# VachaLab/gorder

Hardware: AMD Instinct MI355X
Metric: trajectory frames/sec (higher is better)
Workload: dtype f32

## Files before the change

### gorder_amd/csrc/gorder_hip.hip

```cpp
#include <hip/hip_runtime.h>

#include <dlfcn.h>

#include <cmath>
#include <cstdio>
#include <cstdlib>
#include <cstring>
#include <mutex>
#include <new>
#include <string>
#include <deque>
#include <type_traits>
#include <vector>

#include "../../include/gorder_hip.h"
#include "gm_math.h"
#include "plan.h"
#include "collect_store.h"
#include "device_mem.h"
#include "replay_rows.h"
#include "leaflet_rows.h"
#include "timewise_blocks.h"
#include "ordermap_final.h"
#include "order_route.h"
#include "molecule_rows.h"
#include "ua_molecule_rows.h"
#include "order_hist.h"
#include "bond_corr.h"
#include "neighbour_classes.h"

#pragma clang fp contract(off)

using gorder::DirectItem;
using gorder::Item;
using gorder::kBlock;
using gorder::Plan;
using gorder::Tile;

#include "kernels_common.h"
#include "kernels_tile.h"
#include "kernels_bonds.h"
#include "kernels_extras.h"
#include "kernels_ua.h"
#include "kernels_molrows.h"
#include "kernels_radial.h"
#include "kernels_neighbours.h"
#include "kernels_hist.h"
#include "kernels_ua_samples.h"
#include "kernels_corr.h"
#include "kernels_leaflets.h"
#include "kernels_cluster.h"
#include "kernels_cluster_cutoff.h"
#include "kernels_normals.h"
#include "kernels_xtc.h"
#include "kernels_trr.h"
#include "kernels_collect.h"
#include "kernels_replay.h"
#include "kernels_timewise.h"
#include "kernels_ordermap.h"


struct DeviceMem {
    static void *alloc(size_t bytes) { void *p = nullptr; return hipMalloc(&p, bytes) == hipSuccess ? p : nullptr; }
    static void release(void *p) { (void)hipFree(p); }
};
struct PinnedMem {
    static void *alloc(size_t bytes) { void *p = nullptr; return hipHostMalloc(&p, bytes) == hipSuccess ? p : nullptr; }
    static void release(void *p) { (void)hipHostFree(p); }
};
template <typename T> using DBuf = gorder::Buf<T, DeviceMem>;
template <typename T> using HBuf = gorder::Buf<T, PinnedMem>;
using u64 = unsigned long long;

struct Event {
    hipEvent_t ev = nullptr;
    Event() = default;
    Event(const Event &) = delete;
    Event &operator=(const Event &) = delete;
    ~Event() { if (ev) (void)hipEventDestroy(ev); }
    hipError_t create(unsigned flags = hipEventDisableTiming) { return ev ? hipSuccess : hipEventCreateWithFlags(&ev, flags); }
    operator hipEvent_t() const { return ev; }
};
struct Stream {
    hipStream_t s = nullptr;
    Stream() = default;
    Stream(const Stream &) = delete;
    Stream &operator=(const Stream &) = delete;
    ~Stream() { if (s) (void)hipStreamDestroy(s); }
    hipError_t create() { return s ? hipSuccess : hipStreamCreateWithFlags(&s, hipStreamNonBlocking); }
    operator hipStream_t() const { return s; }
};

struct RepAcc {
    DBuf<u64> acc, rep;
    uint32_t n_rep = 1;
    size_t words = 0;
    bool alloc(size_t n_words, uint32_t n_rep_wanted) {
        words = n_words;
        n_rep = gorder::replica_count(n_rep_wanted, n_words);
        return acc.alloc(words) && rep.alloc((size_t)n_rep * words);
    }
    void reset() { acc.reset(); rep.reset(); words = 0; }
    hipError_t zero_async(hipStream_t stream) {
        const hipError_t e = hipMemsetAsync(acc, 0, words * sizeof(u64), stream);
        return e != hipSuccess ? e : hipMemsetAsync(rep, 0, (size_t)n_rep * words * sizeof(u64), stream);
    }
    hipError_t fold(hipStream_t stream) {
        hipLaunchKernelGGL(k_fold_replicas, dim3((uint32_t)((words + 255) / 256)), dim3(256), 0, stream, acc.get(), rep.get(), n_rep, (uint32_t)words);
        return hipGetLastError();
    }
};

struct BondCorr {
    std::vector<uint32_t> lags;
    DBuf<uint32_t> d_lags;
    DBuf<float4> ring;
    uint32_t ring_planes = 0, subrange = 0;
    uint32_t plane_items = 0;
    uint64_t seen = 0;
    RepAcc acc;
    uint32_t forced_subrange = 0;
    bool chunk_major = false;
    bool on() const { return !lags.empty(); }
};

struct NeighbourClasses {
    uint32_t n_classes = 0;
    float radius = 0.0f, thr = 0.0f;
    std::vector<uint32_t> centres, neighbours;
    DBuf<uint32_t> d_centres, d_neighbours;
    DBuf<uint8_t> rows;
    uint32_t rows_frames = 0;
    RepAcc acc;
    size_t lds_bytes = 0;
    bool direct = false;
    bool force_direct = false;
    uint32_t forced_subrange = 0;
    uint64_t row_bytes = gorder::kClassRowBytes;
    bool on() const { return n_classes != 0; }
};

struct gorder_hip_handle {
    void *traj_cache = nullptr;
    void (*traj_cache_free)(gorder_hip_handle *) = nullptr;
    Plan plan;
    gorder_tables_t tables{};
    int device = 0;
    Stream own_stream;
    hipStream_t stream = nullptr;
    DBuf<Tile> d_tiles;
    DBuf<Item> d_items;
    DBuf<uint32_t> d_tile_slots;
    DBuf<DirectItem> d_direct;
    DBuf<Tile> d_ua_tiles;
    DBuf<gorder::UaItem> d_ua_items;
    DBuf<uint32_t> d_ua_tile_slots;
    uint32_t map_nx = 0, map_ny = 0;
    DBuf<u64> d_map_sums, d_map_cnts;
    DBuf<u64> d_map_packed;
    DBuf<u64> d_map_rec;
    DBuf<gorder::MapRun> d_ua_runs, d_runs;
    DBuf<uint32_t> d_ua_run_begin, d_run_begin;
    DBuf<Item> d_items_by_slot;
    DBuf<uint32_t> d_ua_item_run, d_item_run;
    DBuf<uint4> d_lgrid;
    DBuf<LocalRowPre> d_lrowpre;
    DBuf<LocalEdge> d_ledge;
    DBuf<float4> d_lfinfo;
    static constexpr uint32_t kDecidePause = 16;
    DBuf<uint32_t> d_lsummary;
    HBuf<uint32_t> h_lsummary;
    Event lsummary_written;
    bool lsummary_pending = false;
    uint32_t decide_pause = 0;
    uint64_t decide_submits = 0, decide_paused_submits = 0;
    DBuf<uint32_t> d_lneed;
    DBuf<uint2> d_ltodo;
    size_t map_lds_bytes = 0;
    bool map_staged = false;
    uint64_t map_pending = 0;
    uint64_t map_fold_limit = kMapFoldLimit;
    uint32_t map_max_mol = 1;
    DBuf<u64> d_tw_sums, d_tw_cnts;
    uint64_t tw_cap = 0;
    DBuf<u64> d_twx_blocks, d_twx_rows, d_twx_totals, d_twx_edge;
    DBuf<uint32_t> d_twx_groups;
    DBuf<float> d_twx_out;
    DBuf<uint32_t> d_omx_groups;
    DBuf<float> d_omx_out;
    ExtraArgs extra{};
    DBuf<uint32_t> d_geom_group;
    DBuf<float> d_shapes;
    DBuf<float> d_inv_box;
    uint32_t dyn_slab = 4, local_slab = 4;
    bool local_halo = false;
    size_t local_rec_stride = 0;
    DBuf<XtcCheckpoint> d_xtc_cp;
    bool dyn = false;
    DBuf<uint32_t> d_dyn_cloud, d_dyn_heads;
    DBuf<uint32_t> d_dyn_cell_of, d_dyn_count;
    DBuf<float> d_dyn_rec;
    DBuf<float4> d_dyn_normals;
    DBuf<DynCov> d_dyn_cov;
    std::vector<float> last_normals;
    std::vector<float> manual_normals;
    uint32_t manual_frames = 0;
    bool manual_active = false;
    DBuf<uint32_t> d_err;
    u64 *d_acc = nullptr;
    DBuf<u64> own_acc;
    DBuf<u64> d_rep;
    uint32_t n_rep = 32;
    bool rep_dirty = false;
    size_t acc_words = 0;
    DBuf<uint32_t> d_heads, d_membrane, d_methyl_begin, d_methyl_atoms;
    DBuf<uint8_t> d_aflags;
    size_t aflags_rows = 0;
    DBuf<float> d_adist;
    DBuf<float> d_sph_spill, d_sph_stats;
    uint32_t sph_spill = 0, sph_slab = 1u << 20, sph_threads = 1024;
    DBuf<char> d_cl_scratch;
    DBuf<uint32_t> d_cl_head_slot;
    DBuf<uint8_t> d_cl_carry, d_cl_is0;
    DBuf<float> d_cl_stats;
    uint32_t cl_slab = 1, cl_m_max = 0;
    bool cl_stored_w = false;
    bool cl_have_carry = false;
    bool cl_cut = false;
    uint32_t cl_tiles = 0, cl_sort = 0;
    std::vector<uint8_t> cl_is0;
    DBuf<uint32_t> d_lcell_of, d_lcell_count, d_lcell_fill;
    DBuf<float> d_ltrig;
    DBuf<uint32_t> d_arow, d_aframes;
    std::vector<uint32_t> up_arow, up_aframes;
    bool up_arow_valid = false, up_aframes_valid = false;
    bool have_assignment = false;
    uint64_t assignment_frame = 0;
    bool spec_enabled = false;
    DBuf<uint2> d_own;
    DBuf<float4> d_mom;
    DBuf<float> d_head_z;
    DBuf<uint32_t> d_own_head_begin;
    DBuf<uint2> d_own_heads;
    DBuf<float> d_spec_center;
    DBuf<uint8_t> d_spec_ok;
    DBuf<uint32_t> d_spec_counters;
    static constexpr uint32_t kSpecRing = 8;
    HBuf<uint32_t> h_spec_counters;
    Event spec_counters_copied[kSpecRing];
    uint64_t spec_ring_frames[kSpecRing] = {};
    DBuf<uint32_t> d_spec_mol_begin;
    DBuf<SpecSample> d_spec_samples;
    uint64_t spec_batches = 0, spec_fixed = 0, spec_exact_frames = 0;
    DBuf<float> d_stage_xyz[2], d_stage_box[2];
    Event stage_copied[2], stage_computed[2];
    bool stage_used[2] = {false, false};
    int stage_next = 0;
    Stream copy_stream;
    float n2 = 1.0f, n2sq = 1.0f;
    int axis = -1;
    int frames_per_stage = kFramesPerStage;
    bool membrane_is_frame = false;
    bool use_gather = false;
    uint32_t wg_capacity = 256u * 6u;
    uint32_t wg_target = 0;
    uint32_t lw = 0;
    size_t lds_bytes = 0;
    uint64_t n_frames = 0;
    uint64_t err_index = 0;
    std::string err_msg;
    static constexpr uint32_t kTimingEvents = 1024;
    struct TimingSeg { uint32_t label, ev_a, ev_b; };
    bool timing_on = false;
    Event timing_ev[kTimingEvents];
    uint32_t timing_next_ev = 0;
    int timing_open_label = -1;
    uint32_t timing_open_ev = 0;
    std::deque<TimingSeg> timing_pending;
    std::vector<std::string> timing_labels;
    std::vector<double> timing_label_ms;
    std::vector<uint64_t> timing_label_n;
    uint64_t timing_launches = 0;
    std::string timed_kernels;
    std::vector<uint32_t> host_heads, host_dyn_heads;
    DBuf<uint32_t> d_mol_slot0;
    uint64_t err_frame = 0;
    struct BatchLog { uint64_t ordinal, first, stride; std::vector<uint64_t> list; };
    static constexpr size_t kBatchLog = 4096;
    std::deque<BatchLog> batch_log;
    uint64_t n_submits = 0;
    const unsigned long long *decoder_key = nullptr;
    uint32_t collect = 0;
    bool collect_locked = false;
    gorder::CollectStore collect_flags;
    gorder::CollectStore collect_normals;
    DBuf<u64> d_collect_words;
    DBuf<CollectVec3> d_collect_vec;
    DBuf<uint8_t> d_touched;
    DBuf<u64> d_ltable;
    gorder::ReplayWindow ltable_win;
    bool replay_have_carry = false;
    uint64_t replay_carry_index = 0;
    DBuf<ReplayVec3> d_ntable;
    gorder::ReplayWindow ntable_win;
    uint32_t ntable_step = 1;
    DBuf<uint32_t> d_nrow;
    uint32_t n_shells = 0;
    float shell_thr[GORDER_RADIAL_MAX_SHELLS] = {};
    RepAcc shells;
    size_t shell_lds_bytes = 0;
    bool shell_direct = false;
    bool shell_force_direct = false;
    uint32_t hist_edges = 0;
    DBuf<int32_t> d_hist_edges;
    RepAcc hist;
    size_t hist_table_words = 0;
    bool hist_direct = false;
    bool hist_force_direct = false;
    uint32_t hist_samples_per_word = gorder::kDistSamplesPerWord;
    BondCorr corr;
    NeighbourClasses nb;
    gorder::MolRows mol;
    DBuf<Item> d_mol_items;
    DBuf<gorder::MolRun> d_mol_runs;
    DBuf<uint32_t> d_mol_run_begin;
    gorder::UaMolRows ua_mol;
    DBuf<gorder::UaLaneWords> d_ua_mol_lanes;
    DBuf<uint32_t> d_ua_mol_words, d_ua_mol_word_begin;
    DBuf<u64> d_mol_stage;
    size_t mol_stage_bytes = (size_t)1 << 30;
    gorder::CollectStore mol_store;
    const uint64_t *mol_frame_index = nullptr;
    bool mol_failed = false;
    std::deque<std::pair<uint64_t, uint64_t>> mol_batch_log;
};

namespace {

int fail(gorder_hip_handle *h, int status, const std::string &msg) {
    if (h) h->err_msg = msg;
    return status;
}

#define HIP_TRY(h, expr)                                                                    \
    do {                                                                                    \
        hipError_t e_ = (expr);                                                             \
        if (e_ != hipSuccess)                                                               \
            return fail(h, GORDER_ERR_DEVICE, std::string(#expr) + ": " + hipGetErrorString(e_)); \
    } while (0)

#define ST_TRY(expr)                                \
    do {                                            \
        const int st_ = (expr);                     \
        if (st_ != GORDER_OK) return st_;           \
    } while (0)

int alloc_failed(gorder_hip_handle *h, const char *call) {
    return fail(h, GORDER_ERR_DEVICE, std::string(call) + ": " + hipGetErrorString(hipGetLastError()));
}

template <typename T, typename Mem>
int allocate(gorder_hip_handle *h, gorder::Buf<T, Mem> &dst, size_t n, int fill = -1) {
    if (!dst.alloc(n)) return alloc_failed(h, std::is_same<Mem, DeviceMem>::value ? "hipMalloc" : "hipHostMalloc");
    if (fill >= 0 && n) HIP_TRY(h, hipMemset(dst, fill, n * sizeof(T)));
    return GORDER_OK;
}

template <typename T>
int upload(gorder_hip_handle *h, DBuf<T> &dst, const std::vector<T> &src) {
    ST_TRY(allocate(h, dst, src.size()));
    if (!src.empty()) HIP_TRY(h, hipMemcpy(dst, src.data(), src.size() * sizeof(T), hipMemcpyHostToDevice));
    return GORDER_OK;
}

template <typename T>
int ensure(gorder_hip_handle *h, DBuf<T> &buf, size_t need, bool *grew = nullptr) {
    const gorder::Reserve r = buf.reserve(need);
    if (grew) *grew = r == gorder::Reserve::Grew;
    return r == gorder::Reserve::Failed ? alloc_failed(h, "hipMalloc") : GORDER_OK;
}

int alloc_zeroed(gorder_hip_handle *h, RepAcc &r, size_t words) {
    if (!r.alloc(words, h->n_rep)) {
        r.reset();
        return alloc_failed(h, "hipMalloc");
    }
    HIP_TRY(h, r.zero_async(h->stream));
    return GORDER_OK;
}

uint32_t sample_atom(const Plan &p, uint32_t slot, uint32_t mol, uint32_t which) {
    for (const Tile &t : p.tiles)
        for (uint32_t q = 0; q < t.n_items; q++) {
            const Item &it = p.items[t.item0 + q];
            if (it.mol == mol && p.tile_slots[t.slot0 + it.lslot] == slot) return t.atom0 + (which ? it.lj : it.li);
        }
    for (const DirectItem &d : p.direct)
        if (d.mol == mol && d.slot == slot) return which ? d.j : d.i;
    for (const Tile &t : p.ua_tiles)
        for (uint32_t q = 0; q < t.n_items; q++) {
            const gorder::UaItem &it = p.ua_items[t.item0 + q];
            if (it.mol == mol && p.ua_tile_slots[t.slot0 + it.lslot0] == slot) return t.atom0 + it.l[which & 3u];
        }
    return 0;
}

// ... 217 lines not shown
                                       b.aflags, b.arow, h->d_tiles, h->d_mol_items, h->d_tile_slots, n_tiles, h->lw);
                });
            }); }); });
            HIP_TRY(h, hipGetLastError());
        }
        if (ua) {
            const gorder::FrameChunks c = gorder::extras_chunks(nf, n_ua, h->wg_target, h->wg_capacity, false, true);
            const uint64_t grid = ua_grid(n_ua, c.n_chunks);
            if (grid > 0x7fffffffull) return fail(h, GORDER_ERR_INVALID_ARGUMENT, "batch too large");
            b.frames_per_chunk = c.frames_per_chunk;
            if (bonds) TIMING_MARK(h, "k_ua_mol");
            with_bool(ac, [&](auto AC) {
                hipLaunchKernelGGL((k_ua_mol<AC()>), dim3((uint32_t)grid), dim3(kBlock), gorder::ua_mol_lds_bytes(h->ua_mol.max_local), h->stream, b, e,
                                   um, b.xyz, b.box9, b.aflags, b.arow, h->d_ua_tiles, h->d_ua_items, h->d_ua_tile_slots, n_ua);
            });
            HIP_TRY(h, hipGetLastError());
        }
        if ((st = collect_copy_out(h, h->mol_store, h->d_mol_stage, h->mol_frame_index + lo, nf)) != GORDER_OK) return st;
    }
    return GORDER_OK;
}

bool literal_cosine(const gorder_hip_handle *h) { return (h->tables.flags & GORDER_FLAG_TRIG_ACOS_COS) != 0; }

int launch_geometry_shapes(gorder_hip_handle *h, const FrameArgs &a) {
    ST_TRY(ensure(h, h->d_shapes, (size_t)a.n_frames * 8));
    const gorder_geometry_t &ge = h->tables.geometry;
    GeomArgs ga{};
    ga.xyz = a.xyz; ga.box9 = a.box9; ga.n_atoms = a.n_atoms; ga.pbc = a.pbc;
    ga.kind = ge.kind; ga.reference = ge.reference; ga.orientation = ge.orientation;
    for (int d = 0; d < 3; d++) { ga.point[d] = ge.point[d]; ga.structure_box[d] = ge.structure_box[d]; }
    for (int d = 0; d < 2; d++) { ga.xdim[d] = ge.xdim[d]; ga.ydim[d] = ge.ydim[d]; ga.zdim[d] = ge.zdim[d]; ga.span[d] = ge.span[d]; }
    ga.radius = ge.radius; ga.group = h->d_geom_group; ga.n_group = ge.n_group;
    ga.shapes = h->d_shapes; ga.err = h->d_err;
    TIMING_MARK(h, "k_geom_shapes");
    hipLaunchKernelGGL(k_geom_shapes, dim3(a.n_frames), dim3(256), 0, h->stream, ga);
    HIP_TRY(h, hipGetLastError());
    return GORDER_OK;
}

int launch_tiled(gorder_hip_handle *h, FrameArgs &a, const gorder::OrderRoute &route) {
    const uint32_t n_tiles = (uint32_t)h->plan.tiles.size();
    const gorder::FrameChunks c = gorder::tiled_chunks(a.n_frames, (uint32_t)h->frames_per_stage, n_tiles, h->wg_target, h->wg_capacity);
    a.frames_per_chunk = c.frames_per_chunk;
    const uint64_t grid = (uint64_t)n_tiles * c.n_chunks;
    if (grid > 0x7fffffffull) return fail(h, GORDER_ERR_INVALID_ARGUMENT, "batch too large");
    const dim3 g((uint32_t)grid), b(kBlock);
    TIMING_MARK(h, route.label);
    with_bool(literal_cosine(h), [&](auto AC) { with_bool(a.pbc, [&](auto PBC) { with_bool(a.leaflets, [&](auto LF) {
        if (route.family == gorder::BondFamily::Gather)
            hipLaunchKernelGGL((k_bonds_gather<4, AC(), PBC(), LF()>), g, b, 0, h->stream, a, a.xyz, a.box9, a.aflags, a.arow,
                               h->d_tiles, h->d_items, h->d_tile_slots, n_tiles);
        else with_npf(route.npf, [&](auto NPF) { with_axis(h->axis, [&](auto AX) { with_bool(route.mom, [&](auto MOM) {
            if constexpr (LF() || !MOM())
                hipLaunchKernelGGL((k_bonds_tiled<4, NPF(), AC(), PBC(), LF(), AX(), MOM()>), g, b, h->lds_bytes, h->stream, a,
                                   a.xyz, a.box9, a.aflags, a.arow, h->d_tiles, h->d_items, h->d_tile_slots, n_tiles, h->lw);
        }); }); });
    }); }); });
    HIP_TRY(h, hipGetLastError());
    return GORDER_OK;
}

struct SubRange {
    const FrameArgs &a;
    const gorder::OrderRoute &route;
    uint32_t lo, hi;
    bool class_rows_whole;
    uint32_t nf() const { return hi - lo; }
    FrameArgs frames(const gorder::FrameChunks &c) const {
        FrameArgs b = a;
        b.frame0 = lo; b.n_frames = hi; b.frames_per_chunk = c.frames_per_chunk;
        return b;
    }
};
const Item *bond_items(const gorder_hip_handle *h, const gorder::OrderRoute &route) { return route.items_by_slot ? h->d_items_by_slot : h->d_items; }

int launch_classes(gorder_hip_handle *h, const SubRange &s) {
    const Plan &p = h->plan;
    NeighbourClasses &nb = h->nb;
    const uint32_t nt = (uint32_t)p.tiles.size(), nf = s.nf();
    const gorder::FrameChunks c = gorder::shells_chunks(nf, nt, h->wg_target, h->wg_capacity, kShellChunkMax);
    FrameArgs b = s.frames(c);
    ClassArgs ca{};
    ca.centres = nb.d_centres; ca.neighbours = nb.d_neighbours; ca.n_neighbours = (uint32_t)nb.neighbours.size();
    ca.thr = nb.thr; ca.n = nb.n_classes; ca.rows = nb.rows; ca.row_base = s.class_rows_whole ? 0u : s.lo;
    ca.axis = h->axis; ca.rep = nb.acc.rep; ca.n_rep = nb.acc.n_rep;
    nb.rows_frames = s.class_rows_whole ? s.a.n_frames : nf;
    TIMING_MARK(h, "k_neighbour_counts");
    hipLaunchKernelGGL(k_neighbour_counts, dim3((p.n_mol_total + 255u) / 256u, nf), dim3(256), 0, h->stream, ca, b.xyz, b.box9,
                       b.n_atoms, p.n_mol_total, b.pbc, s.lo, h->d_err);
    TIMING_MARK(h, s.route.label);
    const size_t lds = nb.direct ? (size_t)kBlock * 24u : nb.lds_bytes;
    with_bool(literal_cosine(h), [&](auto AC) { with_bool(nb.direct, [&](auto DIRECT) {
        hipLaunchKernelGGL((k_bonds_classes<AC(), DIRECT()>), dim3(nt * c.n_chunks), dim3(kBlock), lds, h->stream, b, ca, b.xyz, b.box9,
                           b.aflags, b.arow, h->d_tiles, bond_items(h, s.route), h->d_tile_slots, nt);
    }); });
    return GORDER_OK;
}

int launch_shells(gorder_hip_handle *h, const SubRange &s, const ExtraArgs &e) {
    const uint32_t nt = (uint32_t)h->plan.tiles.size();
    const gorder::FrameChunks c = gorder::shells_chunks(s.nf(), nt, h->wg_target, h->wg_capacity, kShellChunkMax);
    FrameArgs b = s.frames(c);
    ShellArgs sa{};
    sa.n = h->n_shells; sa.rep = h->shells.rep; sa.n_rep = h->shells.n_rep;
    for (uint32_t k = 0; k < GORDER_RADIAL_MAX_SHELLS; k++) sa.thr[k] = k < h->n_shells ? h->shell_thr[k] : INFINITY;
    const size_t lds = h->shell_direct ? (size_t)kBlock * 24u : h->shell_lds_bytes;
    TIMING_MARK(h, s.route.label);
    with_bool(literal_cosine(h), [&](auto AC) { with_bool(h->shell_direct, [&](auto DIRECT) {
        hipLaunchKernelGGL((k_bonds_shells<AC(), DIRECT()>), dim3(nt * c.n_chunks), dim3(kBlock), lds, h->stream, b, e, sa, b.xyz, b.box9,
                           b.aflags, b.arow, h->d_tiles, bond_items(h, s.route), h->d_tile_slots, nt);
    }); });
    return GORDER_OK;
}

int launch_dist(gorder_hip_handle *h, const SubRange &s, const ExtraArgs &e) {
    const uint32_t nt = (uint32_t)h->plan.tiles.size();
    const gorder::FrameChunks c = gorder::dist_chunks(s.nf(), nt, h->wg_target, h->wg_capacity, h->hist_direct ? 0u : (uint32_t)h->hist_table_words,
                                                      h->hist_samples_per_word, kDistChunkMax);
    FrameArgs b = s.frames(c);
    DistArgs da{};
    da.n_edges = h->hist_edges; da.edges = h->d_hist_edges; da.rep = h->hist.rep; da.n_rep = h->hist.n_rep;
    const size_t lds = kDistEdgeBytes + std::max<size_t>(kDistReduceBytes, h->hist_direct ? 0u : h->hist_table_words * sizeof(uint32_t));
    TIMING_MARK(h, s.route.label);
    with_bool(literal_cosine(h), [&](auto AC) { with_bool(h->hist_direct, [&](auto DIRECT) {
        hipLaunchKernelGGL((k_bonds_dist<AC(), DIRECT()>), dim3(nt * c.n_chunks), dim3(kBlock), lds, h->stream, b, e, da, b.xyz, b.box9,
                           b.aflags, b.arow, h->d_tiles, bond_items(h, s.route), h->d_tile_slots, nt);
    }); });
    return GORDER_OK;
}

int launch_extras(gorder_hip_handle *h, const SubRange &s, const ExtraArgs &e) {
    const uint32_t nt = (uint32_t)h->plan.tiles.size();
    const gorder::FrameChunks c = gorder::extras_chunks(s.nf(), nt, h->wg_target, h->wg_capacity, s.route.map_accumulate, false);
    FrameArgs b = s.frames(c);
    TIMING_MARK(h, s.route.label);
    with_bool(literal_cosine(h), [&](auto AC) { with_bool(s.route.maps_only, [&](auto MO) {
        hipLaunchKernelGGL((k_bonds_extras<AC(), MO()>), dim3(nt * c.n_chunks), dim3(kBlock), 0, h->stream, b, e, b.xyz, b.box9, b.aflags,
                           b.arow, h->d_tiles, bond_items(h, s.route), h->d_tile_slots, nt);
    }); });
    return GORDER_OK;
}

int launch_tiled_out(gorder_hip_handle *h, const SubRange &s, const ExtraArgs &e) {
    const gorder::OrderRoute &route = s.route;
    const uint32_t nt = (uint32_t)h->plan.tiles.size();
    const gorder::FrameChunks c = gorder::extras_chunks(s.nf(), nt, h->wg_target, h->wg_capacity, route.map_accumulate,
                                                        route.family == gorder::BondFamily::TiledTw);
    FrameArgs b = s.frames(c);
    const dim3 g(nt * c.n_chunks), blk(kBlock);
    const Item *items = bond_items(h, route);
    TIMING_MARK(h, route.label);
    with_npf(route.npf, [&](auto NPF) { with_bool(b.pbc, [&](auto PBC) { with_bool(b.leaflets, [&](auto LF) { with_axis(h->axis, [&](auto AX) {
        if (route.family == gorder::BondFamily::TiledMaps)
            hipLaunchKernelGGL((k_bonds_tiled_maps<NPF(), PBC(), LF(), AX()>), g, blk, h->lds_bytes, h->stream, b, e, b.xyz,
                               b.box9, b.aflags, b.arow, h->d_tiles, items, h->d_tile_slots, nt, h->lw);
        else with_bool(route.tw_maps, [&](auto MAPS) { with_bool(route.mom, [&](auto MOM) {
            if constexpr (!MOM() || (LF() && !MAPS()))
                hipLaunchKernelGGL((k_bonds_tiled_tw<NPF(), PBC(), LF(), AX(), MAPS(), MOM()>), g, blk, h->lds_bytes, h->stream, b, e,
                                   b.xyz, b.box9, b.aflags, b.arow, h->d_tiles, items, h->d_tile_slots, nt, h->lw);
        }); });
    }); }); }); });
    return GORDER_OK;
}

int launch_map_accumulate(gorder_hip_handle *h, const SubRange &s, uint32_t rec_stride, const gorder::MapRun *runs,
                          const uint32_t *run_begin, uint32_t per_item) {
    const uint32_t n_acc = h->plan.n_acc;
    const uint32_t planes = h->tables.leaflets.method != GORDER_LEAFLETS_NONE ? 2u : 1u;
    const uint32_t ntm = h->map_nx * h->map_ny, n_words = planes * ntm;
    const char *ev = getenv("GORDER_HIP_MAP_CHUNKS");
    const gorder::FrameChunks m = gorder::map_chunks(s.nf(), n_acc, ev ? (uint32_t)std::max(1, atoi(ev)) : 0u);
    TIMING_MARK(h, "k_map_accumulate");
    hipLaunchKernelGGL(k_map_accumulate, dim3(n_acc * m.n_chunks), dim3(1024), n_words * sizeof(unsigned long long), h->stream,
                       h->d_map_rec, runs, run_begin, n_acc, s.nf(), rec_stride, m.frames_per_chunk, per_item, n_words, ntm,
                       h->d_map_packed, n_acc);
    return GORDER_OK;
}

int launch_bond_pass(gorder_hip_handle *h, const SubRange &s, ExtraArgs &e) {
    using gorder::BondFamily;
    e.item_run = h->d_item_run;
    switch (s.route.family) {
    case BondFamily::Classes: ST_TRY(launch_classes(h, s)); break;
    case BondFamily::Shells: ST_TRY(launch_shells(h, s, e)); break;
    case BondFamily::Dist: ST_TRY(launch_dist(h, s, e)); break;
    case BondFamily::Extras: ST_TRY(launch_extras(h, s, e)); break;
    default: ST_TRY(launch_tiled_out(h, s, e)); break;
    }
    if (s.route.map_accumulate) ST_TRY(launch_map_accumulate(h, s, e.rec_stride, h->d_runs, h->d_run_begin, 1u));
    HIP_TRY(h, hipGetLastError());
    return GORDER_OK;
}

int launch_ua_dist(gorder_hip_handle *h, const SubRange &s, const ExtraArgs &e) {
    const uint32_t nt = (uint32_t)h->plan.ua_tiles.size();
    const gorder::FrameChunks c = gorder::dist_chunks(s.nf(), nt, h->wg_target, h->wg_capacity, h->hist_direct ? 0u : (uint32_t)h->hist_table_words,
                                                      h->hist_samples_per_word, kDistChunkMax);
    FrameArgs b = s.frames(c);
    DistArgs da{};
    da.n_edges = h->hist_edges; da.edges = h->d_hist_edges; da.rep = h->hist.rep; da.n_rep = h->hist.n_rep;
    const size_t lds = kDistEdgeBytes + std::max<size_t>(kUaSumBytes, h->hist_direct ? 0u : h->hist_table_words * sizeof(uint32_t));
    const dim3 g((uint32_t)ua_grid(nt, c.n_chunks)), blk(kBlock);
    TIMING_MARK(h, "k_ua_dist");
    with_bool(literal_cosine(h), [&](auto AC) { with_bool(h->hist_direct, [&](auto DIRECT) {
        hipLaunchKernelGGL((k_ua_dist<AC(), DIRECT()>), g, blk, lds, h->stream, b, e, da, b.xyz, b.box9, b.aflags, b.arow, h->d_ua_tiles,
                           h->d_ua_items, h->d_ua_tile_slots, nt);
    }); });
    HIP_TRY(h, hipGetLastError());
    return GORDER_OK;
}

int launch_ua_pass(gorder_hip_handle *h, const SubRange &s, ExtraArgs &e) {
    const gorder::OrderRoute &route = s.route;
    if (route.ua_kernel == gorder::UaKernel::Dist) return launch_ua_dist(h, s, e);
    const uint32_t nt = (uint32_t)h->plan.ua_tiles.size();
    const gorder::FrameChunks c = gorder::extras_chunks(s.nf(), nt, h->wg_target, h->wg_capacity, route.map_accumulate, false);
    FrameArgs b = s.frames(c);
    e.item_run = h->d_ua_item_run;
    const dim3 g((uint32_t)ua_grid(nt, c.n_chunks)), blk(kBlock);
    TIMING_MARK(h, "k_ua_extras");
    with_bool(literal_cosine(h), [&](auto AC) { with_bool(route.ua_fast, [&](auto FAST) { with_int<0, 1, 2, 3>(route.ua_mode, [&](auto MODE) {
        if constexpr (FAST() && !AC())
            hipLaunchKernelGGL((k_ua_extras_fast<MODE()>), g, blk, 0, h->stream, b, e, b.xyz, b.box9, b.aflags, b.arow,
                               h->d_ua_tiles, h->d_ua_items, h->d_ua_tile_slots, nt, (const float *)e.inv_box);
        else if constexpr (!FAST())
            hipLaunchKernelGGL((k_ua_extras<AC(), MODE()>), g, blk, 0, h->stream, b, e, b.xyz, b.box9, b.aflags, b.arow,
                               h->d_ua_tiles, h->d_ua_items, h->d_ua_tile_slots, nt, (const float *)nullptr);
    }); }); });
    if (route.map_accumulate) ST_TRY(launch_map_accumulate(h, s, e.rec_stride, h->d_ua_runs, h->d_ua_run_begin, 3u));
    HIP_TRY(h, hipGetLastError());
    return GORDER_OK;
}

int launch_scatter_passes(gorder_hip_handle *h, const FrameArgs &a, const gorder::OrderRoute &route) {
    const Plan &p = h->plan;
    ExtraArgs e = h->extra;
    e.tw_sums = h->d_tw_sums; e.tw_cnts = h->d_tw_cnts; e.tw_row0 = h->n_frames;
    e.shapes = h->d_shapes; e.inv_box = nullptr;
    if (route.ua_fast && a.pbc) {
        ST_TRY(ensure(h, h->d_inv_box, (size_t)a.n_frames * 8));
        hipLaunchKernelGGL(k_inv_box, dim3((4u * a.n_frames + 255u) / 256u), dim3(256), 0, h->stream, a.box9, a.n_frames, h->d_inv_box);
        e.inv_box = h->d_inv_box;
    }
    e.dyn = (h->dyn || h->manual_active) ? h->d_dyn_normals : nullptr;
    const bool staged = route.map_accumulate;
    const size_t rec_per_frame = std::max(p.ua_tiles.size() * 3u, route.extras ? p.tiles.size() : (size_t)0) * kBlock;
    uint32_t sub = gorder::map_subrange(a.n_frames, e.maps != 0, staged, h->map_fold_limit, h->map_max_mol, rec_per_frame);
    bool class_rows_whole = false;
    if (route.family == gorder::BondFamily::Classes) {
        class_rows_whole = gorder::class_rows_whole(a.n_frames, p.n_mol_total, h->nb.row_bytes);
        sub = gorder::class_subrange(a.n_frames, p.n_mol_total, h->nb.forced_subrange, h->nb.row_bytes);
        ST_TRY(ensure(h, h->nb.rows, (size_t)(class_rows_whole ? a.n_frames : sub) * p.n_mol_total));
    }
    if (staged) ST_TRY(ensure(h, h->d_map_rec, rec_per_frame * (((size_t)sub + 15) / 16 * 16)));
    e.map_rec = staged ? h->d_map_rec : nullptr;
    for (uint32_t lo = 0; lo < a.n_frames; lo += sub) {
        const SubRange s{a, route, lo, std::min(a.n_frames, lo + sub), class_rows_whole};
        if (e.maps) {
            const uint64_t cost = (uint64_t)s.nf() * h->map_max_mol;
            if (h->map_pending + cost >= h->map_fold_limit) ST_TRY(fold_maps(h));
            h->map_pending += cost;
        }
        e.rec_frame0 = lo; e.rec_stride = (s.nf() + 15u) / 16u * 16u;
        if (route.extras && !p.tiles.empty()) ST_TRY(launch_bond_pass(h, s, e));
        if (!p.ua_tiles.empty() && route.ua_kernel != gorder::UaKernel::Mol) ST_TRY(launch_ua_pass(h, s, e));
    }
    return GORDER_OK;
}

int launch_bonds_direct(gorder_hip_handle *h, const FrameArgs &a) {
    const uint32_t n_items = (uint32_t)h->plan.direct.size(), bpc = (n_items + kBlock - 1) / kBlock;
    const gorder::FrameChunks c = gorder::direct_chunks(a.n_frames, bpc, h->wg_target);
    FrameArgs b = a;
    b.frames_per_chunk = c.frames_per_chunk;
    TIMING_MARK(h, "k_bonds_direct");
    with_bool(literal_cosine(h), [&](auto AC) { hipLaunchKernelGGL(k_bonds_direct<AC()>, dim3(bpc * c.n_chunks), dim3(kBlock), 0, h->stream, b, h->d_direct, n_items, bpc); });
    HIP_TRY(h, hipGetLastError());
    return GORDER_OK;
}

int launch_orders(gorder_hip_handle *h, FrameArgs &a, const gorder::OrderRoute &route) {
    using gorder::BondFamily;
    if (h->dyn && !h->manual_active) ST_TRY(run_dynamic_normals(h, a));
    if (h->extra.geom_kind) ST_TRY(launch_geometry_shapes(h, a));
    if (route.family == BondFamily::Tiled || route.family == BondFamily::Gather) ST_TRY(launch_tiled(h, a, route));
    const bool ua_mol = route.ua_kernel == gorder::UaKernel::Mol;
    if (route.family == BondFamily::TiledMol || ua_mol) ST_TRY(launch_molecule_rows(h, a, route));
    if (route.extras || (route.ua_mode >= 0 && !ua_mol)) ST_TRY(launch_scatter_passes(h, a, route));
    if (route.direct) ST_TRY(launch_bonds_direct(h, a));
    return GORDER_OK;
}

int collect_copy_out(gorder_hip_handle *h, gorder::CollectStore &store, const void *d_block, const uint64_t *frames, size_t n_rows) {
    std::vector<gorder::CollectPiece> pieces;
    if (!store.reserve(frames, n_rows, pieces)) return fail(h, GORDER_ERR_DEVICE, "collect: no pinned host memory for the history");
    const char *src = static_cast<const char *>(d_block);
    for (const gorder::CollectPiece &pc : pieces) {
        const size_t bytes = pc.rows * store.row_bytes();
        HIP_TRY(h, hipMemcpyAsync(pc.host, src, bytes, hipMemcpyDeviceToHost, h->stream));
        src += bytes;
    }
    return GORDER_OK;
}

int collect_flag_rows(gorder_hip_handle *h, size_t first_row, const std::vector<uint64_t> &frames) {
    if (frames.empty()) return GORDER_OK;
    const uint32_t n_mol = h->plan.n_mol_total, wpr = (uint32_t)gorder::collect_flag_words(n_mol);
    const unsigned long long total = (unsigned long long)frames.size() * wpr;
    if ((total + 3u) / 4u > 0x7fffffffull || frames.size() > 0xffffffffull) return fail(h, GORDER_ERR_INVALID_ARGUMENT, "collect: batch too large");
    int st;
    if ((st = ensure(h, h->d_collect_words, (size_t)total)) != GORDER_OK) return st;
    TIMING_MARK(h, "k_collect_flags");
    hipLaunchKernelGGL(k_collect_flags, dim3((uint32_t)((total + 3u) / 4u)), dim3(256), 0, h->stream,
                       h->d_aflags + first_row * (size_t)n_mol, n_mol, (uint32_t)frames.size(), wpr, h->d_collect_words);
    HIP_TRY(h, hipGetLastError());
    return collect_copy_out(h, h->collect_flags, h->d_collect_words, frames.data(), frames.size());
}

int collect_normal_rows(gorder_hip_handle *h, const uint64_t *frame_index, uint32_t n_frames, const uint8_t *touched) {
    const unsigned long long n = (unsigned long long)n_frames * h->plan.n_mol_total;
    if ((n + 255u) / 256u > 0x7fffffffull) return fail(h, GORDER_ERR_INVALID_ARGUMENT, "collect: batch too large");
    int st;
    if ((st = ensure(h, h->d_collect_vec, (size_t)n)) != GORDER_OK) return st;
    TIMING_MARK(h, "k_collect_normals");
    hipLaunchKernelGGL(k_collect_normals, dim3((uint32_t)((n + 255u) / 256u)), dim3(256), 0, h->stream,
                       (const float4 *)h->d_dyn_normals, touched, n, h->d_collect_vec);
    HIP_TRY(h, hipGetLastError());
    return collect_copy_out(h, h->collect_normals, h->d_collect_vec, frame_index, n_frames);
}

int upload_rows(gorder_hip_handle *h, DBuf<uint32_t> &buf, const std::vector<uint32_t> &rows) {
    ST_TRY(ensure(h, buf, rows.size()));
    HIP_TRY(h, hipMemcpyAsync(buf, rows.data(), rows.size() * sizeof(uint32_t), hipMemcpyHostToDevice, h->stream));
    return GORDER_OK;
}
int upload_if_changed(gorder_hip_handle *h, DBuf<uint32_t> &buf, std::vector<uint32_t> &held, bool &valid, const std::vector<uint32_t> &rows) {
    bool grew = false;
    const int st = ensure(h, buf, rows.size(), &grew);
    if (grew || st != GORDER_OK) valid = false;
    if (st != GORDER_OK || (valid && held == rows)) return st;
    ST_TRY(upload_rows(h, buf, rows));
// ... 168 lines not shown
    }
    return st;
}

namespace {
__global__ void k_selftest_trig(int fn, uint32_t first_bits, uint32_t stride, uint32_t n, float *out) {
    const uint32_t i = blockIdx.x * blockDim.x + threadIdx.x;
    if (i >= n) return;
    const float x = __uint_as_float(first_bits + i * stride);
    float s, c;
    gm_sincosf_0pi(x, s, c);
    out[i] = fn == 0 ? gm_acosf_t<false>(x) : fn == 1 ? gm_acosf_t<true>(x) : fn == 2 ? c : s;
}
}

int gorder_hip_selftest_trig(int device, int fn, uint32_t first_bits, uint32_t stride, uint32_t n, float *out) {
    if (!out || fn < 0 || fn > 3) return GORDER_ERR_INVALID_ARGUMENT;
    int count = 0;
    if (hipGetDeviceCount(&count) != hipSuccess || count <= 0) return GORDER_ERR_NO_DEVICE;
    if (device < 0 || device >= count || hipSetDevice(device) != hipSuccess) return GORDER_ERR_INVALID_ARGUMENT;
    if (n == 0) return GORDER_OK;
    DBuf<float> d;
    if (!d.alloc(n)) return GORDER_ERR_DEVICE;
    hipLaunchKernelGGL(k_selftest_trig, dim3((n + 255u) / 256u), dim3(256), 0, 0, fn, first_bits, stride, n, d.get());
    if (hipDeviceSynchronize() != hipSuccess || hipMemcpy(out, d, (size_t)n * sizeof(float), hipMemcpyDeviceToHost) != hipSuccess)
        return GORDER_ERR_DEVICE;
    return GORDER_OK;
}

namespace {
__global__ __launch_bounds__(1024) void k_selftest_wave_ops(const double *in_f64, const float *in_f32, const uint32_t *in_u32,
                                                            int finfo_empty, double *out_f64, float *out_f32, uint32_t *out_u32,
                                                            uint4 *out_finfo) {
    __shared__ double scratch[32];
    __shared__ float fscratch[32], l_lo[16], l_hi[16];
    __shared__ uint32_t l_flags[16];
    const uint32_t tid = threadIdx.x, lane = tid & 63u, n = blockDim.x;
    const double d = in_f64[tid];
    const float x = in_f32[tid];
    const uint32_t u = in_u32[tid];
    if (tid < 16u) { l_lo[tid] = 3.0e38f; l_hi[tid] = -3.0e38f; l_flags[tid] = 0u; }
    __syncthreads();
    double s = d, q = 3.0 * d, bs[2] = {d, 3.0 * d};
    float lo4 = x, hi4 = x, lo2 = x, hi2 = x, lo3 = x, hi3 = x, blo = x, bhi = x;
    uint32_t or3 = u;
    wave_sum2_minmax_bfly(s, q, lo4, hi4);
    wave_minmax_bfly(lo2, hi2);
    wave_minmax_or_bfly(lo3, hi3, or3);
    block_sum_n<2>(bs, scratch);
    block_minmax(blo, bhi, fscratch);
    const double o64[GORDER_WAVE_OPS_F64_ROWS] = {row_sum(d), rows_to_wave(row_sum(d)), wave_sum_rows(d), wave_scan_rows(d, lane),
                                                  wave_sum_bfly(d), bs[0], bs[1], lane_value(d, 47), s, q};
    const float o32[GORDER_WAVE_OPS_F32_ROWS] = {row_sum(x), rows_to_wave(row_sum(x)), wave_sum_rows(x), wave_min_rows(x),
                                                 wave_max_rows(x), lo2, hi2, blo, bhi, dpp_or_self<0x111>(x),
                                                 dpp_or_zero<0x143, 0xc>(x), lane_value(x, 47), lo4, hi4, lo3, hi3};
    const uint32_t ou[GORDER_WAVE_OPS_U32_ROWS] = {row_sum(u), rows_to_wave(row_sum(u)), wave_sum_rows(u), wave_scan_rows(u, lane),
                                                   wave_scan_shfl(u, lane), or3, wave_max_bfly(u),
                                                   (uint32_t)wave_sum_rows((int)u), lane_value(u, 47)};
    for (int r = 0; r < GORDER_WAVE_OPS_F64_ROWS; r++) out_f64[r * n + tid] = o64[r];
    for (int r = 0; r < GORDER_WAVE_OPS_F32_ROWS; r++) out_f32[r * n + tid] = o32[r];
    for (int r = 0; r < GORDER_WAVE_OPS_U32_ROWS; r++) out_u32[r * n + tid] = ou[r];
    const float zlo = finfo_empty ? 3.0e38f : x, zhi = finfo_empty ? -3.0e38f : x;
    uint32_t fl = u;
    block_finfo_record(zlo, zhi, fl, ~0u, l_lo, l_hi, l_flags, out_finfo);
    if (tid == 0u) out_finfo[2].x = fl;
    __syncthreads();
    fl = u;
    block_finfo_record(zlo, zhi, fl, 1u, l_lo, l_hi, l_flags, out_finfo + 1);
}
}

int gorder_hip_selftest_wave_ops(int device, uint32_t block, const double *f64, const float *f32, const uint32_t *u32,
                                 int finfo_empty, double *out_f64, float *out_f32, uint32_t *out_u32, uint32_t *out_finfo) {
    if (!f64 || !f32 || !u32 || !out_f64 || !out_f32 || !out_u32 || !out_finfo || block < 64u || block > 1024u || (block & 63u))
        return GORDER_ERR_INVALID_ARGUMENT;
    int count = 0;
    if (hipGetDeviceCount(&count) != hipSuccess || count <= 0) return GORDER_ERR_NO_DEVICE;
    if (device < 0 || device >= count || hipSetDevice(device) != hipSuccess) return GORDER_ERR_INVALID_ARGUMENT;
    const size_t n = block, b_fi = 0, b_i64 = 48, b_o64 = b_i64 + 8 * n, b_i32 = b_o64 + 8 * n * GORDER_WAVE_OPS_F64_ROWS,
                 b_iu = b_i32 + 4 * n, b_o32 = b_iu + 4 * n, b_ou = b_o32 + 4 * n * GORDER_WAVE_OPS_F32_ROWS,
                 bytes = b_ou + 4 * n * GORDER_WAVE_OPS_U32_ROWS;
    DBuf<char> owned;
    if (!owned.alloc(bytes)) return GORDER_ERR_DEVICE;
    char *d = owned;
    int st = GORDER_OK;
    if (hipMemset(d, 0, bytes) != hipSuccess || hipMemcpy(d + b_i64, f64, 8 * n, hipMemcpyHostToDevice) != hipSuccess ||
        hipMemcpy(d + b_i32, f32, 4 * n, hipMemcpyHostToDevice) != hipSuccess ||
        hipMemcpy(d + b_iu, u32, 4 * n, hipMemcpyHostToDevice) != hipSuccess)
        st = GORDER_ERR_DEVICE;
    if (st == GORDER_OK) {
        hipLaunchKernelGGL(k_selftest_wave_ops, dim3(1), dim3(block), 0, 0, (const double *)(d + b_i64), (const float *)(d + b_i32),
                           (const uint32_t *)(d + b_iu), finfo_empty, (double *)(d + b_o64), (float *)(d + b_o32),
                           (uint32_t *)(d + b_ou), (uint4 *)(d + b_fi));
        if (hipDeviceSynchronize() != hipSuccess ||
            hipMemcpy(out_f64, d + b_o64, 8 * n * GORDER_WAVE_OPS_F64_ROWS, hipMemcpyDeviceToHost) != hipSuccess ||
            hipMemcpy(out_f32, d + b_o32, 4 * n * GORDER_WAVE_OPS_F32_ROWS, hipMemcpyDeviceToHost) != hipSuccess ||
            hipMemcpy(out_u32, d + b_ou, 4 * n * GORDER_WAVE_OPS_U32_ROWS, hipMemcpyDeviceToHost) != hipSuccess ||
            hipMemcpy(out_finfo, d + b_fi, 4 * GORDER_WAVE_OPS_FINFO_WORDS, hipMemcpyDeviceToHost) != hipSuccess)
            st = GORDER_ERR_DEVICE;
    }
    return st;
}

int gorder_hip_plan_tables(const gorder_tables_t *tables, gorder_hip_plan_t *out, int *selfcheck) {
    if (!tables || !out) return GORDER_ERR_INVALID_ARGUMENT;
    Plan p;
    ST_TRY(gorder::build_plan(*tables, env_flag("GORDER_HIP_FORCE_DIRECT"), p));
    out->n_tiles = (uint32_t)p.tiles.size();
    out->block_threads = kBlock;
    out->max_window_atoms = p.max_window;
    out->n_direct_items = (uint32_t)p.direct.size();
    out->frames_per_stage = kFramesPerStage;
    const uint32_t lw = ((3u * p.max_window + 3u + 3u) / 4u) * 4u;
    size_t lds = (size_t)kFramesPerStage * lw * sizeof(float);
    if (lds < (size_t)kBlock * 24) lds = (size_t)kBlock * 24;
    out->lds_bytes = (uint32_t)lds;
    out->map_staged = 0;
    out->map_lds_bytes = 0;
    out->leaflets_one_read = p.spec_ok ? 1u : 0u;
    if (selfcheck) *selfcheck = gorder::selfcheck_plan(*tables, p);
    return GORDER_OK;
}

static size_t cl_frame_bytes(uint32_t n, uint32_t m_max);
static size_t clcut_frame_bytes(uint32_t n, uint32_t m_max);

static int create_ordermaps(gorder_hip_handle *h, const gorder_tables_t *t) {
    const gorder_ordermap_t &om = t->ordermap;
    if (!om.enabled) return GORDER_OK;
    const Plan &p = h->plan;
    ExtraArgs &e = h->extra;
    if (!(om.bin[0] > 0.0f) || !(om.bin[1] > 0.0f) || om.plane > 2)
        return fail(h, GORDER_ERR_INVALID_ARGUMENT, "ordermap bin/plane");
    const float fx = roundf((om.span_x[1] - om.span_x[0]) / om.bin[0]);
    const float fy = roundf((om.span_y[1] - om.span_y[0]) / om.bin[1]);
    if (!(fx >= 0.0f) || !(fy >= 0.0f) || fx > 65535.0f || fy > 65535.0f)
        return fail(h, GORDER_ERR_INVALID_ARGUMENT, "ordermap span");
    h->map_nx = (uint32_t)fx + 1u;
    h->map_ny = (uint32_t)fy + 1u;
    const size_t nmap = 3 * (size_t)p.n_acc * h->map_nx * h->map_ny;
    const size_t npk = (t->leaflets.method != GORDER_LEAFLETS_NONE ? 2 : 1) * (nmap / 3);
    ST_TRY(allocate(h, h->d_map_sums, nmap, 0));
    ST_TRY(allocate(h, h->d_map_cnts, nmap, 0));
    ST_TRY(allocate(h, h->d_map_packed, npk, 0));
    const size_t lds_bytes = npk / p.n_acc * sizeof(u64);
    h->map_lds_bytes = lds_bytes;
    if (lds_bytes <= 150u * 1024u && !env_flag("GORDER_HIP_MAP_DIRECT")) {
        ST_TRY(upload(h, h->d_ua_runs, p.ua_runs));
        ST_TRY(upload(h, h->d_ua_run_begin, p.ua_run_begin));
        ST_TRY(upload(h, h->d_runs, p.runs));
        ST_TRY(upload(h, h->d_run_begin, p.run_begin));
        ST_TRY(upload(h, h->d_items_by_slot, p.items_by_slot));
        ST_TRY(upload(h, h->d_ua_item_run, p.ua_item_run));
        HIP_TRY(h, hipFuncSetAttribute(reinterpret_cast<const void *>(k_map_accumulate),
                                       hipFuncAttributeMaxDynamicSharedMemorySize, (int)lds_bytes));
        h->map_staged = true;
    }
    e.maps = 1; e.plane = om.plane; e.x0 = om.span_x[0]; e.y0 = om.span_y[0];
    e.binx = om.bin[0]; e.biny = om.bin[1]; e.nx = h->map_nx; e.ny = h->map_ny;
    e.inv_binx = 1.0f / om.bin[0]; e.inv_biny = 1.0f / om.bin[1];
    e.bin_core = (om.bin[0] >= 0x1p-40f && om.bin[0] <= 0x1p+40f && om.bin[1] >= 0x1p-40f && om.bin[1] <= 0x1p+40f) ? 1 : 0;
    e.map_packed = h->d_map_packed;
    return GORDER_OK;
}

static int create_geometry(gorder_hip_handle *h, const gorder_tables_t *t) {
    const gorder_geometry_t &ge = t->geometry;
    if (ge.kind == GORDER_GEOM_NONE) return GORDER_OK;
    ExtraArgs &e = h->extra;
    if (ge.kind > GORDER_GEOM_SPHERE || ge.reference > GORDER_GEOMREF_GROUP || ge.orientation > 2)
        return fail(h, GORDER_ERR_INVALID_ARGUMENT, "geometry kind/reference/orientation");
    if (ge.reference == GORDER_GEOMREF_BOX_CENTER && !t->handle_pbc)
        return fail(h, GORDER_ERR_INVALID_ARGUMENT, "box-centre reference needs handle_pbc (pbc.rs:243-245)");
    if (ge.reference == GORDER_GEOMREF_POINT && t->handle_pbc &&
        !(ge.structure_box[0] > 0.0f && ge.structure_box[1] > 0.0f && ge.structure_box[2] > 0.0f))
        return fail(h, GORDER_ERR_INVALID_ARGUMENT, "geometry.structure_box");
    if (ge.reference == GORDER_GEOMREF_GROUP) {
        if (!ge.group || ge.n_group == 0) return fail(h, GORDER_ERR_INVALID_ARGUMENT, "geometry.group");
        std::vector<uint32_t> grp(ge.group, ge.group + ge.n_group);
        for (uint32_t a : grp)
            if (a >= t->n_atoms) return fail(h, GORDER_ERR_INVALID_ARGUMENT, "geometry group index out of range");
        ST_TRY(upload(h, h->d_geom_group, grp));
    }
    e.geom_kind = (int)ge.kind; e.geom_invert = ge.invert ? 1 : 0; e.geom_orient = (int)ge.orientation;
    e.geom_thr = local_radius_threshold(ge.radius);
    h->tables.geometry.group = nullptr;
    return GORDER_OK;
}

static int create_accumulators(gorder_hip_handle *h) {
    const Plan &p = h->plan;
    ST_TRY(allocate(h, h->d_err, kErrWords + 2u));
    HIP_TRY(h, hipMemset(h->d_err, 0xff, kErrWords * sizeof(uint32_t)));
    HIP_TRY(h, hipMemset(h->d_err + kErrWords, 0, 2u * sizeof(uint32_t)));
    h->acc_words = 4 * (size_t)p.n_acc + 1;
    ST_TRY(allocate(h, h->own_acc, h->acc_words, 0));
    h->d_acc = h->own_acc;
    if (const char *e = getenv("GORDER_HIP_MAP_FOLD_LIMIT")) {
        const long v = atol(e);
        if (v >= 2 && (unsigned long long)v <= kMapFoldLimit) h->map_fold_limit = (uint64_t)v;
    }
    if (const char *e = getenv("GORDER_HIP_REPLICAS")) {
        const int r = atoi(e);
        if (r >= 1 && r <= 1024) h->n_rep = (uint32_t)r;
    }
    return p.n_acc ? allocate(h, h->d_rep, (size_t)h->n_rep * 4u * p.n_acc, 0) : GORDER_OK;
}

static int local_build_attributes(gorder_hip_handle *h) {
    for (const void *fn : {reinterpret_cast<const void *>(k_local_build<2>), reinterpret_cast<const void *>(k_local_build<5>),
                           reinterpret_cast<const void *>(k_local_build<kLocalBuildTrips>)})
        HIP_TRY(h, hipFuncSetAttribute(fn, hipFuncAttributeMaxDynamicSharedMemorySize, (int)kLocalBuildLds));
    return GORDER_OK;
}

static int create_dynamic_normals(gorder_hip_handle *h, const gorder_tables_t *t) {
    const gorder_dynamic_normal_t &dn = t->dynamic_normal;
    if (!dn.enabled) return GORDER_OK;
    const Plan &p = h->plan;
    if (!(dn.radius > 0.0f)) return fail(h, GORDER_ERR_INVALID_ARGUMENT, "dynamic normals need a positive radius");
    if (!dn.cloud || dn.n_cloud == 0) return fail(h, GORDER_ERR_INVALID_ARGUMENT, "dynamic normals need the NormalHeads group");
    if (!p.direct.empty()) return fail(h, GORDER_ERR_INVALID_ARGUMENT, "dynamic normals: a bond spans more than the LDS window");
    std::vector<uint32_t> cloud(dn.cloud, dn.cloud + dn.n_cloud), nheads;
    for (uint32_t a : cloud)
        if (a >= t->n_atoms) return fail(h, GORDER_ERR_INVALID_ARGUMENT, "NormalHeads index out of range");
    for (uint32_t m = 0; m < t->n_molecule_types; m++) {
        const gorder_moltype_t &mt = t->molecule_types[m];
        if (!mt.normal_heads) return fail(h, GORDER_ERR_INVALID_ARGUMENT, "dynamic normals need normal_heads[] per molecule type");
        for (uint32_t k = 0; k < mt.n_molecules; k++) {
            if (mt.normal_heads[k] >= t->n_atoms) return fail(h, GORDER_ERR_INVALID_ARGUMENT, "normal head index out of range");
            nheads.push_back(mt.normal_heads[k]);
        }
    }
    ST_TRY(upload(h, h->d_dyn_cloud, cloud));
    ST_TRY(upload(h, h->d_dyn_heads, nheads));
    h->host_dyn_heads = nheads;
    const size_t nm = dn.n_cloud, ncell = (size_t)kLocalMaxCells1D * kLocalMaxCells1D;
    const size_t sl = h->dyn_slab = local_slab_frames(nm);
    ST_TRY(local_build_attributes(h));
    ST_TRY(allocate(h, h->d_dyn_cell_of, sl * nm));
    ST_TRY(allocate(h, h->d_dyn_rec, sl * nm * 4));
    ST_TRY(allocate(h, h->d_dyn_count, sl * (2 * ncell + 1)));
    ST_TRY(allocate(h, h->d_dyn_cov, sl * (size_t)(p.n_mol_total ? p.n_mol_total : 1)));
    h->dyn = true;
    return GORDER_OK;
}

static int create_leaflet_tables(gorder_hip_handle *h, const gorder_tables_t *t, std::vector<uint32_t> &heads) {
    const gorder_leaflets_t &lf = t->leaflets;
    const Plan &p = h->plan;
    if (lf.method > GORDER_LEAFLETS_CLUSTERING) return fail(h, GORDER_ERR_INVALID_ARGUMENT, "leaflets.method");
    if (lf.method != GORDER_LEAFLETS_SPHERICAL && lf.method != GORDER_LEAFLETS_CLUSTERING && lf.normal_dim > 2) return fail(h, GORDER_ERR_INVALID_ARGUMENT, "leaflets.normal_dim");
    std::vector<uint32_t> mb(1, 0), ma;
    for (uint32_t m = 0; m < t->n_molecule_types; m++) {
        const gorder_moltype_t &mt = t->molecule_types[m];
        if (lf.method != GORDER_LEAFLETS_MANUAL && !mt.heads)
            return fail(h, GORDER_ERR_INVALID_ARGUMENT, "leaflets need heads[] per molecule type");
        if (lf.method == GORDER_LEAFLETS_INDIVIDUAL && (!mt.methyls || mt.n_methyls == 0))
            return fail(h, GORDER_ERR_INVALID_ARGUMENT, "individual leaflets need methyls[]");
        for (uint32_t k = 0; k < mt.n_molecules; k++) {
            const uint32_t hd = mt.heads ? mt.heads[k] : 0;
            if (hd >= t->n_atoms) return fail(h, GORDER_ERR_INVALID_ARGUMENT, "head index out of range");
            heads.push_back(hd);
            if (lf.method == GORDER_LEAFLETS_INDIVIDUAL)
                for (uint32_t q = 0; q < mt.n_methyls; q++) {
                    const uint32_t a = mt.methyls[(size_t)k * mt.n_methyls + q];
                    if (a >= t->n_atoms) return fail(h, GORDER_ERR_INVALID_ARGUMENT, "methyl index out of range");
                    ma.push_back(a);
                }
            mb.push_back((uint32_t)ma.size());
        }
    }
    ST_TRY(upload(h, h->d_heads, heads));
    h->host_heads = heads;
    if (lf.method == GORDER_LEAFLETS_LOCAL) {
        std::vector<uint32_t> ms;
        for (uint32_t m = 0; m < t->n_molecule_types; m++) ms.insert(ms.end(), t->molecule_types[m].n_molecules, p.slot0[m]);
        ST_TRY(upload(h, h->d_mol_slot0, ms));
    }
    ST_TRY(upload(h, h->d_methyl_begin, mb));
    ST_TRY(upload(h, h->d_methyl_atoms, ma));
    if (lf.method == GORDER_LEAFLETS_LOCAL && !(lf.radius > 0.0f))
        return fail(h, GORDER_ERR_INVALID_ARGUMENT, "local leaflets need a positive radius");
    if (lf.method == GORDER_LEAFLETS_GLOBAL || lf.method == GORDER_LEAFLETS_LOCAL) {
        if (!lf.membrane || lf.n_membrane == 0)
            return fail(h, GORDER_ERR_INVALID_ARGUMENT, "global/local leaflets need the membrane group");
        std::vector<uint32_t> mem(lf.membrane, lf.membrane + lf.n_membrane);
        for (uint32_t a : mem)
            if (a >= t->n_atoms) return fail(h, GORDER_ERR_INVALID_ARGUMENT, "membrane index out of range");
        ST_TRY(upload(h, h->d_membrane, mem));
        h->membrane_is_frame = lf.n_membrane == t->n_atoms && !env_flag("GORDER_HIP_LEAFLETS_GENERIC");
        for (uint32_t i = 0; i < lf.n_membrane && h->membrane_is_frame; i++) h->membrane_is_frame = mem[i] == i;
    }
    return GORDER_OK;
}

static int upload_cluster_group(gorder_hip_handle *h, const gorder_tables_t *t, const std::vector<uint32_t> &heads, bool ascending,
                                std::vector<uint32_t> &head_slot) {
    const gorder_leaflets_t &lf = t->leaflets;
    std::vector<uint32_t> grp(lf.membrane, lf.membrane + lf.n_membrane);
    std::vector<int32_t> slot_of(t->n_atoms, -1);
    for (uint32_t i = 0; i < lf.n_membrane; i++) {
        if (grp[i] >= t->n_atoms) return fail(h, GORDER_ERR_INVALID_ARGUMENT, "leaflets.membrane: index out of range");
        if (ascending && i && grp[i] <= grp[i - 1]) return fail(h, GORDER_ERR_INVALID_ARGUMENT, "leaflets.membrane: clustering needs ascending, distinct atoms");
        if (slot_of[grp[i]] < 0) slot_of[grp[i]] = (int32_t)i;
    }
    for (uint32_t hd : heads) {
// ... 398 lines not shown
        hipLaunchKernelGGL(k_cluster_embed, dim3(ns), dim3(1024), 0, h->stream, ca);
        TIMING_MARK(h, "k_cluster_orient");
        hipLaunchKernelGGL(k_cluster_orient, dim3(1), dim3(1024), 0, h->stream, oa);
    }
    h->cl_have_carry = true;
    return GORDER_OK;
}

static int launch_global_leaflets(gorder_hip_handle *h, const LeafletArgs &la) {
    const dim3 g(la.skip ? std::min<uint32_t>(la.n_assign, 512u) : la.n_assign), b(1024);
    TIMING_MARK(h, h->membrane_is_frame ? "k_leaflets_global_contig" : "k_leaflets_global");
    if (h->membrane_is_frame) {
        if (la.skip) hipLaunchKernelGGL(k_leaflets_global_contig<true>, g, dim3(256), 0, h->stream, la);
        else hipLaunchKernelGGL(k_leaflets_global_contig<false>, g, dim3(256), 0, h->stream, la);
    } else {
        if (la.skip) hipLaunchKernelGGL(k_leaflets_global<true>, g, b, 0, h->stream, la);
        else hipLaunchKernelGGL(k_leaflets_global<false>, g, b, 0, h->stream, la);
    }
    return GORDER_OK;
}

static int launch_individual_leaflets(gorder_hip_handle *h, const LeafletArgs &la) {
    TIMING_MARK(h, "k_leaflets_individual");
    for (uint32_t done = 0; done < la.n_assign;) {
        const uint32_t ny = std::min<uint32_t>(la.n_assign - done, 65535u);
        LeafletArgs lb = la;
        lb.aframes = la.aframes + done;
        lb.row0 = la.row0 + done;
        if (done + ny < la.n_assign) lb.adist = nullptr;
        hipLaunchKernelGGL(k_leaflets_individual, dim3((la.n_mol_total + 255) / 256, ny), dim3(256), 0,
                           h->stream, lb);
        done += ny;
    }
    return GORDER_OK;
}

static int launch_spherical_leaflets(gorder_hip_handle *h, const LeafletArgs &la) {
    TIMING_MARK(h, "k_leaflets_spherical");
    SphArgs sa{};
    sa.xyz = la.xyz; sa.box9 = la.box9; sa.n_atoms = la.n_atoms;
    sa.aflags = la.aflags; sa.n_mol_total = la.n_mol_total; sa.heads = la.heads;
    sa.group = la.membrane; sa.n_group = la.n_membrane;
    sa.flip = la.flip; sa.pbc = la.pbc;
    sa.spill = h->d_sph_spill; sa.n_spill = h->sph_spill; sa.err = la.err;
    for (size_t done = 0; done < la.n_assign; done += h->sph_slab) {
        const uint32_t ns = (uint32_t)std::min<size_t>(la.n_assign - done, h->sph_slab);
        const bool last = done + ns == la.n_assign;
        sa.aframes = la.aframes + done;
        sa.row0 = la.row0 + (uint32_t)done;
        sa.n_assign = ns;
        sa.adist = last ? h->d_adist : nullptr;
        sa.stats = last ? h->d_sph_stats : nullptr;
        if (h->sph_threads == 256u) hipLaunchKernelGGL(k_leaflets_spherical<256>, dim3(ns), dim3(256), 0, h->stream, sa);
        else hipLaunchKernelGGL(k_leaflets_spherical<1024>, dim3(ns), dim3(1024), 0, h->stream, sa);
    }
    return GORDER_OK;
}

struct LocalDecisions { bool decide, sums, report; };
static LocalDecisions local_decisions(gorder_hip_handle *h, const LocalArgs &lo) {
    LocalDecisions d{};
    d.decide = lo.halo && lo.prune && lo.n_mol_total && !env_flag("GORDER_HIP_LOCAL_NO_DECIDE");
    if (d.decide) {
        if (h->lsummary_pending) {
            if (hipEventQuery(h->lsummary_written) == hipSuccess) {
                h->lsummary_pending = false;
                if (2u * h->h_lsummary[0] > h->h_lsummary[1]) h->decide_pause = gorder_hip_handle::kDecidePause;
            } else {
                (void)hipGetLastError();
            }
        }
        if (h->decide_pause) { h->decide_pause--; h->decide_paused_submits++; d.decide = false; }
        else h->decide_submits++;
    }
    d.sums = d.decide && lo.n_membrane <= kLocalBuildMax && !env_flag("GORDER_HIP_LOCAL_THREE_KERNELS") &&
             !env_flag("GORDER_HIP_LOCAL_NO_SUMS");
    d.report = d.decide && !h->lsummary_pending;
    return d;
}

static int launch_local_slabs(gorder_hip_handle *h, LocalArgs lo, uint32_t n_assign, uint32_t row0, bool report) {
    const size_t ncell = (size_t)kLocalMaxCells1D * kLocalMaxCells1D;
    for (size_t done = 0; done < n_assign; done += h->local_slab) {
        const uint32_t ns = (uint32_t)std::min<size_t>(n_assign - done, h->local_slab);
        lo.aframes = h->d_aframes + done;
        lo.n_slab = ns;
        lo.row0 = row0 + (uint32_t)done;
        lo.write_dist_frame = (done + ns == n_assign) ? (int)ns - 1 : -1;
        lo.summary_host = report && done + ns == n_assign ? h->h_lsummary : nullptr;
        if (lo.n_membrane > kLocalBuildMax || env_flag("GORDER_HIP_LOCAL_THREE_KERNELS"))
            HIP_TRY(h, hipMemsetAsync(h->d_lcell_fill, 0, ns * ncell * sizeof(uint32_t), h->stream));
        if (lo.sums) {
            HIP_TRY(h, hipMemsetAsync(h->d_lneed, 0, (ns + 1) * sizeof(uint32_t), h->stream));
            TIMING_MARK(h, "k_local_sums");
            hipLaunchKernelGGL(k_local_sums, dim3(ns), dim3(1024), kSumsLds, h->stream, lo);
            TIMING_MARK(h, "k_local_decide");
            hipLaunchKernelGGL(k_local_decide, dim3(ns), dim3(1024), kDecideLds, h->stream, lo);
        }
        ST_TRY(launch_cell_list(h, lo, ns, lo.n_membrane, h->d_lcell_count, ns * (ncell + 1) * sizeof(uint32_t)));
        if (lo.halo) {
            TIMING_MARK(h, "k_local_rowprefix");
            hipLaunchKernelGGL(k_local_rowprefix, dim3(kLocalMaxCells1D / 4u, ns), dim3(256), 0, h->stream, lo);
            lo.rows_groups = (lo.n_mol_total + 15u) / 16u;
            if (lo.need && !lo.sums) {
                TIMING_MARK(h, "k_local_decide");
                hipLaunchKernelGGL(k_local_decide, dim3(ns), dim3(1024), kDecideLds, h->stream, lo);
            }
            TIMING_MARK(h, "k_local_flags_rows");
            if (lo.need) hipLaunchKernelGGL(k_local_flags_rows_open, dim3(lo.rows_groups * 8u * kRowsSlots), dim3(256), 0, h->stream, lo);
            else hipLaunchKernelGGL(k_local_flags_rows, dim3(lo.rows_groups * ((ns + 7u) / 8u * 8u)), dim3(256), 0, h->stream, lo);
            TIMING_MARK(h, "k_local_flags_todo");
            hipLaunchKernelGGL(k_local_flags_todo, dim3(512), dim3(256), 0, h->stream, lo);
        } else {
            TIMING_MARK(h, "k_local_flags");
            hipLaunchKernelGGL(k_local_flags, dim3((lo.n_mol_total + 3) / 4, ns), dim3(256), 0, h->stream, lo);
        }
    }
    return GORDER_OK;
}

static int launch_local_leaflets(gorder_hip_handle *h, const LeafletArgs &la) {
    const gorder_leaflets_t &lf = h->tables.leaflets;
    LocalArgs lo{};
    lo.xyz = la.xyz; lo.box9 = la.box9; lo.n_atoms = la.n_atoms;
    lo.aflags = la.aflags; lo.adist = la.adist; lo.n_mol_total = la.n_mol_total;
    lo.heads = la.heads; lo.mol_slot0 = h->d_mol_slot0; lo.n_membrane = la.n_membrane;
    lo.membrane = h->membrane_is_frame ? nullptr : h->d_membrane;
    lo.dim = la.dim; lo.flip = la.flip; lo.pbc = la.pbc;
    lo.radius = lf.radius;
    lo.radius_thr = local_radius_threshold(lf.radius);
    lo.cell_of = h->d_lcell_of; lo.trig = h->d_ltrig; lo.cell_count = h->d_lcell_count;
    lo.cell_fill = h->d_lcell_fill; lo.err = la.err;
    lo.grid = h->d_lgrid;
    lo.halo = h->local_halo ? 1 : 0;
    lo.prune = env_flag("GORDER_HIP_LOCAL_NO_PRUNE") ? 0 : (env_flag("GORDER_HIP_LOCAL_DECIDE_NOTHING") ? 2 : 1);
    lo.rec_stride = (uint32_t)h->local_rec_stride;
    lo.rowpre = h->d_lrowpre;
    lo.edge = h->d_ledge;
    lo.finfo = h->d_lfinfo;
    lo.todo = h->d_ltodo;
    const LocalDecisions d = local_decisions(h, lo);
    lo.need = d.decide ? h->d_lneed : nullptr;
    lo.sums = d.sums ? 1 : 0;
    lo.summary = d.report ? h->d_lsummary : nullptr;
    ST_TRY(launch_local_slabs(h, lo, la.n_assign, la.row0, d.report));
    if (d.report) {
        HIP_TRY(h, hipEventRecord(h->lsummary_written, h->stream));
        h->lsummary_pending = true;
    }
    return GORDER_OK;
}

static int run_leaflets(gorder_hip_handle *h, const float *d_xyz, const float *d_box,
                        const std::vector<uint32_t> &aframes, uint32_t row0, const uint8_t *skip = nullptr) {
    if (aframes.empty()) return GORDER_OK;
    ST_TRY(upload_if_changed(h, h->d_aframes, h->up_aframes, h->up_aframes_valid, aframes));
    const gorder_leaflets_t &lf = h->tables.leaflets;
    LeafletArgs la{};
    la.xyz = d_xyz; la.box9 = d_box; la.n_atoms = h->plan.n_atoms;
    la.aframes = h->d_aframes; la.row0 = row0; la.aflags = h->d_aflags; la.adist = h->d_adist;
    la.n_mol_total = h->plan.n_mol_total; la.heads = h->d_heads;
    la.membrane = h->d_membrane; la.n_membrane = lf.n_membrane;
    la.methyl_begin = h->d_methyl_begin; la.methyl_atoms = h->d_methyl_atoms;
    la.dim = lf.normal_dim; la.flip = lf.flip ? 1 : 0; la.pbc = h->tables.handle_pbc ? 1 : 0;
    la.err = h->d_err;
    la.skip = skip;
    la.n_assign = (uint32_t)aframes.size();
    switch (lf.method) {
    case GORDER_LEAFLETS_GLOBAL: ST_TRY(launch_global_leaflets(h, la)); break;
    case GORDER_LEAFLETS_INDIVIDUAL: ST_TRY(launch_individual_leaflets(h, la)); break;
    case GORDER_LEAFLETS_SPHERICAL: ST_TRY(launch_spherical_leaflets(h, la)); break;
    case GORDER_LEAFLETS_CLUSTERING: ST_TRY(run_clustering(h, d_xyz, d_box, aframes.size(), row0)); break;
    case GORDER_LEAFLETS_LOCAL: ST_TRY(launch_local_leaflets(h, la)); break;
    default: break;
    }
    HIP_TRY(h, hipGetLastError());
    return GORDER_OK;
}

static int launch_bond_corr(gorder_hip_handle *h, const FrameArgs &a) {
    BondCorr &bc = h->corr;
    const Plan &p = h->plan;
    const uint32_t n_tiles = (uint32_t)p.tiles.size(), n_lags = (uint32_t)bc.lags.size(), max_lag = bc.lags.back();
    if (!bc.ring) {
        const uint64_t fit = gorder::corr_subrange_fit(gorder::corr_plane_bytes(n_tiles, kBlock), max_lag, gorder::kCorrRingBudget);
        bc.subrange = gorder::corr_subrange(fit, a.n_frames, bc.forced_subrange);
        bc.ring_planes = gorder::corr_ring_planes(max_lag, bc.subrange);
        bc.plane_items = n_tiles * kBlock;
        ST_TRY(allocate(h, bc.ring, (size_t)bc.ring_planes * bc.plane_items));
    }
    CorrArgs c{};
    c.ring = bc.ring; c.ring_planes = bc.ring_planes; c.plane_items = bc.plane_items;
    c.base = gorder::corr_plane_of(bc.seen, bc.ring_planes);
    c.history = (uint32_t)std::min<uint64_t>(bc.seen, GORDER_CORR_MAX_LAG);
    c.n_lags = n_lags; c.lags = bc.d_lags; c.rep = bc.acc.rep; c.n_rep = bc.acc.n_rep; c.n_acc = p.n_acc;
    c.leaflets = a.leaflets; c.aflags = a.aflags; c.arow = a.arow; c.n_mol_total = a.n_mol_total;
    c.xyz = a.xyz; c.box9 = a.box9; c.n_atoms = a.n_atoms; c.pbc = a.pbc;
    for (uint32_t lo = 0; lo < a.n_frames; lo += bc.subrange) {
        const uint32_t hi = (uint32_t)std::min<uint64_t>(a.n_frames, (uint64_t)lo + bc.subrange), nf = hi - lo;
        const gorder::CorrChunks ch = gorder::corr_chunks(nf, n_tiles, h->wg_target, h->wg_capacity);
        const uint32_t n_groups = (n_lags + gorder::kCorrLagBlock - 1u) / gorder::kCorrLagBlock;
        const uint64_t grid = (uint64_t)n_tiles * ch.n_chunks * (bc.chunk_major ? 1u : n_groups);
        if ((uint64_t)n_tiles * nf > 0x7fffffffull || grid > 0x7fffffffull) return fail(h, GORDER_ERR_INVALID_ARGUMENT, "batch too large");
        c.frame0 = lo; c.n_frames = hi; c.frames_per_chunk = ch.frames_per_chunk; c.n_chunks = bc.chunk_major ? 0u : ch.n_chunks;
        TIMING_MARK(h, "k_bond_units");
        hipLaunchKernelGGL(k_bond_units, dim3(n_tiles * nf), dim3(kBlock), 0, h->stream, c, h->d_tiles, h->d_items, n_tiles);
        TIMING_MARK(h, "k_bond_corr");
        hipLaunchKernelGGL((k_bond_corr<gorder::kCorrLagBlock>), dim3((uint32_t)grid), dim3(kBlock), 0, h->stream, c, h->d_tiles,
                           h->d_items, h->d_tile_slots, n_tiles);
        HIP_TRY(h, hipGetLastError());
    }
    return GORDER_OK;
}

static int ensure_flag_rows(gorder_hip_handle *h, size_t need, size_t alloc_rows, bool keep_row0) {
    if (need <= h->aflags_rows) return GORDER_OK;
    const size_t n_mol = h->plan.n_mol_total;
    DBuf<uint8_t> nb;
    ST_TRY(allocate(h, nb, alloc_rows * n_mol));
    if (keep_row0 && h->d_aflags) {
        HIP_TRY(h, hipMemcpyAsync(nb, h->d_aflags, n_mol, hipMemcpyDeviceToDevice, h->stream));
        HIP_TRY(h, hipStreamSynchronize(h->stream));
    }
    h->d_aflags.swap(nb);
    h->aflags_rows = alloc_rows;
    return GORDER_OK;
}

namespace {
struct Batch {
    const float *d_xyz, *d_box;
    const uint64_t *frame_index;
    uint32_t n_frames;
    bool pbc = false, leaflets = false;
    bool ltable = false;
    gorder::ReplayLeafletBatch replay;
    std::vector<uint32_t> normal_rows;
    std::vector<uint32_t> arow, aframes;
    std::vector<uint32_t> spec_aframes;
    std::vector<uint64_t> collect_frames;
    uint64_t last_assign_frame = 0;
    size_t n_new_rows = 0;
    uint64_t mol_rows_before = 0;
    gorder::OrderRouteIn ri;
    gorder::OrderRoute route;
    FrameArgs a{};

    int abort_batch(gorder_hip_handle *h, int status) const {
        h->mol_store.truncate(mol_rows_before);
        hipLaunchKernelGGL(k_batch_abort, dim3(1), dim3(1), 0, h->stream, h->d_err);
        (void)hipGetLastError();
        (void)timing_mark(h, nullptr);
        return status;
    }
};
#define BATCH_TRY(expr)                                                 \
    do {                                                                \
        const int bst_ = (expr);                                        \
        if (bst_ != GORDER_OK) return b.abort_batch(h, bst_);           \
    } while (0)
}

static int check_batch(gorder_hip_handle *h, Batch &b) {
    const gorder_leaflets_t &lf = h->tables.leaflets;
    if ((h->n_frames + b.n_frames) > (uint64_t)(9223372036854775807ll / 1000000ll) / h->map_max_mol)
        return fail(h, GORDER_ERR_OVERFLOW, "order accumulators could overflow i64 (frames x molecules >= 2^63 / 1e6)");
    if (h->manual_frames) {
        if (h->manual_frames != b.n_frames) return fail(h, GORDER_ERR_INVALID_ARGUMENT, "gorder_hip_set_normals: frame count differs from the batch");
        if (!h->plan.direct.empty()) return fail(h, GORDER_ERR_INVALID_ARGUMENT, "manual normals: a bond spans more than the LDS window");
    }
    b.ltable = lf.method == GORDER_LEAFLETS_MANUAL && h->d_ltable;
    uint64_t bad = 0;
    if (b.ltable && gorder::replay_plan_leaflets(lf.frequency, h->ltable_win, h->replay_have_carry, h->replay_carry_index, b.frame_index,
                                                 b.n_frames, b.replay, &bad) != gorder::kReplayOk) {
        h->err_frame = bad;
        return fail(h, GORDER_ERR_MANUAL_LEAFLET_FRAME, "manual leaflet table: no row for frame " + std::to_string(bad));
    }
    if (h->d_ntable) {
        const gorder::ReplayStatus rs = gorder::replay_plan_normals(h->ntable_step, h->ntable_win, b.frame_index, b.n_frames, b.normal_rows, &bad);
        if (rs != gorder::kReplayOk) {
            h->err_frame = bad;
            if (rs == gorder::kReplayBadStep)
                return fail(h, GORDER_ERR_INVALID_ARGUMENT, "manual normal table: frame " + std::to_string(bad) + " is no multiple of the step");
            return fail(h, GORDER_ERR_MANUAL_NORMAL_FRAME, "manual normal table: no row for frame " + std::to_string(bad));
        }
    }
    return GORDER_OK;
}

static int plan_batch_rows(gorder_hip_handle *h, Batch &b) {
    const gorder_leaflets_t &lf = h->tables.leaflets;
    b.last_assign_frame = h->assignment_frame;
    if (!b.leaflets) return GORDER_OK;
    if (b.ltable) {
        b.arow = b.replay.arow;
        b.last_assign_frame = b.replay.carry_index * lf.frequency;
        return GORDER_OK;
    }
    switch (gorder::plan_assignment_rows(lf.method, lf.frequency, h->have_assignment, h->cl_have_carry, b.frame_index, b.n_frames,
                                         b.arow, b.aframes, h->cl_is0, b.last_assign_frame)) {
    case gorder::kLeafletRowsNoClusters:
        return fail(h, GORDER_ERR_LEAFLETS_NOT_PRIMED, "clustering: no clusters of an earlier assignment frame to match against");
    case gorder::kLeafletRowsNotPrimed:
        return fail(h, GORDER_ERR_LEAFLETS_NOT_PRIMED, "no leaflet assignment for the first frame");
    default: return GORDER_OK;
    }
}

static void choose_batch_route(gorder_hip_handle *h, Batch &b) {
    const Plan &p = h->plan;
    gorder::OrderRouteIn &ri = b.ri;
    ri.acos = (h->tables.flags & GORDER_FLAG_TRIG_ACOS_COS) != 0; ri.pbc = b.pbc; ri.leaflets = b.leaflets; ri.axis = h->axis;
    ri.maps = h->extra.maps != 0; ri.map_staged = h->map_staged; ri.tw = h->extra.tw != 0; ri.geom = h->extra.geom_kind != 0;
    ri.manual_frames = h->manual_frames != 0; ri.normal_table = h->d_ntable != nullptr;
    ri.dyn_or_manual = h->dyn || ri.manual_frames || ri.normal_table;
    ri.use_gather = h->use_gather; ri.item_run = h->d_item_run != nullptr; ri.frames_per_stage = h->frames_per_stage; ri.max_window = p.max_window;
    ri.bond_tiles = !p.tiles.empty(); ri.ua_tiles = !p.ua_tiles.empty(); ri.direct_items = !p.direct.empty(); ri.ua_fast_flag = (h->tables.flags & GORDER_FLAG_UA_FAST_NORMALISE) != 0;
    ri.global_leaflets = h->tables.leaflets.method == GORDER_LEAFLETS_GLOBAL; ri.spec_enabled = h->spec_enabled && !h->corr.on(); ri.have_assignment = h->have_assignment;
    ri.shells = h->n_shells != 0;
    ri.dist = h->hist_edges != 0;
    ri.classes = h->nb.on();
    ri.mol_rows = h->mol.n_groups != 0 && !h->mol_failed;
    ri.ua_samples_flag = (h->tables.flags & GORDER_FLAG_UA_SAMPLES) != 0;
    ri.npf5 = env_flag("GORDER_HIP_NPF5"); ri.tw_gather = env_flag("GORDER_HIP_TW_GATHER"); ri.maps_gather = env_flag("GORDER_HIP_MAPS_GATHER");
    ri.every_frame_assigns = b.aframes.size() == b.n_frames;
    b.route = gorder::choose_order_route(ri);
    if (!b.route.speculative) return;
    spec_poll(h, false);
    const uint32_t slot = (uint32_t)(h->spec_batches % gorder_hip_handle::kSpecRing);
    if (h->spec_ring_frames[slot]) (void)hipEventSynchronize(h->spec_counters_copied[slot]), spec_poll(h, false);
    ri.spec_enabled = h->spec_enabled && !h->corr.on();
    if (!ri.spec_enabled) b.route = gorder::choose_order_route(ri);
}

static int fill_flag_rows(gorder_hip_handle *h, Batch &b) {
    if (!b.leaflets) return GORDER_OK;
    const bool spec = b.route.speculative;
    if (spec) std::fill(b.arow.begin(), b.arow.end(), 0u);
    const size_t rows = (b.ltable ? b.replay.expand.size() : b.aframes.size()) + 1;
    ST_TRY(ensure_flag_rows(h, rows, rows + rows / 4, true));
    ST_TRY(upload_if_changed(h, h->d_arow, h->up_arow, h->up_arow_valid, b.arow));
    if (h->collect & GORDER_COLLECT_LEAFLETS)
        for (uint32_t f : b.aframes) b.collect_frames.push_back(b.frame_index[f]);
    if (spec) b.spec_aframes = b.aframes;
    else if (b.ltable) BATCH_TRY(replay_flag_rows(h, b.replay));
    else BATCH_TRY(run_leaflets(h, b.d_xyz, b.d_box, b.aframes, 1));
    h->have_assignment = true;
    h->assignment_frame = b.last_assign_frame;
    b.n_new_rows = spec ? 0 : (b.ltable ? b.replay.expand.size() : b.aframes.size());
    return GORDER_OK;
}

static int grow_frame_rows(gorder_hip_handle *h, const Batch &b) {
    if (!h->extra.tw || h->n_frames + b.n_frames <= h->tw_cap) return GORDER_OK;
    const size_t row = 3 * (size_t)h->plan.n_acc;
    const uint64_t ncap = (h->n_frames + b.n_frames) * 2;
    DBuf<u64> ns, nc;
    ST_TRY(allocate(h, ns, ncap * row));
    ST_TRY(allocate(h, nc, ncap * row));
    HIP_TRY(h, hipMemsetAsync(ns, 0, ncap * row * sizeof(u64), h->stream));
    HIP_TRY(h, hipMemsetAsync(nc, 0, ncap * row * sizeof(u64), h->stream));
    if (h->d_tw_sums) {
        HIP_TRY(h, hipMemcpyAsync(ns, h->d_tw_sums, h->n_frames * row * sizeof(u64), hipMemcpyDeviceToDevice, h->stream));
        HIP_TRY(h, hipMemcpyAsync(nc, h->d_tw_cnts, h->n_frames * row * sizeof(u64), hipMemcpyDeviceToDevice, h->stream));
        HIP_TRY(h, hipStreamSynchronize(h->stream));
    }
    h->d_tw_sums.swap(ns); h->d_tw_cnts.swap(nc); h->tw_cap = ncap;
    return GORDER_OK;
}

static int set_batch_normals(gorder_hip_handle *h, Batch &b) {
    const Plan &p = h->plan;
    FrameArgs &a = b.a;
    a.xyz = b.d_xyz; a.box9 = b.d_box; a.n_atoms = p.n_atoms; a.n_frames = b.n_frames;
    a.pbc = b.pbc ? 1 : 0;
    a.nx = h->tables.normal[0]; a.ny = h->tables.normal[1]; a.nz = h->tables.normal[2]; a.n2 = h->n2; a.n2sq = h->n2sq;
    a.leaflets = b.leaflets ? 1 : 0; a.aflags = h->d_aflags; a.arow = h->d_arow; a.n_mol_total = p.n_mol_total;
    a.acc = h->d_acc; a.rep = h->d_rep; a.n_rep = h->n_rep; a.n_acc = p.n_acc; a.err = h->d_err;
    h->manual_active = false;
    if (h->manual_frames) {
        const size_t n4 = (size_t)b.n_frames * p.n_mol_total;
        BATCH_TRY(ensure(h, h->d_dyn_normals, n4));
        if (hipStreamSynchronize(h->stream) != hipSuccess ||
            hipMemcpy(h->d_dyn_normals, h->manual_normals.data(), n4 * 4 * sizeof(float), hipMemcpyHostToDevice) != hipSuccess)
            return b.abort_batch(h, fail(h, GORDER_ERR_DEVICE, "manual normals: copy to the device failed"));
        h->manual_active = true;
        h->manual_frames = 0;
    } else if (h->d_ntable) {
        BATCH_TRY(replay_normal_rows(h, b.normal_rows));
        h->manual_active = true;
    }
    return GORDER_OK;
}

static int run_batch_orders(gorder_hip_handle *h, Batch &b) {
    const Plan &p = h->plan;
    FrameArgs &a = b.a;
    if (b.route.speculative) {
        BATCH_TRY(ensure(h, h->d_mom, (size_t)b.n_frames * p.tiles.size()));
        BATCH_TRY(ensure(h, h->d_head_z, (size_t)b.n_frames * p.n_mol_total));
        a.own = h->d_own; a.mom = h->d_mom; a.mom_dim = (int)h->tables.leaflets.normal_dim;
        a.own_head_begin = h->d_own_head_begin; a.own_heads = h->d_own_heads; a.head_z = h->d_head_z;
    }
    h->extra.touched = nullptr;
    if ((h->collect & GORDER_COLLECT_NORMALS) && h->extra.geom_kind && !p.tiles.empty() && p.ua_tiles.empty()) {
        const size_t nt = (size_t)b.n_frames * p.n_mol_total;
        BATCH_TRY(ensure(h, h->d_touched, nt));
        if (hipMemsetAsync(h->d_touched, 0, nt, h->stream) != hipSuccess) return b.abort_batch(h, fail(h, GORDER_ERR_DEVICE, "collect: hipMemsetAsync"));
        h->extra.touched = h->d_touched;
    }
    h->mol_frame_index = b.frame_index;
    const int st = launch_orders(h, a, b.route);
    h->mol_frame_index = nullptr;
    h->manual_active = false;
    BATCH_TRY(st);
    h->rep_dirty = true;
    return GORDER_OK;
}

static int resolve_speculation(gorder_hip_handle *h, Batch &b) {
    if (!b.route.speculative) return GORDER_OK;
    const Plan &p = h->plan;
    const gorder_leaflets_t &lf = h->tables.leaflets;
    const uint32_t n_frames = b.n_frames;
    BATCH_TRY(ensure(h, h->d_spec_center, n_frames));
    BATCH_TRY(ensure(h, h->d_spec_ok, n_frames));
    uint32_t *cnt = h->d_spec_counters + 2u * (uint32_t)(h->spec_batches & 1u);
    uint32_t *cnt_next = h->d_spec_counters + 2u * (uint32_t)((h->spec_batches + 1u) & 1u);
    SpecArgs sa{};
    sa.xyz = b.d_xyz; sa.box9 = b.d_box; sa.n_atoms = p.n_atoms; sa.n_frames = n_frames; sa.n_tiles = (uint32_t)p.tiles.size();
    sa.n_mol_total = p.n_mol_total; sa.n_membrane = lf.n_membrane; sa.dim = lf.normal_dim; sa.flip = lf.flip ? 1 : 0;
    sa.pbc = b.pbc ? 1 : 0; sa.mom = h->d_mom; sa.head_z = h->d_head_z; sa.center = h->d_spec_center; sa.ok = h->d_spec_ok;
    sa.aflags = h->d_aflags; sa.adist = h->d_adist; sa.counters = cnt; sa.counters_next = cnt_next;
    const uint32_t ring_slot = (uint32_t)(h->spec_batches % gorder_hip_handle::kSpecRing);
    sa.host_counters = h->h_spec_counters + 2u * ring_slot; sa.err = h->d_err;
    (void)timing_mark(h, "k_spec_check + k_spec_fixup");
    hipLaunchKernelGGL(k_spec_check, dim3(std::min<uint32_t>(n_frames, 2048u)), dim3(256), 0, h->stream, sa);
    BATCH_TRY(run_leaflets(h, b.d_xyz, b.d_box, b.spec_aframes, 1, h->d_spec_ok));
    (void)timing_mark(h, "k_spec_check + k_spec_fixup");
    const uint32_t fix_grid = (uint32_t)std::min<uint64_t>(((uint64_t)n_frames * p.n_mol_total + 63u) / 64u, 4096u);
    with_bool(b.route.fixup_ac, [&](auto AC) { with_bool(b.route.fixup_tw, [&](auto TW) {
        if constexpr (!AC() || !TW())
            hipLaunchKernelGGL((k_spec_fixup<AC(), TW()>), dim3(fix_grid), dim3(64), 0, h->stream, b.a, sa, h->d_spec_mol_begin,
                               h->d_spec_samples, TW() ? h->d_tw_sums : nullptr, TW() ? h->d_tw_cnts : nullptr,
                               TW() ? (uint64_t)h->n_frames : (uint64_t)0);
    }); });
    hipLaunchKernelGGL(k_spec_finish, dim3(1), dim3(256), 0, h->stream, sa);
    HIP_TRY(h, hipGetLastError());
    HIP_TRY(h, hipEventRecord(h->spec_counters_copied[ring_slot], h->stream));
    h->spec_ring_frames[ring_slot] = n_frames;
    h->spec_batches++;
    return GORDER_OK;
}

static int collect_batch(gorder_hip_handle *h, const Batch &b) {
    BATCH_TRY(collect_flag_rows(h, 1, b.collect_frames));
    if (b.ltable && (h->collect & GORDER_COLLECT_LEAFLETS)) {
        const gorder::ReplayLeafletBatch &replay = b.replay;
        for (size_t k = 0; k < replay.collect_rows.size();) {
            size_t e = k + 1;
            while (e < replay.collect_rows.size() && replay.collect_rows[e] == replay.collect_rows[e - 1] + 1u) e++;
            const std::vector<uint64_t> run(replay.collect_frames.begin() + k, replay.collect_frames.begin() + e);
            BATCH_TRY(collect_flag_rows(h, replay.collect_rows[k], run));
            k = e;
        }
    }
    if ((h->collect & GORDER_COLLECT_NORMALS) && h->plan.n_mol_total && !h->d_ntable)
        BATCH_TRY(collect_normal_rows(h, b.frame_index, b.n_frames, h->extra.touched));
    return GORDER_OK;
}

static int close_batch(gorder_hip_handle *h, const Batch &b) {
    const Plan &p = h->plan;
    const uint64_t *frame_index = b.frame_index;
    const uint32_t n_frames = b.n_frames;
    if (b.n_new_rows) {
        HIP_TRY(h, hipMemcpyAsync(h->d_aflags, h->d_aflags + b.n_new_rows * (size_t)p.n_mol_total, p.n_mol_total,
                                  hipMemcpyDeviceToDevice, h->stream));
    }
    if (b.ltable) { h->replay_have_carry = b.replay.have_carry; h->replay_carry_index = b.replay.carry_index; }
    gorder_hip_handle::BatchLog rec{h->n_submits, frame_index[0], n_frames > 1 ? frame_index[1] - frame_index[0] : 0, {}};
    for (uint32_t f = 1; f < n_frames; f++)
        if (frame_index[f] != rec.first + (uint64_t)f * rec.stride) { rec.list.assign(frame_index, frame_index + n_frames); break; }
    if (h->batch_log.size() >= gorder_hip_handle::kBatchLog) h->batch_log.pop_front();
    h->batch_log.push_back(std::move(rec));
    if (b.ri.mol_rows) {
        if (h->mol_batch_log.size() >= gorder_hip_handle::kBatchLog) h->mol_batch_log.pop_front();
        h->mol_batch_log.push_back({h->n_submits, b.mol_rows_before});
    }
    TIMING_MARK(h, "k_batch_end");
    hipLaunchKernelGGL(k_batch_end, dim3(b.pbc ? std::min<uint32_t>((n_frames + 255u) / 256u, 256u) : 1u), dim3(256), 0, h->stream,
                       b.pbc ? b.d_box : nullptr, n_frames, h->d_err,
                       h->d_acc + 4 * (size_t)p.n_acc, (unsigned long long)h->n_submits, h->decoder_key);
    HIP_TRY(h, hipGetLastError());
    TIMING_MARK(h, nullptr);
    if (h->timing_on) h->timing_launches++;
    h->n_submits++;
    h->n_frames += n_frames;
    if (h->corr.on()) h->corr.seen += n_frames;
    return GORDER_OK;
}

int gorder_hip_submit_device(gorder_hip_handle *h, const float *d_xyz, const float *d_box,
                             const uint64_t *frame_index, uint32_t n_frames) {
    if (!h || !d_xyz || !frame_index) return GORDER_ERR_INVALID_ARGUMENT;
    Batch b{d_xyz, d_box, frame_index, n_frames};
    b.pbc = h->tables.handle_pbc != 0;
    b.leaflets = h->tables.leaflets.method != GORDER_LEAFLETS_NONE;
    if (b.pbc && !d_box) return fail(h, GORDER_ERR_INVALID_ARGUMENT, "box required when handle_pbc = 1");
    if (((uintptr_t)d_xyz & 15u) != 0) return fail(h, GORDER_ERR_INVALID_ARGUMENT, "d_xyz must be 16-byte aligned");
    if (n_frames == 0) return GORDER_OK;
    HIP_TRY(h, hipSetDevice(h->device));
    h->collect_locked = true;
    b.mol_rows_before = h->mol_store.n_rows();
    ST_TRY(check_batch(h, b));
    ST_TRY(plan_batch_rows(h, b));
    choose_batch_route(h, b);
    ST_TRY(fill_flag_rows(h, b));
    ST_TRY(grow_frame_rows(h, b));
    ST_TRY(set_batch_normals(h, b));
    ST_TRY(run_batch_orders(h, b));
    ST_TRY(resolve_speculation(h, b));
    if (h->corr.on()) BATCH_TRY(launch_bond_corr(h, b.a));
    ST_TRY(collect_batch(h, b));
    return close_batch(h, b);
}

int gorder_hip_submit_host(gorder_hip_handle *h, const float *xyz, const float *box, const uint64_t *frame_index,
                           uint32_t n_frames) {
    if (!h || !xyz || !frame_index) return GORDER_ERR_INVALID_ARGUMENT;
    if (n_frames == 0) return GORDER_OK;
    HIP_TRY(h, hipSetDevice(h->device));
    int st;
    const size_t nx = (size_t)n_frames * h->plan.n_atoms * 3u, nb = (size_t)n_frames * 9u;
    if (!h->copy_stream) {
        HIP_TRY(h, h->copy_stream.create());
        for (int k = 0; k < 2; k++) {
            HIP_TRY(h, h->stage_copied[k].create());
            HIP_TRY(h, h->stage_computed[k].create());
        }
    }
    const int b = h->stage_next;
    h->stage_next ^= 1;
    if (h->stage_used[b]) HIP_TRY(h, hipEventSynchronize(h->stage_computed[b]));
    if ((st = ensure(h, h->d_stage_xyz[b], nx)) != GORDER_OK) return st;
    HIP_TRY(h, hipMemcpyAsync(h->d_stage_xyz[b], xyz, nx * sizeof(float), hipMemcpyHostToDevice, h->copy_stream));
    if (box) {
        if ((st = ensure(h, h->d_stage_box[b], nb)) != GORDER_OK) return st;
        HIP_TRY(h, hipMemcpyAsync(h->d_stage_box[b], box, nb * sizeof(float), hipMemcpyHostToDevice, h->copy_stream));
    }
    HIP_TRY(h, hipEventRecord(h->stage_copied[b], h->copy_stream));
    HIP_TRY(h, hipStreamWaitEvent(h->stream, h->stage_copied[b], 0));
    st = gorder_hip_submit_device(h, h->d_stage_xyz[b], box ? h->d_stage_box[b] : nullptr, frame_index, n_frames);
    if (st != GORDER_OK) return st;
    HIP_TRY(h, hipEventRecord(h->stage_computed[b], h->stream));
    h->stage_used[b] = true;
    HIP_TRY(h, hipEventSynchronize(h->stage_copied[b]));
    return GORDER_OK;
}

int gorder_hip_prime_leaflets(gorder_hip_handle *h, const float *d_xyz, const float *d_box, uint64_t frame_index) {
    if (!h || !d_xyz) return GORDER_ERR_INVALID_ARGUMENT;
    const gorder_leaflets_t &lf = h->tables.leaflets;
    if (lf.method == GORDER_LEAFLETS_NONE || lf.method == GORDER_LEAFLETS_MANUAL) return GORDER_ERR_INVALID_ARGUMENT;
    if (h->tables.handle_pbc && !d_box) return fail(h, GORDER_ERR_INVALID_ARGUMENT, "box required when handle_pbc = 1");
    HIP_TRY(h, hipSetDevice(h->device));
    h->collect_locked = true;
    if (h->tables.handle_pbc) {
        hipLaunchKernelGGL(k_check_box, dim3(1), dim3(256), 0, h->stream, d_box, 1u, h->d_err);
        HIP_TRY(h, hipGetLastError());
    }
    ST_TRY(ensure_flag_rows(h, 2, 2, false));
    std::vector<uint32_t> aframes(1, 0);
    if (lf.method == GORDER_LEAFLETS_CLUSTERING) {
        if (frame_index != 0 && !h->cl_have_carry)
            return fail(h, GORDER_ERR_LEAFLETS_NOT_PRIMED, "clustering: prime frame 0 before a later assignment frame");
        h->cl_is0.assign(1, frame_index == 0 ? 1 : 0);
    }
    const int st = run_leaflets(h, d_xyz, d_box, aframes, 0);
    (void)timing_mark(h, nullptr);
    if (st != GORDER_OK) return st;
    h->have_assignment = true;
    h->assignment_frame = frame_index;
    return GORDER_OK;
}

int gorder_hip_set_manual_leaflets(gorder_hip_handle *h, const uint8_t *flags, uint64_t frame_index) {
    if (!h || !flags) return GORDER_ERR_INVALID_ARGUMENT;
    if (h->tables.leaflets.method != GORDER_LEAFLETS_MANUAL) return GORDER_ERR_INVALID_ARGUMENT;
    if (h->d_ltable) return fail(h, GORDER_ERR_INVALID_ARGUMENT, "gorder_hip_set_manual_leaflets: a manual leaflet table is set");
    HIP_TRY(h, hipSetDevice(h->device));
    const uint32_t n = h->plan.n_mol_total;
    std::vector<uint8_t> tmp(n);
    for (uint32_t i = 0; i < n; i++) tmp[i] = (uint8_t)((flags[i] & 1) ^ (h->tables.leaflets.flip ? 1 : 0));
    ST_TRY(ensure_flag_rows(h, 1, 2, false));
    HIP_TRY(h, hipStreamSynchronize(h->stream));
    HIP_TRY(h, hipMemcpy(h->d_aflags, tmp.data(), n, hipMemcpyHostToDevice));
    h->have_assignment = true;
    h->assignment_frame = frame_index;
    h->collect_locked = true;
    if (h->collect & GORDER_COLLECT_LEAFLETS) {
        const int st = collect_flag_rows(h, 0, std::vector<uint64_t>(1, frame_index));
        (void)timing_mark(h, nullptr);
// ... 1097 lines not shown
```

### gorder_amd/csrc/kernels_bonds.h

```cpp
#pragma once

namespace {

__device__ __forceinline__ int grid_index(float x, float lo, float bin, uint32_t n, bool core) {
    const float k = __builtin_roundf(core ? gm_div_core(x - lo, bin) : (x - lo) / bin);
    if (!(k >= 0.0f) || !(k < (float)n)) return -1;
    return (int)k;
}
__device__ __forceinline__ int grid_index_fast(float x, float lo, float inv_bin, uint32_t n) {
    const float k = __builtin_floorf(__builtin_fmaf(x - lo, inv_bin, 0.5f));
    if (!(k >= 0.0f) || !(k < (float)n)) return -1;
    return (int)k;
}
constexpr uint32_t kRecFrames = 4;
struct TiledMapOut {
    uint32_t plane;
    float x0, y0, binx, biny;
    uint32_t nx, ny;
    int bin_core;
    unsigned long long *words;
    unsigned long long *ticks;
};
__device__ __forceinline__ unsigned long long tick_sample_word(int tick, bool lower) {
    return ((unsigned long long)(lower ? 1u : 0u) << 32) | (unsigned long long)(uint32_t)tick;
}
__device__ __forceinline__ unsigned long long map_sample_word(const TiledMapOut &mo, float px, float py, float pz, int tick, bool lower) {
    float x, y;
    if (mo.plane == 0) { x = px; y = py; }
    else if (mo.plane == 1) { x = px; y = pz; }
    else { x = pz; y = py; }
    const int ix = grid_index(x, mo.x0, mo.binx, mo.nx, mo.bin_core != 0), iy = grid_index(y, mo.y0, mo.biny, mo.ny, mo.bin_core != 0);
    if (ix < 0 || iy < 0) return kMapNoSample;
    const uint32_t nt = mo.nx * mo.ny, t = (uint32_t)ix * mo.ny + (uint32_t)iy;
    return ((unsigned long long)((lower ? nt : 0u) + t) << 32) | (unsigned long long)(uint32_t)tick;
}

template <bool ACOS_COS>
__device__ __forceinline__ bool bond_sample(const FrameArgs &a, uint32_t f, float p1x, float p1y, float p1z,
                                            float p2x, float p2y, float p2z, uint32_t mol, SampleAcc &acc,
                                            int &bad, const TiledMapOut *mo = nullptr, unsigned long long *word = nullptr,
                                            unsigned long long *tick_word = nullptr) {
    float vx = p2x - p1x, vy = p2y - p1y, vz = p2z - p1z;
    if (a.pbc) {
        const float *b = a.box9 + 9 * (size_t)f;
        const float bx = b[0], by = b[4], bz = b[8];
        bool slow = false;
        const float rx = gm_min_image_step(vx, bx, slow);
        const float ry = gm_min_image_step(vy, by, slow);
        const float rz = gm_min_image_step(vz, bz, slow);
        if (__builtin_expect(slow, 0)) {
            vx = gm_min_image_loop(vx, bx, bad);
            vy = gm_min_image_loop(vy, by, bad);
            vz = gm_min_image_loop(vz, bz, bad);
        } else {
            vx = rx; vy = ry; vz = rz;
        }
    }
    const float sch = gm_calc_sch<ACOS_COS>(vx, vy, vz, a.nx, a.ny, a.nz, a.n2, a.n2sq);
    const long long tick = gm_tick(sch);
    acc.s_tot += tick;
    acc.n_tot += 1;
    bool lower = false;
    if (a.leaflets) {
        const uint8_t fl = a.aflags[(size_t)a.arow[f] * a.n_mol_total + mol];
        lower = fl != 0;
        if (fl == 0) {
            acc.s_up += tick;
            acc.n_up += 1;
        }
    }
    if (mo) {
        *word = mo->nx == 0u ? tick_sample_word((int)tick, lower)
                             : map_sample_word(*mo, p1x + vx / 2.0f, p1y + vy / 2.0f, p1z + vz / 2.0f, (int)tick, lower);
        if (tick_word) *tick_word = tick_sample_word((int)tick, lower);
    }
    return sch != sch;
}

#ifndef GORDER_COMPUTE_NF
#define GORDER_COMPUTE_NF 8
#endif
typedef float v4f __attribute__((ext_vector_type(4)));

template <int G, int NPF, bool ACOS_COS, bool PBC, bool LEAF, int AXIS = -1>
struct TiledStage {
    static constexpr uint32_t TPF = kBlock / G;

    template <bool TAIL>
    static __device__ __forceinline__ void load(const FrameArgs &a, const Tile &t, uint32_t f0, uint32_t f_end,
                                                uint32_t sk, uint32_t si, v4f (&pre)[NPF]) {
        const uint32_t f = f0 + sk;
        if (TAIL && f >= f_end) return;
        const size_t base = ((size_t)f * a.n_atoms + t.atom0) * 3u;
        const uint32_t n4 = ((uint32_t)(base & 3u) + 3u * t.n_window + 3u) >> 2;
        const v4f *src = reinterpret_cast<const v4f *>(a.xyz + (base & ~(size_t)3));
#pragma unroll
        for (int j = 0; j < NPF; j++) {
            const uint32_t i = si + (uint32_t)j * TPF;
            pre[j] = __builtin_nontemporal_load(src + (i < n4 ? i : n4 - 1u));
        }
    }
    template <bool TAIL, bool FINITE = false>
    static __device__ __forceinline__ bool store(const FrameArgs &a, const Tile &t, uint32_t f0, uint32_t f_end,
                                                 uint32_t sk, uint32_t si, const v4f (&pre)[NPF], float *lds,
                                                 uint32_t lw) {
        const uint32_t f = f0 + sk;
        if (TAIL && f >= f_end) return true;
        const size_t base = ((size_t)f * a.n_atoms + t.atom0) * 3u;
        const uint32_t n4 = ((uint32_t)(base & 3u) + 3u * t.n_window + 3u) >> 2;
        const v4f *src = reinterpret_cast<const v4f *>(a.xyz + (base & ~(size_t)3));
        v4f *dst = reinterpret_cast<v4f *>(lds + (size_t)sk * lw);
        typedef float v2f __attribute__((ext_vector_type(2)));
        v2f poison = {0.0f, 0.0f};
        const v2f zero2 = {0.0f, 0.0f};
#pragma unroll
        for (int j = 0; j < NPF; j++) {
            const uint32_t i = si + (uint32_t)j * TPF;
            if (i < n4) dst[i] = pre[j];
            if (FINITE) {
                poison = __builtin_elementwise_fma(pre[j].xy, zero2, poison);
                poison = __builtin_elementwise_fma(pre[j].zw, zero2, poison);
            }
        }
        for (uint32_t i = si + (uint32_t)NPF * TPF; i < n4; i += TPF) {
            const v4f v = __builtin_nontemporal_load(src + i);
            dst[i] = v;
            if (FINITE) {
                poison = __builtin_elementwise_fma(v.xy, zero2, poison);
                poison = __builtin_elementwise_fma(v.zw, zero2, poison);
            }
        }
        return poison.x + poison.y == 0.0f;
    }
    template <int NF, int OUT = 0>
    static __device__ __forceinline__ void compute_core(const FrameArgs &a, const Tile &t, const Item &it,
                                                        uint32_t f0, const float (&P)[NF][6], SampleAcc &acc,
                                                        int &bad, uint32_t &nan_which, uint32_t &nan_frame,
                                                        const TiledMapOut *mo = nullptr, uint32_t k0 = 0) {
        constexpr bool MAPS = OUT != 0;
        int tick[NF];
        uint8_t fl[NF];
        float bx[NF], by[NF], bz[NF];
        uint32_t rare = 0;
        auto stage_word = [&](int k, float vx, float vy, float vz) {
            mo->words[k0 + (uint32_t)k] = OUT == 2
                ? tick_sample_word(tick[k], LEAF && fl[k] != 0)
                : map_sample_word(*mo, P[k][0] + vx / 2.0f, P[k][1] + vy / 2.0f, P[k][2] + vz / 2.0f, tick[k], LEAF && fl[k] != 0);
            if (OUT == 3) mo->ticks[k0 + (uint32_t)k] = tick_sample_word(tick[k], LEAF && fl[k] != 0);
        };
#pragma unroll
        for (int k = 0; k < NF; k++) {
            if (PBC) {
                const float *b = a.box9 + 9 * (size_t)(f0 + k);
                bx[k] = b[0]; by[k] = b[4]; bz[k] = b[8];
            }
            if (LEAF) fl[k] = a.aflags[(size_t)a.arow[f0 + k] * a.n_mol_total + it.mol];
        }
#pragma unroll
        for (int k = 0; k < NF; k++) {
            float vx = P[k][3] - P[k][0], vy = P[k][4] - P[k][1], vz = P[k][5] - P[k][2];
            bool slow = false;
            if (PBC && AXIS >= 0 && !ACOS_COS && !MAPS) {
                const float ax = __builtin_fabsf(vx), ay = __builtin_fabsf(vy), az = __builtin_fabsf(vz);
                const float tx = bx[k] - ax, ty = by[k] - ay, tz = bz[k] - az;
                vx = ax > bx[k] / 2.0f ? tx : ax;
                vy = ay > by[k] / 2.0f ? ty : ay;
                vz = az > bz[k] / 2.0f ? tz : az;
                slow = __builtin_fminf(__builtin_fminf(tx, ty), tz) < 0.0f;
            } else if (PBC) {
                vx = gm_min_image_step(vx, bx[k], slow);
                vy = gm_min_image_step(vy, by[k], slow);
                vz = gm_min_image_step(vz, bz[k], slow);
            }
            if (AXIS >= 0 && !ACOS_COS) {
                const float sch = gm_sch_axis<AXIS>(vx, vy, vz, slow);
                rare |= (slow ? 1u : 0u) << k;
                tick[k] = gm_tick_finite(sch);
            } else if (AXIS >= 0) {
                const float sch = gm_sch_axis_acos<AXIS>(vx, vy, vz, slow);
                rare |= (slow ? 1u : 0u) << k;
                tick[k] = gm_tick_finite(sch);
            } else {
                bool nonfinite = false;
                const float sch = gm_calc_sch<ACOS_COS, AXIS>(vx, vy, vz, a.nx, a.ny, a.nz, a.n2, a.n2sq, &nonfinite);
                rare |= ((slow || nonfinite || sch != sch) ? 1u : 0u) << k;
                tick[k] = gm_tick(sch);
            }
            if (MAPS) stage_word(k, vx, vy, vz);
        }
        if (__builtin_expect(rare != 0, 0)) {
#pragma unroll
            for (int k = 0; k < NF; k++) {
                if (!((rare >> k) & 1u)) continue;
                float vx = P[k][3] - P[k][0], vy = P[k][4] - P[k][1], vz = P[k][5] - P[k][2];
                if (PBC) {
                    vx = gm_min_image_loop(vx, bx[k], bad);
                    vy = gm_min_image_loop(vy, by[k], bad);
                    vz = gm_min_image_loop(vz, bz[k], bad);
                }
                const float sch = gm_calc_sch<ACOS_COS>(vx, vy, vz, a.nx, a.ny, a.nz, a.n2, a.n2sq);
                tick[k] = gm_tick(sch);
                if (MAPS) stage_word(k, vx, vy, vz);
                if (sch != sch && nan_frame == kNoNan) note_undefined(P[k][0], P[k][3], f0 + k, nan_which, nan_frame);
            }
        }
        int st = 0, su = 0;
        uint32_t nu = 0;
#pragma unroll
        for (int k = 0; k < NF; k++) {
            st += tick[k];
            if (LEAF) {
                su += fl[k] == 0 ? tick[k] : 0;
                nu += fl[k] == 0 ? 1u : 0u;
            }
        }
        acc.s_tot += st;
        acc.n_tot += NF;
        acc.s_up += su;
        acc.n_up += nu;
    }
    template <int OUT = 0>
    static __device__ __forceinline__ void compute(const FrameArgs &a, const Tile &t, const Item &it, uint32_t f0,
                                                   const float *lds, uint32_t lw, SampleAcc &acc, int &bad,
                                                   uint32_t &nan_which, uint32_t &nan_frame, const TiledMapOut *mo = nullptr) {
        constexpr int NF = (OUT == 1 || OUT == 3 || (OUT == 2 && LEAF)) ? 2 : (GORDER_COMPUTE_NF < G ? GORDER_COMPUTE_NF : G);
#pragma unroll
        for (int h = 0; h < G; h += NF) {
            float P[NF][6];
#pragma unroll
            for (int k = 0; k < NF; k++) {
                const uint32_t sh = (uint32_t)((((size_t)(f0 + h + k) * a.n_atoms + t.atom0) * 3u) & 3u);
                const float *w = lds + (size_t)(h + k) * lw + sh;
                P[k][0] = w[3u * it.li]; P[k][1] = w[3u * it.li + 1]; P[k][2] = w[3u * it.li + 2];
                P[k][3] = w[3u * it.lj]; P[k][4] = w[3u * it.lj + 1]; P[k][5] = w[3u * it.lj + 2];
            }
            compute_core<NF, OUT>(a, t, it, f0 + h, P, acc, bad, nan_which, nan_frame, mo, (uint32_t)h);
        }
    }
    template <int OUT = 0>
    static __device__ __forceinline__ void compute_tail(const FrameArgs &a, const Tile &t, const Item &it,
                                                        uint32_t f0, uint32_t f_end, const float *lds, uint32_t lw,
                                                        SampleAcc &acc, int &bad, uint32_t &nan_which,
                                                        uint32_t &nan_frame, const TiledMapOut *mo = nullptr) {
        if (OUT != 0) {
#pragma unroll
            for (int k = 0; k < G; k++) {
                const uint32_t f = f0 + (uint32_t)k;
                if (f >= f_end) continue;
                const uint32_t sh = (uint32_t)((((size_t)f * a.n_atoms + t.atom0) * 3u) & 3u);
                const float *w = lds + (size_t)k * lw + sh;
                const float p1x = w[3u * it.li], p1y = w[3u * it.li + 1], p1z = w[3u * it.li + 2];
                const float p2x = w[3u * it.lj], p2y = w[3u * it.lj + 1], p2z = w[3u * it.lj + 2];
                if (bond_sample<ACOS_COS>(a, f, p1x, p1y, p1z, p2x, p2y, p2z, it.mol, acc, bad, mo, mo->words + k, OUT == 3 ? mo->ticks + k : nullptr) &&
                    nan_frame == kNoNan)
                    note_undefined(p1x, p2x, f, nan_which, nan_frame);
            }
            return;
        }
#pragma unroll 1
        for (uint32_t f = f0; f < f_end; f++) {
            const uint32_t sh = (uint32_t)((((size_t)f * a.n_atoms + t.atom0) * 3u) & 3u);
            const float *w = lds + (size_t)(f - f0) * lw + sh;
            const float p1x = w[3u * it.li], p1y = w[3u * it.li + 1], p1z = w[3u * it.li + 2];
            const float p2x = w[3u * it.lj], p2y = w[3u * it.lj + 1], p2z = w[3u * it.lj + 2];
            if (bond_sample<ACOS_COS>(a, f, p1x, p1y, p1z, p2x, p2y, p2z, it.mol, acc, bad) && nan_frame == kNoNan)
                note_undefined(p1x, p2x, f, nan_which, nan_frame);
        }
    }
};

#ifndef GORDER_TILED_MIN_WAVES
#define GORDER_TILED_MIN_WAVES 4
#endif
__device__ __forceinline__ float mom_min(float x, float y) { float r; __asm__("v_min_f32_e32 %0, %1, %2" : "=v"(r) : "v"(x), "v"(y)); return r; }
__device__ __forceinline__ float mom_max(float x, float y) { float r; __asm__("v_max_f32_e32 %0, %1, %2" : "=v"(r) : "v"(x), "v"(y)); return r; }
#define GORDER_MOM_MINMAX_DPP(CTRL_TEXT)                                                                    \
    __asm__("s_nop 1\n\tv_min_f32_dpp %0, %0, %0 " CTRL_TEXT "\n\tv_max_f32_dpp %1, %1, %1 " CTRL_TEXT : "+v"(mn), "+v"(mx))
__device__ __forceinline__ void tiled_moments(const FrameArgs &a, const Tile &t, uint2 own, uint32_t tile_id, uint32_t n_tiles,
                                              uint32_t f, const float *slot, bool finite, uint2 my_head) {
    const uint32_t lane = threadIdx.x & 63u;
    const uint32_t sh = (uint32_t)((((size_t)f * a.n_atoms + t.atom0) * 3u) & 3u);
    const float *w = slot + sh + a.mom_dim + 3u * (own.x - t.atom0);
    const uint32_t n_own = own.y - own.x;
    float s = 0.0f, q = 0.0f, mn = 3.0e38f, mx = -3.0e38f;
    for (uint32_t i0 = 0; i0 < n_own; i0 += 512u) {
        float z[8];
#pragma unroll
        for (uint32_t u = 0; u < 8u; u++) z[u] = w[3u * min(i0 + 64u * u + lane, n_own - 1u)];
#pragma unroll
        for (uint32_t u = 0; u < 8u; u++) {
            if (i0 + 64u * u >= n_own) break;
            float d = z[u];
            if (i0 + 64u * u + 64u > n_own) d = i0 + 64u * u + lane < n_own ? d : 0.0f;
            s += d;
            q = __builtin_fmaf(d, d, q);
            mn = mom_min(mn, z[u]);
            mx = mom_max(mx, z[u]);
        }
    }
#define GORDER_MOM_STEP(CTRL, MASK, CTRL_TEXT)                                                  \
    s += dpp_or_zero<CTRL, MASK>(s); q += dpp_or_zero<CTRL, MASK>(q);                               \
    GORDER_MOM_MINMAX_DPP(CTRL_TEXT);
    GORDER_MOM_STEP(0x111, 0xf, "row_shr:1 row_mask:0xf bank_mask:0xf")
    GORDER_MOM_STEP(0x112, 0xf, "row_shr:2 row_mask:0xf bank_mask:0xf")
    GORDER_MOM_STEP(0x114, 0xf, "row_shr:4 row_mask:0xf bank_mask:0xf")
    GORDER_MOM_STEP(0x118, 0xf, "row_shr:8 row_mask:0xf bank_mask:0xf")
    GORDER_MOM_STEP(0x142, 0xa, "row_bcast:15 row_mask:0xa bank_mask:0xf")
    GORDER_MOM_STEP(0x143, 0xc, "row_bcast:31 row_mask:0xc bank_mask:0xf")
#undef GORDER_MOM_STEP
    const bool all_finite = __all(finite);
    if (lane == 63u) a.mom[(size_t)f * n_tiles + tile_id] = make_float4(all_finite ? s : __builtin_nanf(""), q, mn, mx);
    if (my_head.y != 0xffffffffu) a.head_z[(size_t)f * a.n_mol_total + my_head.y] = slot[sh + a.mom_dim + 3u * my_head.x];
}
template <int G, int NPF, bool ACOS_COS, bool PBC, bool LEAF, int AXIS, bool MOM = false>
__global__ __launch_bounds__(kBlock, GORDER_TILED_MIN_WAVES) void k_bonds_tiled(FrameArgs a_in, const float *__restrict__ xyz,
                                                      const float *__restrict__ box9,
                                                      const uint8_t *__restrict__ aflags,
                                                      const uint32_t *__restrict__ arow,
                                                      const Tile *__restrict__ tiles,
                                                      const Item *__restrict__ items,
                                                      const uint32_t *__restrict__ tile_slots,
                                                      uint32_t n_tiles, uint32_t lw) {
    extern __shared__ __attribute__((aligned(16))) float lds[];
    using S = TiledStage<G, NPF, ACOS_COS, PBC, LEAF, AXIS>;
    FrameArgs a = a_in;
    a.xyz = xyz; a.box9 = box9; a.aflags = aflags; a.arow = arow;
    const TileCtx tc = tile_prologue(tiles, items, n_tiles, 0u, a.frames_per_chunk, a.n_frames);
    const auto &[t, it, tile_id, chunk, tid, active, f_begin, f_end] = tc;
    const uint32_t sk = tid / S::TPF, si = tid % S::TPF;
    const uint32_t f_full = f_begin + ((f_end - f_begin) / G) * G;

    SampleAcc acc;
    int bad = 0;
    uint32_t nan_which = 0, nan_frame = kNoNan;
    v4f pre[NPF];
    uint2 own = make_uint2(0u, 0u), my_head = make_uint2(0u, 0xffffffffu);
    if (MOM) {
        own = a.own[tile_id];
        const uint32_t hq = a.own_head_begin[tile_id] + (tid & 63u);
        if (hq < a.own_head_begin[tile_id + 1u]) my_head = a.own_heads[hq];
    }

    if (f_begin < f_full) S::template load<false>(a, t, f_begin, f_end, sk, si, pre);
    for (uint32_t f0 = f_begin; f0 < f_full; f0 += G) {
        const bool finite = S::template store<false, MOM>(a, t, f0, f_end, sk, si, pre, lds, lw);
        __syncthreads();
        if (f0 + G < f_full) S::template load<false>(a, t, f0 + G, f_end, sk, si, pre);
        if (MOM) {
            static_assert(!MOM || (uint32_t)G * 64u == kBlock, "a wave per frame slot");
            tiled_moments(a, t, own, tile_id, n_tiles, f0 + sk, lds + (size_t)sk * lw, finite, my_head);
        }
        if (active) S::compute(a, t, it, f0, lds, lw, acc, bad, nan_which, nan_frame);
        __syncthreads();
    }
    if (f_full < f_end) {
        S::template load<true>(a, t, f_full, f_end, sk, si, pre);
        const bool finite = S::template store<true, MOM>(a, t, f_full, f_end, sk, si, pre, lds, lw);
        __syncthreads();
        if (MOM && f_full + sk < f_end) tiled_moments(a, t, own, tile_id, n_tiles, f_full + sk, lds + (size_t)sk * lw, finite, my_head);
        if (active) S::compute_tail(a, t, it, f_full, f_end, lds, lw, acc, bad, nan_which, nan_frame);
        __syncthreads();
    }

    raise_tile_errors(a.err, tc, tile_slots, nan_which, nan_frame, bad);
    fold_tile_sums(a.rep, a.n_rep, a.n_acc, tc, acc, lds, [&] { return tile_slots[tc.t.slot0 + tc.tid]; });
}

template <int G, bool ACOS_COS, bool PBC, bool LEAF>
__global__ __launch_bounds__(kBlock) void k_bonds_gather(FrameArgs a_in, const float *__restrict__ xyz,
                                                       const float *__restrict__ box9,
                                                       const uint8_t *__restrict__ aflags,
                                                       const uint32_t *__restrict__ arow,
                                                       const Tile *__restrict__ tiles,
                                                       const Item *__restrict__ items,
                                                       const uint32_t *__restrict__ tile_slots, uint32_t n_tiles) {
    __shared__ unsigned long long l_s[2 * kBlock];
    __shared__ uint32_t l_n[2 * kBlock];
    using S = TiledStage<G, 1, ACOS_COS, PBC, LEAF>;
    FrameArgs a = a_in;
    a.xyz = xyz; a.box9 = box9; a.aflags = aflags; a.arow = arow;
    const TileCtx tc = tile_prologue(tiles, items, n_tiles, 0u, a.frames_per_chunk, a.n_frames);
    const auto &[t, it, tile_id, chunk, tid, active, f_begin, f_end] = tc;
    const uint32_t f_full = f_begin + ((f_end - f_begin) / G) * G;
    const size_t fstride = (size_t)a.n_atoms * 3u;
    const float *pi = xyz + ((size_t)t.atom0 + it.li) * 3u;
    const float *pj = xyz + ((size_t)t.atom0 + it.lj) * 3u;

    SampleAcc acc;
    int bad = 0;
    uint32_t nan_which = 0, nan_frame = kNoNan;
    float cur[G][6], nxt[G][6];
    auto fetch = [&](float (&P)[G][6], uint32_t f0) {
#pragma unroll
        for (int k = 0; k < G; k++) {
            const float *q1 = pi + (size_t)(f0 + k) * fstride, *q2 = pj + (size_t)(f0 + k) * fstride;
            P[k][0] = q1[0]; P[k][1] = q1[1]; P[k][2] = q1[2];
            P[k][3] = q2[0]; P[k][4] = q2[1]; P[k][5] = q2[2];
        }
    };
    if (active) {
        if (f_begin < f_full) fetch(cur, f_begin);
        for (uint32_t f0 = f_begin; f0 < f_full; f0 += G) {
            const bool more = f0 + G < f_full;
            if (more) fetch(nxt, f0 + G);
            S::template compute_core<G>(a, t, it, f0, cur, acc, bad, nan_which, nan_frame);
            if (more) {
// ... 51 lines not shown
```

### gorder_amd/csrc/kernels_extras.h

```cpp
#pragma once

namespace {

struct ExtraArgs {
    int maps;
    uint32_t plane;
    float x0, y0, binx, biny;
    uint32_t nx, ny;
    unsigned long long *map_packed;
    unsigned long long *map_rec;
    const uint32_t *item_run;
    uint32_t rec_frame0, rec_stride;
    const float4 *dyn;
    int bin_core;
    float inv_binx, inv_biny;
    int axis;
    int tw;
    unsigned long long *tw_sums;
    unsigned long long *tw_cnts;
    unsigned long long tw_row0;
    float sin_tet, cos_tet, sin_ch3, cos_ch3, sin_half, cos_half;
    int geom_kind, geom_invert, geom_orient;
    float geom_thr;
    const float *shapes;
// ... 72 lines not shown
                                                uint32_t n_slots, uint32_t f, int *l_tw, uint32_t *l_twn,
                                                uint32_t lstride) {
    for (uint32_t ls = threadIdx.x; ls < n_slots; ls += blockDim.x) {
        const size_t row = ((size_t)e.tw_row0 + f) * 3u * a.n_acc;
        for (uint32_t w = 0; w < 2; w++) {
            const uint32_t n = l_twn[w * lstride + ls];
            if (n) {
                atomicAdd(&e.tw_sums[row + (size_t)w * a.n_acc + slots[ls]],
                          (unsigned long long)(long long)l_tw[w * lstride + ls]);
                atomicAdd(&e.tw_cnts[row + (size_t)w * a.n_acc + slots[ls]], (unsigned long long)n);
            }
            l_tw[w * lstride + ls] = 0;
            l_twn[w * lstride + ls] = 0;
        }
    }
}


__device__ __forceinline__ void rec_store(const ExtraArgs &e, uint32_t tile_id, uint32_t f_first, uint32_t tid,
                                          const unsigned long long (&v)[kRecFrames]) {
    static_assert(kRecFrames == 4, "a thread's four words");
    typedef unsigned long long ull2 __attribute__((ext_vector_type(2)));
    ull2 *row = reinterpret_cast<ull2 *>(e.map_rec + (size_t)tile_id * kBlock * e.rec_stride +
                                         (size_t)((f_first - e.rec_frame0) / kRecFrames) * (kRecFrames * kBlock) + (size_t)tid * kRecFrames);
    __builtin_nontemporal_store(ull2{v[0], v[1]}, row);
    __builtin_nontemporal_store(ull2{v[2], v[3]}, row + 1);
}
__device__ __forceinline__ TiledMapOut tiled_map_out(const ExtraArgs &e, unsigned long long *words) {
    TiledMapOut mo{};
    mo.plane = e.plane; mo.x0 = e.x0; mo.y0 = e.y0; mo.binx = e.binx; mo.biny = e.biny; mo.nx = e.nx; mo.ny = e.ny;
    mo.bin_core = e.bin_core; mo.words = words;
    return mo;
}

template <bool ACOS_COS, bool MAPS_ONLY>
__global__ __launch_bounds__(kBlock) void k_bonds_extras(FrameArgs a_in, ExtraArgs e, const float *__restrict__ xyz,
                                                          const float *__restrict__ box9,
                                                          const uint8_t *__restrict__ aflags,
                                                          const uint32_t *__restrict__ arow,
                                                          const Tile *__restrict__ tiles,
                                                          const Item *__restrict__ items,
                                                          const uint32_t *__restrict__ tile_slots, uint32_t n_tiles) {
    __shared__ unsigned long long l_s[2 * kBlock];
    __shared__ uint32_t l_n[2 * kBlock];
    __shared__ int l_tw[MAPS_ONLY ? 1 : 3 * kBlock];
    __shared__ uint32_t l_twn[MAPS_ONLY ? 1 : 3 * kBlock];
    FrameArgs a = a_in;
    a.xyz = xyz; a.box9 = box9; a.aflags = aflags; a.arow = arow;
    const uint32_t tile_id = blockIdx.x % n_tiles, chunk = blockIdx.x / n_tiles;
    const Tile t = tiles[tile_id];
    const uint32_t tid = threadIdx.x;
    const bool active = tid < t.n_items;
    Item it{0, 0, 0, 0, 0};
    if (active) it = items[t.item0 + tid];
    const uint32_t gslot = active ? tile_slots[t.slot0 + it.lslot] : 0;
    const uint32_t f_begin = a.frame0 + chunk * a.frames_per_chunk;
    const uint32_t f_end = min(a.n_frames, f_begin + a.frames_per_chunk);
    const TileCtx tc{t, it, tile_id, chunk, tid, active, f_begin, f_end};
    const size_t fstride = (size_t)a.n_atoms * 3u;
    const float *pi = xyz + ((size_t)t.atom0 + it.li) * 3u;
    const float *pj = xyz + ((size_t)t.atom0 + it.lj) * 3u;
    if (!MAPS_ONLY)
        for (uint32_t k = tid; k < 3 * kBlock; k += kBlock) { l_tw[k] = 0; l_twn[k] = 0; }
    __syncthreads();
    SampleAcc acc;
    unsigned long long recs[kRecFrames] = {kMapNoSample, kMapNoSample, kMapNoSample, kMapNoSample};
    int bad = 0;
    constexpr uint32_t kAhead = 2;
    float nx1[kAhead][3], nx2[kAhead][3];
#pragma unroll
    for (uint32_t u = 0; u < kAhead; u++) {
        const uint32_t fu = min(f_begin + u, a.n_frames - 1u);
#pragma unroll
        for (int d = 0; d < 3; d++) { nx1[u][d] = pi[(size_t)fu * fstride + d]; nx2[u][d] = pj[(size_t)fu * fstride + d]; }
    }
    for (uint32_t f = f_begin; f < f_end; f++) {
        unsigned long long rec = kMapNoSample;
        const float p1x = nx1[0][0], p1y = nx1[0][1], p1z = nx1[0][2];
        const float p2x = nx2[0][0], p2y = nx2[0][1], p2z = nx2[0][2];
#pragma unroll
        for (uint32_t u = 0; u + 1 < kAhead; u++)
#pragma unroll
            for (int d = 0; d < 3; d++) { nx1[u][d] = nx1[u + 1][d]; nx2[u][d] = nx2[u + 1][d]; }
        {
            const uint32_t fu = min(f + kAhead, a.n_frames - 1u);
#pragma unroll
            for (int d = 0; d < 3; d++) {
                nx1[kAhead - 1][d] = pi[(size_t)fu * fstride + d];
                nx2[kAhead - 1][d] = pj[(size_t)fu * fstride + d];
            }
        }
        if (active) {
            float vx = p2x - p1x, vy = p2y - p1y, vz = p2z - p1z;
            if (a.pbc) {
                const float *b = a.box9 + 9 * (size_t)f;
                vx = gm_min_image(vx, b[0], bad);
                vy = gm_min_image(vy, b[4], bad);
                vz = gm_min_image(vz, b[8], bad);
            }
            if (p1x != p1x) raise_error(a.err, GORDER_ERR_UNDEFINED_POSITION, f, kStageTypes, gslot, 1, it.mol, 0);
            else if (p2x != p2x) raise_error(a.err, GORDER_ERR_UNDEFINED_POSITION, f, kStageTypes, gslot, 1, it.mol, 1);
            const float mx = p1x + vx / 2.0f, my = p1y + vy / 2.0f, mz = p1z + vz / 2.0f;
            bool in = true;
            if (!MAPS_ONLY && e.geom_kind) {
                float box[3] = {1.0f, 1.0f, 1.0f};
                if (a.pbc) { const float *b = a.box9 + 9 * (size_t)f; box[0] = b[0]; box[1] = b[4]; box[2] = b[8]; }
                in = geom_inside(e, e.shapes + 8 * (size_t)f, mx, my, mz, box, a.pbc != 0, bad);
            }
            if (in) {
                float sch;
                if (!MAPS_ONLY && e.dyn) {
                    const float4 n = e.dyn[(size_t)f * a.n_mol_total + it.mol];
                    if (e.touched) e.touched[(size_t)f * a.n_mol_total + it.mol] = 1;
                    if (n.w < 3.0f) raise_error(a.err, GORDER_ERR_DYNAMIC_NORMAL, f, kStageTypes, gslot, 1, it.mol, (uint32_t)n.w);
                    const float n2sq = (n.x * n.x + n.y * n.y) + n.z * n.z;
                    sch = gm_calc_sch<ACOS_COS>(vx, vy, vz, n.x, n.y, n.z, __builtin_sqrtf(n2sq), n2sq);
                } else if (!ACOS_COS && e.axis >= 0) {
                    bool rare = false;
                    sch = e.axis == 0 ? gm_sch_axis<0>(vx, vy, vz, rare) : (e.axis == 1 ? gm_sch_axis<1>(vx, vy, vz, rare) : gm_sch_axis<2>(vx, vy, vz, rare));
                    if (__builtin_expect(rare, 0)) sch = gm_calc_sch<ACOS_COS>(vx, vy, vz, a.nx, a.ny, a.nz, a.n2, a.n2sq);
                } else {
                    sch = gm_calc_sch<ACOS_COS>(vx, vy, vz, a.nx, a.ny, a.nz, a.n2, a.n2sq);
                }
                const int tick = gm_tick(sch);
                int leaflet = -1;
                if (a.leaflets) leaflet = a.aflags[(size_t)a.arow[f] * a.n_mol_total + it.mol] ? 1 : 0;
                acc.s_tot += tick;
                acc.n_tot += 1;
                if (leaflet == 0) { acc.s_up += tick; acc.n_up += 1; }
                extras_add<MAPS_ONLY>(a, e, gslot, it.lslot, tick, mx, my, mz, leaflet, l_tw, l_twn, kBlock,
                                      (MAPS_ONLY || e.map_rec) ? &rec : nullptr);
            }
        }
        if (MAPS_ONLY || e.map_rec) {
            const uint32_t c = (f - f_begin) % kRecFrames;
#pragma unroll
            for (uint32_t m = 0; m < kRecFrames; m++) recs[m] = m == c ? rec : recs[m];
            if (c == kRecFrames - 1 || f + 1 == f_end) {
                rec_store(e, tile_id, f - c, tid, recs);
#pragma unroll
                for (uint32_t m = 0; m < kRecFrames; m++) recs[m] = kMapNoSample;
            }
        }
        if (!MAPS_ONLY && e.tw) {
            __syncthreads();
            extras_flush_tw(a, e, tile_slots + t.slot0, t.n_slots, f, l_tw, l_twn, kBlock);
            __syncthreads();
        }
    }
    if (bad) raise_box_range(a.err, f_begin);
    fold_tile_sums(a.rep, a.n_rep, a.n_acc, tc, acc, l_s, l_n, [&] { return tile_slots[tc.t.slot0 + tc.tid]; });
}

template <int NPF, bool PBC, bool LEAF, int AXIS>
__global__ __launch_bounds__(kBlock, 4) void k_bonds_tiled_maps(FrameArgs a_in, ExtraArgs e, const float *__restrict__ xyz,
                                                               const float *__restrict__ box9, const uint8_t *__restrict__ aflags,
                                                               const uint32_t *__restrict__ arow, const Tile *__restrict__ tiles,
                                                               const Item *__restrict__ items, const uint32_t *__restrict__ tile_slots,
                                                               uint32_t n_tiles, uint32_t lw) {
    constexpr int G = (int)kRecFrames;
    extern __shared__ __attribute__((aligned(16))) float lds[];
    using S = TiledStage<G, NPF, false, PBC, LEAF, AXIS>;
    FrameArgs a = a_in;
    a.xyz = xyz; a.box9 = box9; a.aflags = aflags; a.arow = arow;
    const TileCtx tc = tile_prologue(tiles, items, n_tiles, a.frame0, a.frames_per_chunk, a.n_frames);
    const auto &[t, it, tile_id, chunk, tid, active, f_begin, f_end] = tc;
    const uint32_t sk = tid / S::TPF, si = tid % S::TPF;
    const uint32_t f_full = f_begin + ((f_end - f_begin) / G) * G;
    unsigned long long words[kRecFrames] = {kMapNoSample, kMapNoSample, kMapNoSample, kMapNoSample};
    const TiledMapOut mo = tiled_map_out(e, words);
    SampleAcc acc;
    int bad = 0;
    uint32_t nan_which = 0, nan_frame = kNoNan;
    v4f pre[NPF];
    if (f_begin < f_full) S::template load<false>(a, t, f_begin, f_end, sk, si, pre);
    for (uint32_t f0 = f_begin; f0 < f_full; f0 += G) {
        S::template store<false>(a, t, f0, f_end, sk, si, pre, lds, lw);
        __syncthreads();
        if (f0 + G < f_full) S::template load<false>(a, t, f0 + G, f_end, sk, si, pre);
        if (active) S::template compute<1>(a, t, it, f0, lds, lw, acc, bad, nan_which, nan_frame, &mo);
        rec_store(e, tile_id, f0, tid, words);
        __syncthreads();
    }
    if (f_full < f_end) {
        S::template load<true>(a, t, f_full, f_end, sk, si, pre);
        S::template store<true>(a, t, f_full, f_end, sk, si, pre, lds, lw);
        __syncthreads();
#pragma unroll
        for (uint32_t m = 0; m < kRecFrames; m++) words[m] = kMapNoSample;
        if (active) S::template compute_tail<1>(a, t, it, f_full, f_end, lds, lw, acc, bad, nan_which, nan_frame, &mo);
        rec_store(e, tile_id, f_full, tid, words);
        __syncthreads();
    }
    raise_tile_errors(a.err, tc, tile_slots, nan_which, nan_frame, bad);
    __syncthreads();
    fold_tile_sums(a.rep, a.n_rep, a.n_acc, tc, acc, lds, [&] { return tile_slots[tc.t.slot0 + tc.tid]; });
}

template <int NPF, bool PBC, bool LEAF, int AXIS, bool MAPS, bool MOM = false>
__global__ __launch_bounds__(kBlock, 4) void k_bonds_tiled_tw(FrameArgs a_in, ExtraArgs e, const float *__restrict__ xyz,
                                                             const float *__restrict__ box9, const uint8_t *__restrict__ aflags,
                                                             const uint32_t *__restrict__ arow, const Tile *__restrict__ tiles,
                                                             const Item *__restrict__ items, const uint32_t *__restrict__ tile_slots,
                                                             uint32_t n_tiles, uint32_t lw) {
    constexpr int G = (int)kRecFrames;
    extern __shared__ __attribute__((aligned(16))) float lds[];
    __shared__ int l_tick[kRecFrames][kBlock];
    __shared__ uint8_t l_side[kRecFrames][kBlock];
    __shared__ uint32_t l_slot_run[kBlock];
    __shared__ uint32_t l_slot_id[kBlock];
    using S = TiledStage<G, NPF, false, PBC, LEAF, AXIS>;
    FrameArgs a = a_in;
    a.xyz = xyz; a.box9 = box9; a.aflags = aflags; a.arow = arow;
    const uint32_t tile_id = blockIdx.x % n_tiles, chunk = blockIdx.x / n_tiles;
    const Tile t = tiles[tile_id];
    const uint32_t tid = threadIdx.x;
    const uint32_t sk = tid / S::TPF, si = tid % S::TPF;
    const bool active = tid < t.n_items;
    Item it{0, 0, 0, 0, 0};
    if (active) {
        it = items[t.item0 + tid];
        const uint32_t run = e.item_run[t.item0 + tid];
        if ((run >> 16) == tid) l_slot_run[it.lslot] = run;
    }
    const uint32_t f_begin = a.frame0 + chunk * a.frames_per_chunk;
    const uint32_t f_end = min(a.n_frames, f_begin + a.frames_per_chunk);
    const TileCtx tc{t, it, tile_id, chunk, tid, active, f_begin, f_end};
    unsigned long long words[kRecFrames], mwords[MAPS ? kRecFrames : 1];
    TiledMapOut mo{};
    if (MAPS) {
        mo = tiled_map_out(e, mwords);
        mo.ticks = words;
    } else {
        mo.nx = 0;
        mo.words = words;
    }
    SampleAcc acc;
    int bad = 0;
    uint32_t nan_which = 0, nan_frame = kNoNan;
    v4f pre[NPF];
    const uint32_t my_slot = tid < t.n_slots ? tile_slots[t.slot0 + tid] : 0u;
    l_slot_id[tid] = my_slot;
    uint2 own = make_uint2(0u, 0u), my_head = make_uint2(0u, 0xffffffffu);
    if (MOM) {
        own = a.own[tile_id];
        const uint32_t hq = a.own_head_begin[tile_id] + (tid & 63u);
        if (hq < a.own_head_begin[tile_id + 1u]) my_head = a.own_heads[hq];
    }
    if (f_begin + G <= f_end) S::template load<false>(a, t, f_begin, f_end, sk, si, pre);
    for (uint32_t fs = f_begin; fs < f_end; fs += G) {
        const bool full = fs + G <= f_end;
        bool finite;
        if (full) {
            finite = S::template store<false, MOM>(a, t, fs, f_end, sk, si, pre, lds, lw);
        } else {
            S::template load<true>(a, t, fs, f_end, sk, si, pre);
            finite = S::template store<true, MOM>(a, t, fs, f_end, sk, si, pre, lds, lw);
        }
        __syncthreads();
        if (full && fs + 2u * G <= f_end) S::template load<false>(a, t, fs + G, f_end, sk, si, pre);
        if (MOM && fs + sk < f_end) {
            static_assert(!MOM || (uint32_t)G * 64u == kBlock, "a wave per frame slot");
            tiled_moments(a, t, own, tile_id, n_tiles, fs + sk, lds + (size_t)sk * lw, finite, my_head);
        }
#pragma unroll
        for (uint32_t k = 0; k < kRecFrames; k++) { words[k] = kMapNoSample; if (MAPS) mwords[k] = kMapNoSample; }
        if (active) {
            if (full) S::template compute<MAPS ? 3 : 2>(a, t, it, fs, lds, lw, acc, bad, nan_which, nan_frame, &mo);
            else S::template compute_tail<MAPS ? 3 : 2>(a, t, it, fs, f_end, lds, lw, acc, bad, nan_which, nan_frame, &mo);
        }
        if constexpr (MAPS) rec_store(e, tile_id, fs, tid, mwords);
#pragma unroll
        for (uint32_t k = 0; k < kRecFrames; k++) {
            l_tick[k][tid] = (int)(uint32_t)words[k];
            l_side[k][tid] = words[k] == kMapNoSample ? (uint8_t)2 : (uint8_t)(words[k] >> 32);
        }
        __syncthreads();
        for (uint32_t w = tid; w < kRecFrames * t.n_slots; w += kBlock) {
            const uint32_t k = w % kRecFrames, ls = w / kRecFrames;
            if (fs + k >= f_end) continue;
            const uint32_t run = l_slot_run[ls], tid0 = run >> 16, n = run & 0xffffu;
            int s_all = 0, s_low = 0;
            uint32_t n_all = 0, n_low = 0;
            for (uint32_t j = 0; j < n; j++) {
                const uint32_t side = l_side[k][tid0 + j];
                const int tick = l_tick[k][tid0 + j];
                if (side == 2u) continue;
                s_all += tick; n_all += 1u;
                if (side == 1u) { s_low += tick; n_low += 1u; }
            }
            if (!n_all) continue;
            const uint32_t slot = l_slot_id[ls];
            const size_t row = ((size_t)e.tw_row0 + fs + k) * 3u * a.n_acc;
            atomicAdd(&e.tw_sums[row + slot], (unsigned long long)(long long)s_all);
            atomicAdd(&e.tw_cnts[row + slot], (unsigned long long)n_all);
            if (LEAF) {
                const uint32_t n_up = n_all - n_low;
                if (n_up) {
                    atomicAdd(&e.tw_sums[row + (size_t)a.n_acc + slot], (unsigned long long)(long long)(s_all - s_low));
                    atomicAdd(&e.tw_cnts[row + (size_t)a.n_acc + slot], (unsigned long long)n_up);
                }
            }
        }
    }
    __syncthreads();
    raise_tile_errors(a.err, tc, tile_slots, nan_which, nan_frame, bad);
    fold_tile_sums(a.rep, a.n_rep, a.n_acc, tc, acc, lds, [&] { return my_slot; });
}

constexpr uint32_t kMapRunBatch = 1024;
__global__ __launch_bounds__(1024) void k_map_accumulate(const unsigned long long *__restrict__ rec,
                                                         const gorder::MapRun *__restrict__ runs,
                                                         const uint32_t *__restrict__ run_begin, uint32_t n_slots,
                                                         uint32_t rec_frames, uint32_t rec_stride,
                                                         uint32_t frames_per_chunk, uint32_t k_max,
                                                         uint32_t n_words , uint32_t n_tiles_map,
                                                         unsigned long long *__restrict__ map_packed, uint32_t n_acc) {
    extern __shared__ unsigned long long l_map[];
    typedef unsigned long long ull2 __attribute__((ext_vector_type(2)));
    const uint32_t slot = blockIdx.x % n_slots, chunk = blockIdx.x / n_slots;
    const uint32_t r0 = run_begin[slot], r1 = run_begin[slot + 1];
    if (r0 == r1) return;
    const uint32_t f0 = chunk * frames_per_chunk, f1 = min(rec_frames, f0 + frames_per_chunk);
    for (uint32_t w = threadIdx.x; w < n_words; w += blockDim.x) l_map[w] = 0ull;
    __syncthreads();
    auto add = [&](unsigned long long v) {
        if (v != kMapNoSample) atomicAdd(&l_map[(uint32_t)(v >> 32)], kMapOne + (unsigned long long)(long long)(int)(uint32_t)v);
    };
    if (k_max == 1u) {
        __shared__ uint32_t l_pref[kMapRunBatch + 1];
        const uint32_t fb0 = f0 / kRecFrames, fb1 = (f1 + kRecFrames - 1) / kRecFrames;
        for (uint32_t rb = r0; rb < r1; rb += kMapRunBatch) {
            const uint32_t nr = min(kMapRunBatch, r1 - rb);
            for (uint32_t i = threadIdx.x; i < nr; i += blockDim.x) l_pref[i + 1u] = runs[rb + i].n;
            if (threadIdx.x == 0) l_pref[0] = 0;
            __syncthreads();
            if (threadIdx.x < 64u) {
                uint32_t carry = 0;
                for (uint32_t i0 = 1; i0 <= nr; i0 += 64u) {
                    const uint32_t i = i0 + threadIdx.x, v = i <= nr ? l_pref[i] : 0u;
                    const uint32_t incl = wave_scan_shfl(v, threadIdx.x);
                    if (i <= nr) l_pref[i] = carry + incl;
                    carry += __shfl(incl, 63, 64);
                }
            }
            __syncthreads();
            const uint32_t total = l_pref[nr];
            const uint32_t parts = total ? max(1u, min(blockDim.x / total, fb1 - fb0)) : 1u;
            const uint32_t fb_per = (fb1 - fb0 + parts - 1u) / parts;
            for (uint32_t lane_item = threadIdx.x; lane_item < total * parts; lane_item += blockDim.x) {
                const uint32_t item = lane_item % total, part = lane_item / total;
                const uint32_t fb_lo = fb0 + part * fb_per, fb_hi = min(fb1, fb_lo + fb_per);
                uint32_t lo = 0, hi = nr;
                while (hi - lo > 1u) {
                    const uint32_t mid = (lo + hi) >> 1;
                    if (l_pref[mid] <= item) lo = mid; else hi = mid;
                }
                const gorder::MapRun run = runs[rb + lo];
                const unsigned long long *base = rec + (size_t)run.tile * kBlock * rec_stride + kRecFrames * (run.tid0 + (item - l_pref[lo]));
                uint32_t cur = 0;
                unsigned long long sum = 0ull;
                ull2 wa, wb, na, nb;
                auto fetch = [&](uint32_t fb, ull2 &a2, ull2 &b2) {
                    const ull2 *p = reinterpret_cast<const ull2 *>(base + (size_t)fb * (kRecFrames * kBlock));
                    a2 = __builtin_nontemporal_load(p);
                    b2 = __builtin_nontemporal_load(p + 1);
                };
                if (fb_lo < fb_hi) fetch(fb_lo, na, nb);
                for (uint32_t fb = fb_lo; fb < fb_hi; fb++) {
                    wa = na; wb = nb;
                    if (fb + 1u < fb_hi) fetch(fb + 1u, na, nb);
                    const unsigned long long w[4] = {wa.x, wa.y, wb.x, wb.y};
#pragma unroll
                    for (uint32_t m = 0; m < 4u; m++) {
                        if (w[m] == kMapNoSample) continue;
                        const uint32_t pt = (uint32_t)(w[m] >> 32);
                        if (sum != 0ull && pt != cur) { atomicAdd(&l_map[cur], sum); sum = 0ull; }
                        cur = pt;
                        sum += kMapOne + (unsigned long long)(long long)(int)(uint32_t)w[m];
                    }
                }
                if (sum != 0ull) atomicAdd(&l_map[cur], sum);
            }
            __syncthreads();
        }
    } else {
        const uint32_t n_waves = blockDim.x >> 6;
        const bool per_wave = r1 - r0 >= n_waves;
        const uint32_t r_first = r0 + (per_wave ? threadIdx.x >> 6 : 0u), r_step = per_wave ? n_waves : 1u;
        const uint32_t i_first = per_wave ? threadIdx.x & 63u : threadIdx.x, i_step = per_wave ? 64u : blockDim.x;
        for (uint32_t r = r_first; r < r1; r += r_step) {
            const gorder::MapRun run = runs[r];
            const uint32_t total = (f1 - f0) * run.n;
            const unsigned long long *piece = rec + (((size_t)run.tile * k_max + run.k) * kBlock + run.tid0) * rec_stride + (size_t)f0 * run.n;
            for (uint32_t i = i_first; i < total / 2u; i += i_step) {
                const ull2 w = __builtin_nontemporal_load(reinterpret_cast<const ull2 *>(piece) + i);
                add(w.x);
                add(w.y);
            }
            if ((total & 1u) && i_first == 0u) add(piece[total - 1u]);
        }
    }
    __syncthreads();
    for (uint32_t w = threadIdx.x; w < n_words; w += blockDim.x) {
        const unsigned long long v = l_map[w];
        if (!v) continue;
        const uint32_t plane = w / n_tiles_map, t = w % n_tiles_map;
        atomicAdd(&map_packed[((size_t)plane * n_acc + slot) * n_tiles_map + t], v);
    }
}

}
```

### gorder_amd/csrc/kernels_leaflets.h

```cpp
#pragma once

namespace {

struct LeafletArgs {
    const float *xyz;
    const float *box9;
    uint32_t n_atoms;
    const uint32_t *aframes;
    uint32_t row0;
    uint8_t *aflags;
    float *adist;
    uint32_t n_mol_total;
    const uint32_t *heads;
    const uint32_t *membrane;
    uint32_t n_membrane;
    const uint32_t *methyl_begin;
    const uint32_t *methyl_atoms;
    uint32_t dim;
    int flip, pbc;
    uint32_t *err;
    const uint8_t *skip;
    uint32_t n_assign;
};

// ... 199 lines not shown
    if (a.pbc) L = a.box9[9 * (size_t)f + 4 * dn];
    int bad = 0;
    const size_t start = (size_t)f * a.n_atoms * 3u;
    const uint32_t sh = (uint32_t)(start & 3u), n_float = 3u * a.n_atoms;
    const uint32_t n4 = (sh + n_float + 3u) >> 2;
    const v4f *src = reinterpret_cast<const v4f *>(a.xyz + (start - sh));
    const float *x = a.xyz + start;
    const bool pbc = a.pbc != 0;
    const float inv = pbc ? 1.0f / L : 0.0f;
    const float zref = a.n_mol_total ? x[3u * (size_t)a.heads[0] + dn] : 0.0f;
    uint32_t r = (dn + sh + 3u * 256u - threadIdx.x) % 3u;
    float nonfinite = 0.0f, sc = 0.0f, ss = 0.0f, su = 0.0f, ulo = 3.0e38f, uhi = -3.0e38f;
    auto take = [&](float z, bool ok) {
        z = ok ? z : zref;
        if (pbc) {
            bad |= (ok && !(z <= 9.0f * L && z >= -8.0f * L)) ? 1 : 0;
            float sn, cs;
            fast_sincos_rev(z * inv, &sn, &cs);
            sc += ok ? cs : 0.0f;
            ss += ok ? sn : 0.0f;
        }
        const float u = pbc ? gm_min_image(z - zref, L, bad) : z - zref;
        su += ok ? u : 0.0f;
        ulo = ok ? fminf(ulo, u) : ulo;
        uhi = ok ? fmaxf(uhi, u) : uhi;
    };
    auto chunk = [&](const v4f v, uint32_t c, uint32_t j0) {
        float za = v.x;
        za = j0 == 1 ? v.y : za;
        za = j0 == 2 ? v.z : za;
        const uint32_t e0 = 4u * c;
        if (e0 >= sh && e0 + 4u <= sh + n_float) {
            const float t = (v.x + v.y) + (v.z + v.w);
            nonfinite += t - t;
            take(za, true);
            take(v.w, j0 == 0);
        } else {
            const float e[4] = {v.x, v.y, v.z, v.w};
#pragma unroll
            for (uint32_t j = 0; j < 4; j++) {
                const bool in = e0 + j >= sh && e0 + j < sh + n_float;
                nonfinite += in ? e[j] - e[j] : 0.0f;
            }
            take(za, e0 + j0 >= sh && e0 + j0 < sh + n_float);
            take(v.w, j0 == 0 && e0 + 3u >= sh && e0 + 3u < sh + n_float);
        }
    };
    const uint32_t j1 = r == 0 ? 2u : r - 1u, j2 = j1 == 0 ? 2u : j1 - 1u;
    auto pick = [](const v4f v, uint32_t j0) {
        float z = v.x;
        z = j0 == 1 ? v.y : z;
        z = j0 == 2 ? v.z : z;
        return z;
    };
    auto group = [&](const v4f v0, const v4f v1, const v4f v2, uint32_t c0) {
        if (4u * c0 >= sh && 4u * (c0 + 512u) + 4u <= sh + n_float) {
            const float t = ((v0.x + v0.y) + (v0.z + v0.w)) + ((v1.x + v1.y) + (v1.z + v1.w)) + ((v2.x + v2.y) + (v2.z + v2.w));
            nonfinite += t - t;
            take(pick(v0, r), true);
            take(pick(v1, j1), true);
            take(pick(v2, j2), true);
            take(r == 0 ? v0.w : (r == 1 ? v1.w : v2.w), true);
        } else {
            chunk(v0, c0, r);
            chunk(v1, c0 + 256u, j1);
            chunk(v2, c0 + 512u, j2);
        }
    };
    uint32_t c = threadIdx.x;
    for (; c + 5u * 256u < n4; c += 6u * 256u) {
        v4f v[6];
#pragma unroll
        for (uint32_t k = 0; k < 6; k++) v[k] = __builtin_nontemporal_load(src + c + k * 256u);
        group(v[0], v[1], v[2], c);
        group(v[3], v[4], v[5], c + 3u * 256u);
    }
    for (; c + 2u * 256u < n4; c += 3u * 256u) {
        v4f v[3];
#pragma unroll
        for (uint32_t k = 0; k < 3; k++) v[k] = __builtin_nontemporal_load(src + c + k * 256u);
        group(v[0], v[1], v[2], c);
    }
    for (; c < n4; c += 256u) {
        chunk(__builtin_nontemporal_load(src + c), c, r);
        r = r == 0 ? 2u : r - 1u;
    }
    double cs2[2] = {(double)sc, (double)ss}, un[2] = {(double)su, (double)nonfinite};
    block_sum_n<2>(cs2, scratch);
    block_sum_n<2>(un, scratch);
    const double tc = cs2[0], ts = cs2[1], tu = un[0], nf = un[1];
    block_minmax(ulo, uhi, fscratch);
    float center;
    if (!pbc) {
        center = zref + (float)(tu / (double)a.n_atoms);
    } else {
        const float est = (atan2f(-(float)ts, -(float)tc) + 3.1415927f) / (6.2831855f / L);
        const float shift = gm_min_image(zref - est, L, bad);
        const float half = L / 2.0f, margin = 1e-4f * L;
        if (ulo + shift > -half + margin && uhi + shift < half - margin) {
            center = gm_wrap((est + shift) + (float)(tu / (double)a.n_atoms), L, bad);
        } else {
            float acc = 0.0f;
            uint32_t r2 = (dn + sh + 3u * 256u - threadIdx.x) % 3u;
            for (uint32_t c2 = threadIdx.x; c2 < n4; c2 += 256u) {
                const v4f v = src[c2];
                const uint32_t e0 = 4u * c2, j0 = r2;
                float za = v.x;
                za = j0 == 1 ? v.y : za;
                za = j0 == 2 ? v.z : za;
                if (e0 + j0 >= sh && e0 + j0 < sh + n_float) acc += gm_min_image(za - est, L, bad);
                if (j0 == 0 && e0 + 3u >= sh && e0 + 3u < sh + n_float) acc += gm_min_image(v.w - est, L, bad);
                r2 = r2 == 0 ? 2u : r2 - 1u;
            }
            const double tot = block_sum((double)acc, scratch);
            center = gm_wrap(est + (float)(tot / (double)a.n_atoms), L, bad);
        }
    }
    if (threadIdx.x == 0) {
        if (center != center || nf != 0.0 || a.n_atoms == 0) {
            raise_error(a.err, GORDER_ERR_INVALID_GLOBAL_MEMBRANE_CENTER, f, kStageSystem);
            center = __builtin_nanf("");
        }
        s_center = center;
    }
    __syncthreads();
    const float cdim = s_center;
    uint8_t *row = a.aflags + (size_t)(a.row0 + bi) * a.n_mol_total;
    const bool last = bi + 1 == a.n_assign;
    for (uint32_t m = threadIdx.x; m < a.n_mol_total; m += blockDim.x) {
        const float hp = x[3u * (size_t)a.heads[m] + dn];
        float d = hp - cdim;
        if (pbc) d = gm_min_image(d, L, bad);
        row[m] = (uint8_t)((d >= 0.0f ? 0 : 1) ^ (a.flip ? 1 : 0));
        if (last && a.adist) a.adist[m] = d;
    }
    if (bad) raise_box_range(a.err, f);
}
template <bool TURNS>
__global__ __launch_bounds__(256) void k_leaflets_global_contig(LeafletArgs a) {
    if (!TURNS) {
        leaflets_global_contig_frame(a, blockIdx.x);
        return;
    }
    for (uint32_t bi = blockIdx.x; bi < a.n_assign; bi += gridDim.x) {
        leaflets_global_contig_frame(a, bi);
        __syncthreads();
    }
}

struct SpecArgs {
    const float *xyz;
    const float *box9;
    uint32_t n_atoms, n_frames, n_tiles, n_mol_total, n_membrane;
    uint32_t dim;
    int flip, pbc;
    const float4 *mom;
    const float *head_z;
    float *center;
    uint8_t *ok;
    uint8_t *aflags;
    float *adist;
    uint32_t *counters;
    uint32_t *counters_next;
    uint32_t *host_counters;
    uint32_t *err;
};
__global__ __launch_bounds__(256) void k_spec_check(SpecArgs a) {
    __shared__ float s_center;
    __shared__ int s_ok;
    for (uint32_t f = blockIdx.x; f < a.n_frames; f += gridDim.x) {
        const float L = a.pbc ? a.box9[9 * (size_t)f + 4 * a.dim] : 0.0f;
        if (threadIdx.x < 64u) {
            double S = 0.0, Q = 0.0;
            float mn = 3.0e38f, mx = -3.0e38f;
            for (uint32_t t = threadIdx.x; t < a.n_tiles; t += 64u) {
                const float4 m = a.mom[(size_t)f * a.n_tiles + t];
                S += (double)m.x; Q += (double)m.y;
                mn = fminf(mn, m.z); mx = fmaxf(mx, m.w);
            }
            wave_sum2_minmax_bfly(S, Q, mn, mx);
            if (threadIdx.x == 0u) {
                const double n = (double)a.n_membrane, c = S / n;
                bool ok = (S - S == 0.0) && (Q - Q == 0.0) && mn <= mx;
                if (ok && a.pbc) {
                    const double k = 6.283185307179586 / (double)L;
                    const double var = fmax(Q - S * S / n, 0.0) + 1e-4 * Q + 1e-6 * n;
                    const double dmax = k * fmax((double)mx - c, c - (double)mn), S2 = k * k * var, den = n - 0.5 * S2;
                    ok = den > 0.0 && L > 0.0f;
                    if (ok) {
                        const double dist = (dmax * S2 / 6.0 / den) / k;
                        const double room = 0.5 * (double)L - 1e-4 * (double)L - dist;
                        ok = (double)mx - c < room && c - (double)mn < room;
                    }
                }
                a.center[f] = (float)c;
                a.ok[f] = ok ? 1 : 0;
                s_center = (float)c;
                s_ok = ok ? 1 : 0;
                if (!ok) atomicAdd(&a.counters[1], 1u);
            }
        }
        __syncthreads();
        if (s_ok) {
            const float c = s_center;
            const bool last = f + 1 == a.n_frames;
            int bad = 0;
            for (uint32_t m = threadIdx.x; m < a.n_mol_total; m += blockDim.x) {
                float d = a.head_z[(size_t)f * a.n_mol_total + m] - c;
                if (a.pbc) d = gm_min_image(d, L, bad);
                a.aflags[(size_t)(1u + f) * a.n_mol_total + m] = (uint8_t)((d >= 0.0f ? 0 : 1) ^ (a.flip ? 1 : 0));
                if (last && a.adist) a.adist[m] = d;
            }
            if (bad) raise_box_range(a.err, f);
        }
        __syncthreads();
    }
}
struct SpecSample { uint32_t i, j, slot; };
template <bool ACOS_COS, bool TW>
__global__ __launch_bounds__(64) void k_spec_fixup(FrameArgs a, SpecArgs sa, const uint32_t *__restrict__ mol_begin,
                                                   const SpecSample *__restrict__ samples, unsigned long long *tw_sums,
                                                   unsigned long long *tw_cnts, uint64_t tw_row0) {
    const uint64_t n_pairs = (uint64_t)sa.n_frames * sa.n_mol_total;
    uint32_t moved = 0;
    for (uint64_t p0 = (uint64_t)blockIdx.x * 64u; p0 < n_pairs; p0 += (uint64_t)gridDim.x * 64u) {
        const uint64_t pi = p0 + threadIdx.x;
        bool differs = false;
        uint32_t exact_l = 0;
        if (pi < n_pairs) {
            exact_l = sa.aflags[(size_t)sa.n_mol_total + pi];
            differs = exact_l != sa.aflags[pi % sa.n_mol_total];
        }
        unsigned long long todo = __ballot(differs);
        moved += (uint32_t)__popcll(todo);
        while (todo) {
            const int l = __ffsll((long long)todo) - 1;
            todo &= todo - 1ull;
            const uint64_t pj = p0 + (uint64_t)l;
            const uint32_t f = (uint32_t)(pj / sa.n_mol_total), m = (uint32_t)(pj - (uint64_t)f * sa.n_mol_total);
            const uint32_t exact = (uint32_t)__shfl((int)exact_l, l, 64);
            const float *x = a.xyz + (size_t)f * a.n_atoms * 3u;
            for (uint32_t q = mol_begin[m] + threadIdx.x; q < mol_begin[m + 1]; q += 64u) {
                const SpecSample sm = samples[q];
                SampleAcc acc;
                int bad = 0;
                const float *p1 = x + 3u * (size_t)sm.i, *p2 = x + 3u * (size_t)sm.j;
                bond_sample<ACOS_COS>(a, f, p1[0], p1[1], p1[2], p2[0], p2[1], p2[2], m, acc, bad);
                unsigned long long *rep = a.rep;
                if (exact == 0u) {
                    atomicAdd(&rep[(size_t)a.n_acc + sm.slot], (unsigned long long)acc.s_tot);
                    atomicAdd(&rep[3u * (size_t)a.n_acc + sm.slot], 1ull);
                } else {
                    atomicAdd(&rep[(size_t)a.n_acc + sm.slot], (unsigned long long)(-acc.s_tot));
                    atomicAdd(&rep[3u * (size_t)a.n_acc + sm.slot], ~0ull);
                }
                if (TW) {
                    const size_t up = (size_t)(tw_row0 + f) * 3u * a.n_acc + (size_t)a.n_acc + sm.slot;
                    atomicAdd(&tw_sums[up], (unsigned long long)(exact == 0u ? acc.s_tot : -acc.s_tot));
                    atomicAdd(&tw_cnts[up], exact == 0u ? 1ull : ~0ull);
                }
            }
        }
    }
    if (threadIdx.x == 0u && moved) atomicAdd(&sa.counters[0], moved);
}
__global__ __launch_bounds__(256) void k_spec_finish(SpecArgs sa) {
    for (uint32_t m = threadIdx.x; m < sa.n_mol_total; m += blockDim.x)
        sa.aflags[m] = sa.aflags[(size_t)sa.n_frames * sa.n_mol_total + m];
    if (threadIdx.x == 0u) {
        sa.host_counters[0] = sa.counters[0];
        sa.host_counters[1] = sa.counters[1];
        sa.counters_next[0] = 0u;
        sa.counters_next[1] = 0u;
    }
}

__global__ __launch_bounds__(256) void k_leaflets_individual(LeafletArgs a) {
    const uint32_t m = blockIdx.x * blockDim.x + threadIdx.x;
    if (m >= a.n_mol_total) return;
    const uint32_t f = a.aframes[blockIdx.y];
    const float *x = a.xyz + (size_t)f * a.n_atoms * 3u;
    float L = 1.0f;
    if (a.pbc) L = a.box9[9 * (size_t)f + 4 * a.dim];
    int bad = 0;
    const float hp = x[3u * (size_t)a.heads[m] + a.dim];
    float total = 0.0f;
    for (uint32_t k = a.methyl_begin[m]; k < a.methyl_begin[m + 1]; k++) {
        const float mp = x[3u * (size_t)a.methyl_atoms[k] + a.dim];
        const float d = hp - mp;
        total += a.pbc ? gm_min_image(d, L, bad) : d;
    }
    a.aflags[(size_t)(a.row0 + blockIdx.y) * a.n_mol_total + m] =
        (uint8_t)((total >= 0.0f ? 0 : 1) ^ (a.flip ? 1 : 0));
    if (blockIdx.y + 1 == gridDim.y && a.adist) a.adist[m] = total;
    if (bad) raise_box_range(a.err, f);
}

constexpr uint32_t kLocalMaxCells1D = 128;
constexpr uint32_t kLocalSlabMax = 2048;
inline uint32_t local_slab_frames(size_t n_membrane) {
    const size_t per_frame = n_membrane * (2u * 12u + 4u) + (size_t)(2 * 4u + 16u + 16u) * kLocalMaxCells1D * (kLocalMaxCells1D + 1u) + 32u;
    const size_t n = ((size_t)4096 << 20) / per_frame;
    uint32_t cap = kLocalSlabMax;
    if (const char *ev = getenv("GORDER_HIP_LOCAL_SLAB")) cap = (uint32_t)std::max(4, atoi(ev));
    return (uint32_t)(n < 4 ? 4 : (n > cap ? cap : n));
}

struct LocalRowPre { float sc, ss; double sz; };
struct alignas(16) LocalEdge { uint32_t q; float zm, sq; uint32_t cs; };
constexpr uint32_t kEdgeSpanMax = 2000;
__device__ __forceinline__ uint32_t local_edge_trig(float sc, float ss) {
    return ((uint32_t)(int)__builtin_rintf(sc * 16.0f) & 0xffffu) | ((uint32_t)(int)__builtin_rintf(ss * 16.0f) << 16);
}
__device__ __forceinline__ void local_edge_trig_diff(uint32_t hi, uint32_t lo, float &dc, float &ds) {
    dc = (float)(int16_t)((hi & 0xffffu) - (lo & 0xffffu)) * 0.0625f;
    ds = (float)(int16_t)((hi >> 16) - (lo >> 16)) * 0.0625f;
}
struct LocalRec { float x, y, z; };

struct LocalArgs {
    const float *xyz;
    const float *box9;
    uint32_t n_atoms;
    const uint32_t *aframes;
    uint32_t frame0;
    uint32_t n_slab;
    uint32_t row0;
    uint8_t *aflags;
    float *adist;
    int write_dist_frame;
    uint32_t n_mol_total;
    const uint32_t *heads;
    const uint32_t *mol_slot0;
    const uint32_t *membrane;
    uint32_t n_membrane;
    uint4 *grid;
    uint32_t dim;
    int flip, pbc;
    float radius;
    float radius_thr;
    uint32_t *cell_of;
    float *trig;
    uint32_t *cell_count;
    uint32_t *cell_fill;
    int halo;
    int prune;
    uint32_t rows_groups;
    uint32_t rec_stride;
    LocalEdge *edge;
    LocalRowPre *rowpre;
    float4 *finfo;
    uint2 *todo;
    int sums;
    uint32_t *summary;
    uint32_t *summary_host;
    uint32_t *need;
    uint32_t *err;
};

constexpr uint32_t kLocalFine = 4;
constexpr uint32_t kLocalFineRows = 7;
__device__ __forceinline__ void local_axis(float L, float radius, uint32_t &nc, uint32_t &k, uint32_t k_max = kLocalFine,
                                           uint32_t nc_max = kLocalMaxCells1D) {
    nc = 1; k = 0;
    for (uint32_t kk = k_max; kk >= 1u; kk--) {
        const float fine = floorf(L / (radius / (float)kk) * 0.9999f);
        if (fine >= (float)(2u * kk + 1u) && fine <= (float)nc_max) { nc = (uint32_t)fine; k = kk; return; }
    }
}
__device__ __forceinline__ void local_grid(const LocalArgs &a, const float *box, uint32_t &nca, uint32_t &ncb,
                                           int &da, int &db, uint32_t &ka, uint32_t &kb) {
    da = (int)((a.dim + 1u) % 3u);
    db = (int)((a.dim + 2u) % 3u);
    nca = ncb = 1;
    ka = kb = 0;
    if (a.pbc) {
        const uint32_t k_max = a.halo ? kLocalFineRows : kLocalFine;
        local_axis(box[da], a.radius, nca, ka, k_max);
// ... 1456 lines not shown
```

### gorder_amd/csrc/order_route.h

```cpp
#ifndef GORDER_ORDER_ROUTE_H
#define GORDER_ORDER_ROUTE_H
#include <stddef.h>
#include <stdint.h>
#include <algorithm>

namespace gorder {
constexpr uint32_t kStageFrames = 4;

struct OrderRouteIn {
    bool acos = false, pbc = false, leaflets = false; int axis = -1;
    bool maps = false, map_staged = false, tw = false, geom = false, dyn_or_manual = false;
    bool use_gather = false, item_run = false, bond_tiles = false, ua_tiles = false, direct_items = false, ua_fast_flag = false;
    int frames_per_stage = (int)kStageFrames; uint32_t max_window = 0;
    bool global_leaflets = false, spec_enabled = false, have_assignment = false, every_frame_assigns = false, manual_frames = false, normal_table = false;
    bool npf5 = false, tw_gather = false, maps_gather = false;
    bool shells = false;
    bool mol_rows = false;
    bool dist = false;
    bool classes = false;
    bool ua_samples_flag = false;
};
enum class UaKernel { None, Extras, Dist, Mol };
enum class BondFamily { None, Tiled, Gather, TiledTw, TiledMaps, Extras, Shells, TiledMol, Dist, Classes };

struct OrderRoute {
    BondFamily family = BondFamily::None;
    const char *label = nullptr;
    int npf = 4;
    bool mom = false, tw_maps = false;
    bool maps_only = false;
    bool items_by_slot = false;
    bool extras = false;
    int ua_mode = -1; bool ua_fast = false;
    bool map_accumulate = false, direct = false;
    bool speculative = false, fixup_ac = false, fixup_tw = false;
    UaKernel ua_kernel = UaKernel::None;
};

inline OrderRoute choose_order_route(const OrderRouteIn &in) {
    OrderRoute r;
    const bool staged = in.maps && in.map_staged;
    const bool rows_or_maps_only = !in.geom && !in.dyn_or_manual;
    const bool tiled_out = !in.acos && !in.use_gather && in.frames_per_stage == (int)kStageFrames;
    r.extras = in.maps || in.tw || in.geom || in.dyn_or_manual || in.dist || in.classes;
    r.maps_only = staged && !in.tw && rows_or_maps_only;
    r.npf = (3u * in.max_window + 6u) / 4u <= 4u * 64u && !in.npf5 ? 4 : 5;
    if (!in.bond_tiles) r.family = BondFamily::None;
    else if (in.mol_rows) r.family = BondFamily::TiledMol;
    else if (in.dist) r.family = BondFamily::Dist;
    else if (in.classes) r.family = BondFamily::Classes;
    else if (!r.extras) r.family = in.use_gather ? BondFamily::Gather : BondFamily::Tiled;
    else if (in.shells) r.family = BondFamily::Shells;
    else if (r.maps_only && tiled_out && !in.maps_gather) r.family = BondFamily::TiledMaps;
    else if (in.tw && (!in.maps || staged) && rows_or_maps_only && tiled_out && in.item_run && !in.tw_gather) r.family = BondFamily::TiledTw;
    else r.family = BondFamily::Extras;
    static const char *const labels[] = {nullptr, "k_bonds_tiled", "k_bonds_gather", "k_bonds_tiled_tw", "k_bonds_tiled_maps", "k_bonds_extras", "k_bonds_shells",
                                         "k_bonds_tiled_mol", "k_bonds_dist", "k_bonds_classes"};
    r.label = labels[(int)r.family];
    r.tw_maps = r.family == BondFamily::TiledTw && staged;
    r.items_by_slot = r.family == BondFamily::TiledTw || r.family == BondFamily::TiledMaps || (r.family == BondFamily::Extras && staged);
    r.ua_mode = !in.ua_tiles ? -1 : r.maps_only ? 1 : in.tw && !in.maps && rows_or_maps_only ? 3 : r.extras ? 2 : 0;
    r.ua_fast = in.ua_tiles && in.ua_fast_flag && !in.acos;
    r.ua_kernel = !in.ua_tiles ? UaKernel::None : in.ua_samples_flag && in.mol_rows ? UaKernel::Mol : in.ua_samples_flag && in.dist ? UaKernel::Dist : UaKernel::Extras;
    r.map_accumulate = staged; r.direct = in.direct_items;
    r.speculative = (r.family == BondFamily::Tiled || (r.family == BondFamily::TiledTw && !r.tw_maps)) && in.leaflets && in.global_leaflets &&
                    in.spec_enabled && in.have_assignment && in.every_frame_assigns && !in.manual_frames && !in.normal_table;
    r.mom = r.speculative;
    r.fixup_tw = in.tw; r.fixup_ac = in.acos && !in.tw;
    return r;
}

struct FrameChunks { uint32_t frames_per_chunk, n_chunks; };
inline uint32_t ceil_div(uint32_t a, uint32_t b) { return (a + b - 1) / b; }

inline FrameChunks tiled_chunks(uint32_t n_frames, uint32_t stage, uint32_t n_tiles, uint32_t wg_target, uint32_t wg_capacity) {
    const uint32_t n_stages = ceil_div(n_frames, stage);
    uint32_t n_chunks = std::max(1u, (wg_target ? wg_target : 12u * wg_capacity) / n_tiles);
    n_chunks = std::min(n_chunks, std::max(1u, n_stages / 4u));
    const uint32_t fpc = ceil_div(n_stages, n_chunks) * stage;
    return {fpc, ceil_div(n_frames, fpc)};
}

inline FrameChunks extras_chunks(uint32_t n_frames, uint32_t n_tiles, uint32_t wg_target, uint32_t wg_capacity, bool staged, bool whole_stages) {
    const uint32_t n_chunks = std::min(std::max(1u, (wg_target ? wg_target : 8u * wg_capacity) / n_tiles), n_frames);
    uint32_t fpc = ceil_div(n_frames, n_chunks);
    if (staged) fpc = ceil_div(fpc, 16u) * 16u;
    if (whole_stages) fpc = ceil_div(fpc, kStageFrames) * kStageFrames;
    return {fpc, ceil_div(n_frames, fpc)};
}

inline FrameChunks shells_chunks(uint32_t n_frames, uint32_t n_tiles, uint32_t wg_target, uint32_t wg_capacity, uint32_t max_chunk) {
    const FrameChunks c = extras_chunks(n_frames, n_tiles, wg_target, wg_capacity, false, false);
    if (c.frames_per_chunk <= max_chunk) return c;
    return {max_chunk, ceil_div(n_frames, max_chunk)};
}

constexpr uint32_t kDistSamplesPerWord = 8;
inline FrameChunks dist_chunks(uint32_t n_frames, uint32_t n_tiles, uint32_t wg_target, uint32_t wg_capacity, uint32_t table_words,
                               uint32_t samples_per_word, uint32_t max_chunk) {
    const FrameChunks c = extras_chunks(n_frames, n_tiles, wg_target, wg_capacity, false, false);
    const uint64_t floor_fpc = ((uint64_t)table_words * samples_per_word + 255u) / 256u;
    const uint32_t fpc = (uint32_t)std::min<uint64_t>(std::min<uint64_t>(std::max<uint64_t>(c.frames_per_chunk, floor_fpc), max_chunk), n_frames);
    return {fpc, ceil_div(n_frames, fpc)};
}

inline FrameChunks direct_chunks(uint32_t n_frames, uint32_t blocks_per_chunk, uint32_t wg_target) {
    const uint32_t n_chunks = std::min(std::max(1u, ceil_div(wg_target ? wg_target : 256u * 8u, blocks_per_chunk)), n_frames);
    const uint32_t fpc = ceil_div(n_frames, n_chunks);
    return {fpc, ceil_div(n_frames, fpc)};
}

inline FrameChunks map_chunks(uint32_t n_frames, uint32_t n_acc, uint32_t forced) {
    uint32_t n_chunks = forced ? forced : std::max(1u, 512u / std::max(1u, n_acc));
    n_chunks = std::min(n_chunks, std::max(1u, n_frames / 16u));
    const uint32_t fpc = ceil_div(ceil_div(n_frames, n_chunks), 16u) * 16u;
    return {fpc, ceil_div(n_frames, fpc)};
}


inline uint32_t map_subrange(uint32_t n_frames, bool maps, bool staged, uint64_t fold_limit, uint32_t max_mol, size_t words_per_frame) {
    uint32_t sub = maps ? (uint32_t)std::max<uint64_t>(1, (fold_limit - 1) / max_mol) : n_frames;
    if (staged) sub = std::min(std::min<uint32_t>(sub, (uint32_t)std::max<size_t>(1, ((size_t)1 << 27) / words_per_frame)), n_frames);
    return sub;
}

}
#endif
```

Baseline: 20.52 million.

## Speculate leaflet sides for ordermap route and apply them at map accumulation

Extends speculative leaflet assignment to the TiledMaps bond route. The tiled-maps kernel computes moments in the same pass and emits plane-agnostic map words. The leaflet side is then resolved per subrange and applied from aflags inside k_map_accumulate. The aim is to avoid a separate leaflet pass that reads the trajectory coordinates again, at the cost of extra spec check/fixup launches per subrange and side lookups in accumulation. It is gated on batch size (at least 128 MiB of coordinates) and on several other conditions.

After: 21.07 million (median of 3 runs). 1.03x the previous value.

```diff
diff --git a/gorder_amd/csrc/gorder_hip.hip b/gorder_amd/csrc/gorder_hip.hip
--- a/gorder_amd/csrc/gorder_hip.hip
+++ b/gorder_amd/csrc/gorder_hip.hip
@@ -10,6 +10,7 @@
 #include <new>
 #include <string>
 #include <deque>
+#include <functional>
 #include <type_traits>
 #include <vector>
 
@@ -252,6 +253,7 @@
     DBuf<uint32_t> d_spec_mol_begin;
     DBuf<SpecSample> d_spec_samples;
     uint64_t spec_batches = 0, spec_fixed = 0, spec_exact_frames = 0;
+    std::function<int(uint32_t, uint32_t)> resolve_subrange;
     DBuf<float> d_stage_xyz[2], d_stage_box[2];
     Event stage_copied[2], stage_computed[2];
     bool stage_used[2] = {false, false};
@@ -775,9 +777,11 @@
     const Item *items = bond_items(h, route);
     TIMING_MARK(h, route.label);
     with_npf(route.npf, [&](auto NPF) { with_bool(b.pbc, [&](auto PBC) { with_bool(b.leaflets, [&](auto LF) { with_axis(h->axis, [&](auto AX) {
-        if (route.family == gorder::BondFamily::TiledMaps)
-            hipLaunchKernelGGL((k_bonds_tiled_maps<NPF(), PBC(), LF(), AX()>), g, blk, h->lds_bytes, h->stream, b, e, b.xyz,
-                               b.box9, b.aflags, b.arow, h->d_tiles, items, h->d_tile_slots, nt, h->lw);
+        if (route.family == gorder::BondFamily::TiledMaps) with_bool(route.mom, [&](auto MOM) {
+            if constexpr (LF() || !MOM())
+                hipLaunchKernelGGL((k_bonds_tiled_maps<NPF(), PBC(), LF(), AX(), MOM()>), g, blk, h->lds_bytes, h->stream, b, e, b.xyz,
+                                   b.box9, b.aflags, b.arow, h->d_tiles, items, h->d_tile_slots, nt, h->lw);
+        });
         else with_bool(route.tw_maps, [&](auto MAPS) { with_bool(route.mom, [&](auto MOM) {
             if constexpr (!MOM() || (LF() && !MAPS()))
                 hipLaunchKernelGGL((k_bonds_tiled_tw<NPF(), PBC(), LF(), AX(), MAPS(), MOM()>), g, blk, h->lds_bytes, h->stream, b, e,
@@ -794,10 +798,14 @@
     const uint32_t ntm = h->map_nx * h->map_ny, n_words = planes * ntm;
     const char *ev = getenv("GORDER_HIP_MAP_CHUNKS");
     const gorder::FrameChunks m = gorder::map_chunks(s.nf(), n_acc, ev ? (uint32_t)std::max(1, atoi(ev)) : 0u);
+    const bool sides = s.route.sides_at_accumulation && per_item == 1u;
+    const MapSides sd{h->d_tiles, h->d_items_by_slot, s.a.aflags, s.a.n_mol_total, s.lo};
     TIMING_MARK(h, "k_map_accumulate");
-    hipLaunchKernelGGL(k_map_accumulate, dim3(n_acc * m.n_chunks), dim3(1024), n_words * sizeof(unsigned long long), h->stream,
-                       h->d_map_rec, runs, run_begin, n_acc, s.nf(), rec_stride, m.frames_per_chunk, per_item, n_words, ntm,
-                       h->d_map_packed, n_acc);
+    with_bool(sides, [&](auto SIDES) {
+        hipLaunchKernelGGL(k_map_accumulate<SIDES()>, dim3(n_acc * m.n_chunks), dim3(1024), n_words * sizeof(unsigned long long), h->stream,
+                           h->d_map_rec, runs, run_begin, n_acc, s.nf(), rec_stride, m.frames_per_chunk, per_item, n_words, ntm,
+                           h->d_map_packed, n_acc, sd);
+    });
     return GORDER_OK;
 }
 
@@ -811,6 +819,7 @@
     case BondFamily::Extras: ST_TRY(launch_extras(h, s, e)); break;
     default: ST_TRY(launch_tiled_out(h, s, e)); break;
     }
+    if (s.route.sides_at_accumulation) ST_TRY(h->resolve_subrange(s.lo, s.hi));
     if (s.route.map_accumulate) ST_TRY(launch_map_accumulate(h, s, e.rec_stride, h->d_runs, h->d_run_begin, 1u));
     HIP_TRY(h, hipGetLastError());
     return GORDER_OK;
@@ -1285,7 +1294,9 @@
         ST_TRY(upload(h, h->d_run_begin, p.run_begin));
         ST_TRY(upload(h, h->d_items_by_slot, p.items_by_slot));
         ST_TRY(upload(h, h->d_ua_item_run, p.ua_item_run));
-        HIP_TRY(h, hipFuncSetAttribute(reinterpret_cast<const void *>(k_map_accumulate),
+        HIP_TRY(h, hipFuncSetAttribute(reinterpret_cast<const void *>(k_map_accumulate<false>),
+                                       hipFuncAttributeMaxDynamicSharedMemorySize, (int)lds_bytes));
+        HIP_TRY(h, hipFuncSetAttribute(reinterpret_cast<const void *>(k_map_accumulate<true>),
                                        hipFuncAttributeMaxDynamicSharedMemorySize, (int)lds_bytes));
         h->map_staged = true;
     }
@@ -1990,7 +2001,8 @@
 }
 
 static int run_leaflets(gorder_hip_handle *h, const float *d_xyz, const float *d_box,
-                        const std::vector<uint32_t> &aframes, uint32_t row0, const uint8_t *skip = nullptr) {
+                        const std::vector<uint32_t> &aframes, uint32_t row0, const uint8_t *skip = nullptr,
+                        uint32_t first = 0, uint32_t last = 0xffffffffu) {
     if (aframes.empty()) return GORDER_OK;
     ST_TRY(upload_if_changed(h, h->d_aframes, h->up_aframes, h->up_aframes_valid, aframes));
     const gorder_leaflets_t &lf = h->tables.leaflets;
@@ -2004,6 +2016,10 @@
     la.err = h->d_err;
     la.skip = skip;
     la.n_assign = (uint32_t)aframes.size();
+    if (first != 0 || last < la.n_assign) {
+        la.aframes += first; la.row0 += first; la.n_assign = std::min(last, la.n_assign) - first;
+        if (last < (uint32_t)aframes.size()) la.adist = nullptr;
+    }
     switch (lf.method) {
     case GORDER_LEAFLETS_GLOBAL: ST_TRY(launch_global_leaflets(h, la)); break;
     case GORDER_LEAFLETS_INDIVIDUAL: ST_TRY(launch_individual_leaflets(h, la)); break;
@@ -2083,6 +2099,7 @@
     gorder::OrderRouteIn ri;
     gorder::OrderRoute route;
     FrameArgs a{};
+    SpecArgs sa{};
 
     int abort_batch(gorder_hip_handle *h, int status) const {
         h->mol_store.truncate(mol_rows_before);
@@ -2162,6 +2179,9 @@
     ri.ua_samples_flag = (h->tables.flags & GORDER_FLAG_UA_SAMPLES) != 0;
     ri.npf5 = env_flag("GORDER_HIP_NPF5"); ri.tw_gather = env_flag("GORDER_HIP_TW_GATHER"); ri.maps_gather = env_flag("GORDER_HIP_MAPS_GATHER");
     ri.every_frame_assigns = b.aframes.size() == b.n_frames;
+    const char *min_bytes = getenv("GORDER_HIP_SPECULATE_MAPS_MIN_BYTES");
+    ri.maps_one_read = !env_flag("GORDER_HIP_NO_SPECULATE_MAPS") &&
+                       gorder::maps_one_read_pays(b.n_frames, p.n_atoms, min_bytes ? strtoull(min_bytes, nullptr, 10) : gorder::kMapsOneReadMinBytes);
     b.route = gorder::choose_order_route(ri);
     if (!b.route.speculative) return;
     spec_poll(h, false);
@@ -2231,6 +2251,8 @@
     return GORDER_OK;
 }
 
+static int begin_speculation(gorder_hip_handle *h, Batch &b);
+static int resolve_frames(gorder_hip_handle *h, Batch &b, uint32_t lo, uint32_t hi);
 static int run_batch_orders(gorder_hip_handle *h, Batch &b) {
     const Plan &p = h->plan;
     FrameArgs &a = b.a;
@@ -2247,8 +2269,13 @@
         if (hipMemsetAsync(h->d_touched, 0, nt, h->stream) != hipSuccess) return b.abort_batch(h, fail(h, GORDER_ERR_DEVICE, "collect: hipMemsetAsync"));
         h->extra.touched = h->d_touched;
     }
+    if (b.route.sides_at_accumulation) {
+        BATCH_TRY(begin_speculation(h, b));
+        h->resolve_subrange = [h, &b](uint32_t lo, uint32_t hi) { return resolve_frames(h, b, lo, hi); };
+    }
     h->mol_frame_index = b.frame_index;
     const int st = launch_orders(h, a, b.route);
+    h->resolve_subrange = nullptr;
     h->mol_frame_index = nullptr;
     h->manual_active = false;
     BATCH_TRY(st);
@@ -2256,37 +2283,52 @@
     return GORDER_OK;
 }
 
-static int resolve_speculation(gorder_hip_handle *h, Batch &b) {
-    if (!b.route.speculative) return GORDER_OK;
+static int begin_speculation(gorder_hip_handle *h, Batch &b) {
     const Plan &p = h->plan;
     const gorder_leaflets_t &lf = h->tables.leaflets;
     const uint32_t n_frames = b.n_frames;
-    BATCH_TRY(ensure(h, h->d_spec_center, n_frames));
-    BATCH_TRY(ensure(h, h->d_spec_ok, n_frames));
+    ST_TRY(ensure(h, h->d_spec_center, n_frames));
+    ST_TRY(ensure(h, h->d_spec_ok, n_frames));
     uint32_t *cnt = h->d_spec_counters + 2u * (uint32_t)(h->spec_batches & 1u);
     uint32_t *cnt_next = h->d_spec_counters + 2u * (uint32_t)((h->spec_batches + 1u) & 1u);
-    SpecArgs sa{};
+    SpecArgs &sa = b.sa;
     sa.xyz = b.d_xyz; sa.box9 = b.d_box; sa.n_atoms = p.n_atoms; sa.n_frames = n_frames; sa.n_tiles = (uint32_t)p.tiles.size();
+    sa.f_lo = 0; sa.f_hi = n_frames;
     sa.n_mol_total = p.n_mol_total; sa.n_membrane = lf.n_membrane; sa.dim = lf.normal_dim; sa.flip = lf.flip ? 1 : 0;
     sa.pbc = b.pbc ? 1 : 0; sa.mom = h->d_mom; sa.head_z = h->d_head_z; sa.center = h->d_spec_center; sa.ok = h->d_spec_ok;
     sa.aflags = h->d_aflags; sa.adist = h->d_adist; sa.counters = cnt; sa.counters_next = cnt_next;
     const uint32_t ring_slot = (uint32_t)(h->spec_batches % gorder_hip_handle::kSpecRing);
     sa.host_counters = h->h_spec_counters + 2u * ring_slot; sa.err = h->d_err;
+    return GORDER_OK;
+}
+static int resolve_frames(gorder_hip_handle *h, Batch &b, uint32_t lo, uint32_t hi) {
+    const Plan &p = h->plan;
+    SpecArgs sa = b.sa;
+    sa.f_lo = lo; sa.f_hi = hi;
     (void)timing_mark(h, "k_spec_check + k_spec_fixup");
-    hipLaunchKernelGGL(k_spec_check, dim3(std::min<uint32_t>(n_frames, 2048u)), dim3(256), 0, h->stream, sa);
-    BATCH_TRY(run_leaflets(h, b.d_xyz, b.d_box, b.spec_aframes, 1, h->d_spec_ok));
+    hipLaunchKernelGGL(k_spec_check, dim3(std::min<uint32_t>(hi - lo, 2048u)), dim3(256), 0, h->stream, sa);
+    ST_TRY(run_leaflets(h, b.d_xyz, b.d_box, b.spec_aframes, 1, h->d_spec_ok, lo, hi));
     (void)timing_mark(h, "k_spec_check + k_spec_fixup");
-    const uint32_t fix_grid = (uint32_t)std::min<uint64_t>(((uint64_t)n_frames * p.n_mol_total + 63u) / 64u, 4096u);
+    const uint32_t fix_grid = (uint32_t)std::min<uint64_t>(((uint64_t)(hi - lo) * p.n_mol_total + 63u) / 64u, 4096u);
     with_bool(b.route.fixup_ac, [&](auto AC) { with_bool(b.route.fixup_tw, [&](auto TW) {
         if constexpr (!AC() || !TW())
             hipLaunchKernelGGL((k_spec_fixup<AC(), TW()>), dim3(fix_grid), dim3(64), 0, h->stream, b.a, sa, h->d_spec_mol_begin,
                                h->d_spec_samples, TW() ? h->d_tw_sums : nullptr, TW() ? h->d_tw_cnts : nullptr,
                                TW() ? (uint64_t)h->n_frames : (uint64_t)0);
     }); });
-    hipLaunchKernelGGL(k_spec_finish, dim3(1), dim3(256), 0, h->stream, sa);
+    return GORDER_OK;
+}
+static int resolve_speculation(gorder_hip_handle *h, Batch &b) {
+    if (!b.route.speculative) return GORDER_OK;
+    if (!b.route.sides_at_accumulation) {
+        BATCH_TRY(begin_speculation(h, b));
+        BATCH_TRY(resolve_frames(h, b, 0, b.n_frames));
+    }
+    const uint32_t ring_slot = (uint32_t)(h->spec_batches % gorder_hip_handle::kSpecRing);
+    hipLaunchKernelGGL(k_spec_finish, dim3(1), dim3(256), 0, h->stream, b.sa);
     HIP_TRY(h, hipGetLastError());
     HIP_TRY(h, hipEventRecord(h->spec_counters_copied[ring_slot], h->stream));
-    h->spec_ring_frames[ring_slot] = n_frames;
+    h->spec_ring_frames[ring_slot] = b.n_frames;
     h->spec_batches++;
     return GORDER_OK;
 }
diff --git a/gorder_amd/csrc/kernels_bonds.h b/gorder_amd/csrc/kernels_bonds.h
--- a/gorder_amd/csrc/kernels_bonds.h
+++ b/gorder_amd/csrc/kernels_bonds.h
@@ -35,7 +35,7 @@
     return ((unsigned long long)((lower ? nt : 0u) + t) << 32) | (unsigned long long)(uint32_t)tick;
 }
 
-template <bool ACOS_COS>
+template <bool ACOS_COS, bool NO_PLANE = false>
 __device__ __forceinline__ bool bond_sample(const FrameArgs &a, uint32_t f, float p1x, float p1y, float p1z,
                                             float p2x, float p2y, float p2z, uint32_t mol, SampleAcc &acc,
                                             int &bad, const TiledMapOut *mo = nullptr, unsigned long long *word = nullptr,
@@ -71,7 +71,7 @@
     }
     if (mo) {
         *word = mo->nx == 0u ? tick_sample_word((int)tick, lower)
-                             : map_sample_word(*mo, p1x + vx / 2.0f, p1y + vy / 2.0f, p1z + vz / 2.0f, (int)tick, lower);
+                             : map_sample_word(*mo, p1x + vx / 2.0f, p1y + vy / 2.0f, p1z + vz / 2.0f, (int)tick, !NO_PLANE && lower);
         if (tick_word) *tick_word = tick_sample_word((int)tick, lower);
     }
     return sch != sch;
@@ -145,7 +145,7 @@
         auto stage_word = [&](int k, float vx, float vy, float vz) {
             mo->words[k0 + (uint32_t)k] = OUT == 2
                 ? tick_sample_word(tick[k], LEAF && fl[k] != 0)
-                : map_sample_word(*mo, P[k][0] + vx / 2.0f, P[k][1] + vy / 2.0f, P[k][2] + vz / 2.0f, tick[k], LEAF && fl[k] != 0);
+                : map_sample_word(*mo, P[k][0] + vx / 2.0f, P[k][1] + vy / 2.0f, P[k][2] + vz / 2.0f, tick[k], OUT != 4 && LEAF && fl[k] != 0);
             if (OUT == 3) mo->ticks[k0 + (uint32_t)k] = tick_sample_word(tick[k], LEAF && fl[k] != 0);
         };
 #pragma unroll
@@ -223,7 +223,7 @@
     static __device__ __forceinline__ void compute(const FrameArgs &a, const Tile &t, const Item &it, uint32_t f0,
                                                    const float *lds, uint32_t lw, SampleAcc &acc, int &bad,
                                                    uint32_t &nan_which, uint32_t &nan_frame, const TiledMapOut *mo = nullptr) {
-        constexpr int NF = (OUT == 1 || OUT == 3 || (OUT == 2 && LEAF)) ? 2 : (GORDER_COMPUTE_NF < G ? GORDER_COMPUTE_NF : G);
+        constexpr int NF = (OUT == 1 || OUT == 3 || OUT == 4 || (OUT == 2 && LEAF)) ? 2 : (GORDER_COMPUTE_NF < G ? GORDER_COMPUTE_NF : G);
 #pragma unroll
         for (int h = 0; h < G; h += NF) {
             float P[NF][6];
@@ -251,7 +251,7 @@
                 const float *w = lds + (size_t)k * lw + sh;
                 const float p1x = w[3u * it.li], p1y = w[3u * it.li + 1], p1z = w[3u * it.li + 2];
                 const float p2x = w[3u * it.lj], p2y = w[3u * it.lj + 1], p2z = w[3u * it.lj + 2];
-                if (bond_sample<ACOS_COS>(a, f, p1x, p1y, p1z, p2x, p2y, p2z, it.mol, acc, bad, mo, mo->words + k, OUT == 3 ? mo->ticks + k : nullptr) &&
+                if (bond_sample<ACOS_COS, OUT == 4>(a, f, p1x, p1y, p1z, p2x, p2y, p2z, it.mol, acc, bad, mo, mo->words + k, OUT == 3 ? mo->ticks + k : nullptr) &&
                     nan_frame == kNoNan)
                     note_undefined(p1x, p2x, f, nan_which, nan_frame);
             }
diff --git a/gorder_amd/csrc/kernels_extras.h b/gorder_amd/csrc/kernels_extras.h
--- a/gorder_amd/csrc/kernels_extras.h
+++ b/gorder_amd/csrc/kernels_extras.h
@@ -248,7 +248,7 @@
     fold_tile_sums(a.rep, a.n_rep, a.n_acc, tc, acc, l_s, l_n, [&] { return tile_slots[tc.t.slot0 + tc.tid]; });
 }
 
-template <int NPF, bool PBC, bool LEAF, int AXIS>
+template <int NPF, bool PBC, bool LEAF, int AXIS, bool MOM = false>
 __global__ __launch_bounds__(kBlock, 4) void k_bonds_tiled_maps(FrameArgs a_in, ExtraArgs e, const float *__restrict__ xyz,
                                                                const float *__restrict__ box9, const uint8_t *__restrict__ aflags,
                                                                const uint32_t *__restrict__ arow, const Tile *__restrict__ tiles,
@@ -269,22 +269,35 @@
     int bad = 0;
     uint32_t nan_which = 0, nan_frame = kNoNan;
     v4f pre[NPF];
+    static_assert(!MOM || LEAF, "moments only for a batch with leaflets");
+    constexpr int OUT = MOM ? 4 : 1;
+    uint2 own = make_uint2(0u, 0u), my_head = make_uint2(0u, 0xffffffffu);
+    if (MOM) {
+        own = a.own[tile_id];
+        const uint32_t hq = a.own_head_begin[tile_id] + (tid & 63u);
+        if (hq < a.own_head_begin[tile_id + 1u]) my_head = a.own_heads[hq];
+    }
     if (f_begin < f_full) S::template load<false>(a, t, f_begin, f_end, sk, si, pre);
     for (uint32_t f0 = f_begin; f0 < f_full; f0 += G) {
-        S::template store<false>(a, t, f0, f_end, sk, si, pre, lds, lw);
+        const bool finite = S::template store<false, MOM>(a, t, f0, f_end, sk, si, pre, lds, lw);
         __syncthreads();
         if (f0 + G < f_full) S::template load<false>(a, t, f0 + G, f_end, sk, si, pre);
-        if (active) S::template compute<1>(a, t, it, f0, lds, lw, acc, bad, nan_which, nan_frame, &mo);
+        if (MOM) {
+            static_assert(!MOM || (uint32_t)G * 64u == kBlock, "a wave per frame slot");
+            tiled_moments(a, t, own, tile_id, n_tiles, f0 + sk, lds + (size_t)sk * lw, finite, my_head);
+        }
+        if (active) S::template compute<OUT>(a, t, it, f0, lds, lw, acc, bad, nan_which, nan_frame, &mo);
         rec_store(e, tile_id, f0, tid, words);
         __syncthreads();
     }
     if (f_full < f_end) {
         S::template load<true>(a, t, f_full, f_end, sk, si, pre);
-        S::template store<true>(a, t, f_full, f_end, sk, si, pre, lds, lw);
+        const bool finite = S::template store<true, MOM>(a, t, f_full, f_end, sk, si, pre, lds, lw);
         __syncthreads();
+        if (MOM && f_full + sk < f_end) tiled_moments(a, t, own, tile_id, n_tiles, f_full + sk, lds + (size_t)sk * lw, finite, my_head);
 #pragma unroll
         for (uint32_t m = 0; m < kRecFrames; m++) words[m] = kMapNoSample;
-        if (active) S::template compute_tail<1>(a, t, it, f_full, f_end, lds, lw, acc, bad, nan_which, nan_frame, &mo);
+        if (active) S::template compute_tail<OUT>(a, t, it, f_full, f_end, lds, lw, acc, bad, nan_which, nan_frame, &mo);
         rec_store(e, tile_id, f_full, tid, words);
         __syncthreads();
     }
@@ -405,13 +418,22 @@
 }
 
 constexpr uint32_t kMapRunBatch = 1024;
+struct MapSides {
+    const Tile *tiles;
+    const Item *items;
+    const uint8_t *aflags;
+    uint32_t n_mol_total;
+    uint32_t frame0;
+};
+template <bool SIDES = false>
 __global__ __launch_bounds__(1024) void k_map_accumulate(const unsigned long long *__restrict__ rec,
                                                          const gorder::MapRun *__restrict__ runs,
                                                          const uint32_t *__restrict__ run_begin, uint32_t n_slots,
                                                          uint32_t rec_frames, uint32_t rec_stride,
                                                          uint32_t frames_per_chunk, uint32_t k_max,
                                                          uint32_t n_words , uint32_t n_tiles_map,
-                                                         unsigned long long *__restrict__ map_packed, uint32_t n_acc) {
+                                                         unsigned long long *__restrict__ map_packed, uint32_t n_acc,
+                                                         MapSides sd) {
     extern __shared__ unsigned long long l_map[];
     typedef unsigned long long ull2 __attribute__((ext_vector_type(2)));
     const uint32_t slot = blockIdx.x % n_slots, chunk = blockIdx.x / n_slots;
@@ -462,15 +484,35 @@
                     a2 = __builtin_nontemporal_load(p);
                     b2 = __builtin_nontemporal_load(p + 1);
                 };
-                if (fb_lo < fb_hi) fetch(fb_lo, na, nb);
+                const uint8_t *side = nullptr;
+                uint32_t cs = 0, ns = 0;
+                auto fetch_sides = [&](uint32_t fb) {
+                    uint32_t bits = 0;
+#pragma unroll
+                    for (uint32_t m = 0; m < kRecFrames; m++)
+                        bits |= (side[(size_t)min(kRecFrames * fb + m, rec_frames - 1u) * sd.n_mol_total] != 0 ? 1u : 0u) << m;
+                    return bits;
+                };
+                if constexpr (SIDES) {
+                    const uint32_t mol = sd.items[sd.tiles[run.tile].item0 + run.tid0 + (item - l_pref[lo])].mol;
+                    side = sd.aflags + (size_t)(1u + sd.frame0) * sd.n_mol_total + mol;
+                }
+                if (fb_lo < fb_hi) {
+                    fetch(fb_lo, na, nb);
+                    if constexpr (SIDES) ns = fetch_sides(fb_lo);
+                }
                 for (uint32_t fb = fb_lo; fb < fb_hi; fb++) {
-                    wa = na; wb = nb;
-                    if (fb + 1u < fb_hi) fetch(fb + 1u, na, nb);
+                    wa = na; wb = nb; cs = ns;
+                    if (fb + 1u < fb_hi) {
+                        fetch(fb + 1u, na, nb);
+                        if constexpr (SIDES) ns = fetch_sides(fb + 1u);
+                    }
                     const unsigned long long w[4] = {wa.x, wa.y, wb.x, wb.y};
 #pragma unroll
                     for (uint32_t m = 0; m < 4u; m++) {
                         if (w[m] == kMapNoSample) continue;
-                        const uint32_t pt = (uint32_t)(w[m] >> 32);
+                        uint32_t pt = (uint32_t)(w[m] >> 32);
+                        if constexpr (SIDES) pt += (cs >> m) & 1u ? n_tiles_map : 0u;
                         if (sum != 0ull && pt != cur) { atomicAdd(&l_map[cur], sum); sum = 0ull; }
                         cur = pt;
                         sum += kMapOne + (unsigned long long)(long long)(int)(uint32_t)w[m];
diff --git a/gorder_amd/csrc/kernels_leaflets.h b/gorder_amd/csrc/kernels_leaflets.h
--- a/gorder_amd/csrc/kernels_leaflets.h
+++ b/gorder_amd/csrc/kernels_leaflets.h
@@ -375,6 +375,7 @@
     const float *xyz;
     const float *box9;
     uint32_t n_atoms, n_frames, n_tiles, n_mol_total, n_membrane;
+    uint32_t f_lo, f_hi;
     uint32_t dim;
     int flip, pbc;
     const float4 *mom;
@@ -391,7 +392,7 @@
 __global__ __launch_bounds__(256) void k_spec_check(SpecArgs a) {
     __shared__ float s_center;
     __shared__ int s_ok;
-    for (uint32_t f = blockIdx.x; f < a.n_frames; f += gridDim.x) {
+    for (uint32_t f = a.f_lo + blockIdx.x; f < a.f_hi; f += gridDim.x) {
         const float L = a.pbc ? a.box9[9 * (size_t)f + 4 * a.dim] : 0.0f;
         if (threadIdx.x < 64u) {
             double S = 0.0, Q = 0.0;
@@ -444,9 +445,9 @@
 __global__ __launch_bounds__(64) void k_spec_fixup(FrameArgs a, SpecArgs sa, const uint32_t *__restrict__ mol_begin,
                                                    const SpecSample *__restrict__ samples, unsigned long long *tw_sums,
                                                    unsigned long long *tw_cnts, uint64_t tw_row0) {
-    const uint64_t n_pairs = (uint64_t)sa.n_frames * sa.n_mol_total;
+    const uint64_t n_pairs = (uint64_t)sa.f_hi * sa.n_mol_total;
     uint32_t moved = 0;
-    for (uint64_t p0 = (uint64_t)blockIdx.x * 64u; p0 < n_pairs; p0 += (uint64_t)gridDim.x * 64u) {
+    for (uint64_t p0 = (uint64_t)sa.f_lo * sa.n_mol_total + (uint64_t)blockIdx.x * 64u; p0 < n_pairs; p0 += (uint64_t)gridDim.x * 64u) {
         const uint64_t pi = p0 + threadIdx.x;
         bool differs = false;
         uint32_t exact_l = 0;
diff --git a/gorder_amd/csrc/order_route.h b/gorder_amd/csrc/order_route.h
--- a/gorder_amd/csrc/order_route.h
+++ b/gorder_amd/csrc/order_route.h
@@ -19,6 +19,7 @@
     bool dist = false;
     bool classes = false;
     bool ua_samples_flag = false;
+    bool maps_one_read = false;
 };
 enum class UaKernel { None, Extras, Dist, Mol };
 enum class BondFamily { None, Tiled, Gather, TiledTw, TiledMaps, Extras, Shells, TiledMol, Dist, Classes };
@@ -35,6 +36,7 @@
     bool map_accumulate = false, direct = false;
     bool speculative = false, fixup_ac = false, fixup_tw = false;
     UaKernel ua_kernel = UaKernel::None;
+    bool sides_at_accumulation = false;
 };
 
 inline OrderRoute choose_order_route(const OrderRouteIn &in) {
@@ -63,11 +65,18 @@
     r.ua_fast = in.ua_tiles && in.ua_fast_flag && !in.acos;
     r.ua_kernel = !in.ua_tiles ? UaKernel::None : in.ua_samples_flag && in.mol_rows ? UaKernel::Mol : in.ua_samples_flag && in.dist ? UaKernel::Dist : UaKernel::Extras;
     r.map_accumulate = staged; r.direct = in.direct_items;
-    r.speculative = (r.family == BondFamily::Tiled || (r.family == BondFamily::TiledTw && !r.tw_maps)) && in.leaflets && in.global_leaflets &&
+    const bool maps_spec = r.family == BondFamily::TiledMaps && in.maps_one_read && !in.ua_tiles && !in.direct_items;
+    r.speculative = (r.family == BondFamily::Tiled || (r.family == BondFamily::TiledTw && !r.tw_maps) || maps_spec) && in.leaflets && in.global_leaflets &&
                     in.spec_enabled && in.have_assignment && in.every_frame_assigns && !in.manual_frames && !in.normal_table;
     r.mom = r.speculative;
+    r.sides_at_accumulation = r.speculative && r.family == BondFamily::TiledMaps;
     r.fixup_tw = in.tw; r.fixup_ac = in.acos && !in.tw;
     return r;
+}
+
+constexpr uint64_t kMapsOneReadMinBytes = (uint64_t)128 << 20;
+inline bool maps_one_read_pays(uint32_t n_frames, uint32_t n_atoms, uint64_t min_bytes) {
+    return (uint64_t)n_frames * n_atoms >= min_bytes / 12u + (min_bytes % 12u ? 1u : 0u);
 }
 
 struct FrameChunks { uint32_t frames_per_chunk, n_chunks; };
```
